# a16z/Lasso

Measured on AMD Instinct MI355X. Metric: prover lookups/sec for SparsePolynomialEvaluationProof, 2^24 AND lookups, higher is better.
Workload: dtype u256 (Montgomery Fr / ed25519 Fq integers)

## Files before the change

lasso_amd/_abi.py:

```python
import ctypes as C

u64 = C.c_uint64
u32 = C.c_uint32
i32 = C.c_int32
sz = C.c_size_t
vp = C.c_void_p


class Strategy(C.Structure):
    _fields_ = [("kind", i32), ("c", u32), ("log_m", u32), ("log_r", u32)]


class StrategyCustom(C.Structure):
    _fields_ = [("base", Strategy), ("num_subtables", u32), ("num_memories", u32), ("tables_u32", C.POINTER(vp)), ("tables_fr", C.POINTER(vp)),
                ("memory_subtable", vp), ("memory_dimension", vp), ("num_terms", u32), ("reserved", u32), ("coeff", vp), ("term_start", vp), ("term_mem", vp)]


class OperandLayout(C.Structure):
    _fields_ = [("operands", u32), ("chunk_bits", u32), ("msb_first", u32)]

    def __repr__(self):
        return f"OperandLayout({self.operands}, {self.chunk_bits}, {self.msb_first})"


# ... 101 lines not shown
        "lasso_rccl_selftest": (i32, [vp]),
        "lasso_ctx_device_uuid": (i32, [vp, vp]),
        "lasso_bullet_tail_ahead_ok": (i32, [vp, vp]),
        "lasso_bullet_tail_ahead": (i32, [vp, vp, sz, vp, vp, vp, sz, vp, vp, vp]),
        "lasso_bases_prepare": (i32, [vp, vp, u32]),
        "lasso_rccl_allgather": (i32, [vp, vp, vp, sz]),
        "lasso_point_row_bytes": (sz, []),
        "lasso_hyrax_commit_rows_dev": (i32, [vp, vp, sz, sz, vp, vp]),
        "lasso_points_reduce_compress": (i32, [vp, vp, u32, sz, vp]),
        "lasso_gather_u32": (i32, [vp, vp, vp, sz, vp]),
        "lasso_materialize_subtable_u32": (i32, [vp, P(Strategy), u32, vp]),
        "lasso_msm": (i32, [vp, vp, vp, sz, vp]),
        "lasso_msm_dev": (i32, [vp, vp, vp, sz, vp]),
        "lasso_inner_products_lr": (i32, [vp, vp, vp, sz, vp]),
        "lasso_bullet_lr": (i32, [vp, vp, sz, vp, sz, vp, vp, vp]),
        "lasso_bullet_round": (i32, [vp, vp, sz, vp, vp, vp, vp, vp, vp, sz, vp, vp, vp, vp]),
        "lasso_bullet_ahead_ok": (i32, [vp, vp]),
        "lasso_bullet_round_ahead": (i32, [vp, vp, sz, vp, vp, vp, vp, vp, vp, sz, vp]),
        "lasso_bullet_post": (i32, [vp, vp, vp]),
        "lasso_bullet_fold": (i32, [vp, vp, vp, sz, vp, sz, vp, vp, vp]),
    }
    for name, (res, args) in sig.items():
        fn = getattr(lib, name)
        fn.restype = res
        fn.argtypes = args
    return sorted(sig)


WIRE_STATUS = ["ok", "ok-identity", "non-canonical", "bad-flags", "not-on-curve", "not-in-subgroup"]


def declare_wire(lib):
    fn = lib.lasso_points_decompress
    fn.restype = i32
    fn.argtypes = [vp, vp, sz, vp, vp, vp]
    return ["lasso_points_decompress"]


def declare_msm_points(lib):
    for name in ("lasso_msm_points", "lasso_msm_points_dev"):
        fn = getattr(lib, name)
        fn.restype = i32
        fn.argtypes = [vp, vp, vp, sz, vp]
    return ["lasso_msm_points", "lasso_msm_points_dev"]


def declare_operands(lib):
    fn = lib.lasso_densify_dim_operands
    fn.restype = i32
    fn.argtypes = [vp, vp, vp, sz, C.POINTER(OperandLayout), sz, sz, sz, u32, u32, u32, vp, vp, vp, vp]
    return ["lasso_densify_dim_operands"]


HEADER_SYMBOLS = None
```

lasso_amd/build.py:

```python
import os
import subprocess
import sys

HERE = os.path.dirname(os.path.abspath(__file__))
ROOT = os.path.dirname(HERE)
HIPCC = os.environ.get("HIPCC", "/opt/rocm/bin/hipcc")
ARCH = "gfx950"


def _stale(target, sources):
    if not os.path.exists(target):
        return True
    t = os.path.getmtime(target)
    return any(os.path.getmtime(s) > t for s in sources)


def _glob(d, exts):
    return [os.path.join(d, f) for f in sorted(os.listdir(d)) if f.endswith(exts)]


CURVES = {"curve25519": ("", []), "bn254": ("_bn254", ["-DLASSO_BN254", "-Wl,-Bsymbolic"])}


def build_device(force=False, verbose=False, curve="curve25519"):
    suffix, flags = CURVES[curve]
    csrc = os.path.join(HERE, "csrc")
    target = os.path.join(HERE, f"liblasso_hip{suffix}.so")
    sources = _glob(csrc, (".hip", ".cuh")) + [os.path.join(ROOT, "include", f) for f in ("lasso_hip.h", "lasso_hip_wire.h", "lasso_hip_msm.h", "lasso_hip_operands.h", "lasso_custom_check.h")]
    if force or _stale(target, sources):
        extra = os.environ.get("LASSO_EXTRA_HIPCC_FLAGS", "").split()
        cmd = [HIPCC, f"--offload-arch={ARCH}", "-O3", "-std=c++17", "-fPIC", "-shared", "-Wno-unused-result", *flags, *extra,
               "-o", target, os.path.join(csrc, "lasso_hip.hip")]
        if verbose:
            print(" ".join(cmd))
        subprocess.check_call(cmd)
    return target


def host_march_flags():
    ov = os.environ.get("LASSO_HOST_MARCH")
    if ov:
        return [] if ov == "none" else [f"-march={ov}"] + (["-DLASSO_HOST_V3"] if ov == "x86-64-v3" else [])
    try:
        flags = set(next(l for l in open("/proc/cpuinfo") if l.startswith("flags")).split())
    except Exception:
        flags = set()
    if {"avx2", "bmi1", "bmi2", "fma", "movbe"} <= flags:
        return ["-march=x86-64-v3", "-DLASSO_HOST_V3"]
    return []


def build_host(force=False, verbose=False, curve="curve25519"):
    suffix, flags = CURVES[curve]
    hdir = os.path.join(HERE, "host")
    target = os.path.join(HERE, f"liblasso_prover{suffix}.so")
    sources = _glob(hdir, (".cpp", ".hpp")) + _glob(os.path.join(HERE, "csrc"), (".cuh",)) + [os.path.join(ROOT, "include", f) for f in ("lasso_hip.h", "lasso_hip_wire.h", "lasso_hip_msm.h", "lasso_hip_operands.h", "lasso_prover.h", "lasso_custom_check.h")]
    if not os.path.exists(os.path.join(hdir, "prover_capi.cpp")):
        return None
    dev = build_device(force=False, verbose=verbose, curve=curve)
    if force or _stale(target, sources + [dev]):
        cmd = ["g++", "-O2", *host_march_flags(), "-std=c++17", "-fPIC", "-shared", "-Wall", "-Wno-unused-function", "-Wno-unknown-pragmas", "-fno-gnu-unique", "-Wl,-Bsymbolic", *flags, "-o", target,
               os.path.join(hdir, "prover_capi.cpp"), "-L" + HERE, f"-llasso_hip{suffix}", "-Wl,-rpath,$ORIGIN"]
        if verbose:
            print(" ".join(cmd))
        subprocess.check_call(cmd)
    return target


def build_all(force=False, verbose=False):
    out = []
    for curve in CURVES:
        out += [build_device(force, verbose, curve), build_host(force, verbose, curve)]
    return tuple(out)


if __name__ == "__main__":
    print(build_all(force="--force" in sys.argv, verbose=True))
```

lasso_amd/csrc/densify_kernels.cuh:

```cuda
#pragma once
#include <hip/hip_runtime.h>
#include "fr29.cuh"
#include "operand_layout.cuh"

#define RADIX_TILE 4096
#define RADIX_THREADS 256

__global__ void __launch_bounds__(256) k_densify_extract(const uint64_t* __restrict__ idx, size_t n_lookups, size_t C, size_t col, size_t s, uint64_t m, uint32_t world, uint32_t rank,
                                                          uint32_t* __restrict__ keys, uint32_t* __restrict__ vals, uint32_t* __restrict__ dim_u32, fr_t* __restrict__ dim_fr, uint32_t* __restrict__ bad) {
  const fr29 r2s = fr29_r2s();
  for (size_t k = blockIdx.x * (size_t)blockDim.x + threadIdx.x; k < s; k += (size_t)gridDim.x * blockDim.x) {
    uint64_t a = k < n_lookups ? idx[k * C + col] : 0;
    if (a >= m) { atomicOr(bad, 1u); a = 0; }
    keys[k] = (uint32_t)a; vals[k] = (uint32_t)k;
    if (k % world == rank) { dim_u32[k / world] = (uint32_t)a; dim_fr[k / world] = fr29_store(fr29_mul(fr29_from_u64_int(a), r2s)); }
  }
}

__global__ void __launch_bounds__(256) k_densify_extract_operands(const uint64_t* __restrict__ x, const uint64_t* __restrict__ y, size_t n_lookups, lasso_operand_layout layout, size_t C, size_t col, size_t s,
                                                                   uint32_t world, uint32_t rank, uint32_t* __restrict__ keys, uint32_t* __restrict__ vals, uint32_t* __restrict__ dim_u32,
                                                                   fr_t* __restrict__ dim_fr, uint32_t* __restrict__ bad) {
  const fr29 r2s = fr29_r2s();
  for (size_t k = blockIdx.x * (size_t)blockDim.x + threadIdx.x; k < s; k += (size_t)gridDim.x * blockDim.x) {
    uint64_t a = 0;
// ... 44 lines not shown
  for (size_t b0 = 0; b0 < nb; b0 += 256) {
    const size_t i = b0 + threadIdx.x;
    const uint32_t v = i < nb ? sums[i] : 0;
    uint32_t total; const uint32_t ex = block_exscan_256(v, sm, total);
    if (i < nb) sums[i] = carry + ex;
    __syncthreads();
    if (threadIdx.x == 0) carry += total;
    __syncthreads();
  }
}
__global__ void __launch_bounds__(256) k_scan_apply(uint32_t* __restrict__ data, size_t n, const uint32_t* __restrict__ sums) {
  __shared__ uint32_t sm[256];
  const size_t base = (size_t)blockIdx.x * 4096 + (size_t)threadIdx.x * 16;
  uint32_t v[16], s = 0;
  for (int j = 0; j < 16; j++) { v[j] = base + j < n ? data[base + j] : 0; s += v[j]; }
  uint32_t total; uint32_t run = sums[blockIdx.x] + block_exscan_256(s, sm, total);
  for (int j = 0; j < 16; j++) if (base + j < n) { data[base + j] = run; run += v[j]; }
}

__global__ void __launch_bounds__(RADIX_THREADS) k_radix_scatter(const uint32_t* __restrict__ keys_in, const uint32_t* __restrict__ vals_in, size_t n, uint32_t shift, const uint32_t* __restrict__ offs,
                                                                  uint32_t ntiles, uint32_t* __restrict__ keys_out, uint32_t* __restrict__ vals_out) {
  __shared__ uint32_t next[256];
  const uint32_t t = threadIdx.x, tile = blockIdx.x, lane = t & 63, wave = t >> 6;
  next[t] = offs[(size_t)t * ntiles + tile];
  __syncthreads();
  const size_t base = (size_t)tile * RADIX_TILE;
  for (uint32_t r = 0; r < RADIX_TILE / RADIX_THREADS; r++) {
    const size_t i = base + r * RADIX_THREADS + t;
    const bool valid = i < n;
    const uint32_t key = valid ? keys_in[i] : 0, val = valid ? vals_in[i] : 0, d = (key >> shift) & 255u;
    uint64_t peers = __ballot(valid);
#pragma unroll
    for (int b = 0; b < 8; b++) { const uint64_t bal = __ballot((d >> b) & 1u); peers &= ((d >> b) & 1u) ? bal : ~bal; }
    const uint32_t rank = (uint32_t)__popcll(peers & ((1ull << lane) - 1ull)), cnt = (uint32_t)__popcll(peers);
    uint32_t pos = 0;
    for (uint32_t w = 0; w < RADIX_THREADS / 64; w++) {
      if (wave == w && valid) pos = next[d] + rank;
      __syncthreads();
      if (wave == w && valid && rank == 0) next[d] += cnt;
      __syncthreads();
    }
    if (valid) { keys_out[pos] = key; vals_out[pos] = val; }
  }
}

__global__ void __launch_bounds__(256) k_densify_runs(const uint32_t* __restrict__ skeys, size_t s, uint32_t* __restrict__ run_start, uint32_t* __restrict__ run_end) {
  for (size_t i = blockIdx.x * (size_t)blockDim.x + threadIdx.x; i < s; i += (size_t)gridDim.x * blockDim.x) {
    const uint32_t a = skeys[i];
    if (i == 0 || skeys[i - 1] != a) run_start[a] = (uint32_t)i;
    if (i + 1 == s || skeys[i + 1] != a) run_end[a] = (uint32_t)(i + 1);
  }
}
__global__ void __launch_bounds__(256) k_densify_read(const uint32_t* __restrict__ skeys, const uint32_t* __restrict__ svals, size_t s, const uint32_t* __restrict__ run_start, uint32_t world,
                                                       uint32_t rank, fr_t* __restrict__ read_fr) {
  const fr29 r2s = fr29_r2s();
  for (size_t i = blockIdx.x * (size_t)blockDim.x + threadIdx.x; i < s; i += (size_t)gridDim.x * blockDim.x) {
    const uint32_t pos = svals[i];
    if (pos % world != rank) continue;
    const uint32_t ts = (uint32_t)i - run_start[skeys[i]];
    read_fr[pos / world] = fr29_store(fr29_mul(fr29_from_u64_int(ts), r2s));
  }
}
__global__ void __launch_bounds__(256) k_densify_final(const uint32_t* __restrict__ run_start, const uint32_t* __restrict__ run_end, size_t m, uint32_t world, uint32_t rank, fr_t* __restrict__ final_fr) {
  const fr29 r2s = fr29_r2s();
  for (size_t a = (blockIdx.x * (size_t)blockDim.x + threadIdx.x) * world + rank; a < m; a += (size_t)gridDim.x * blockDim.x * world)
    final_fr[a / world] = fr29_store(fr29_mul(fr29_from_u64_int(run_end[a] - run_start[a]), r2s));
}
```

lasso_amd/csrc/device_switches.cuh:

```cuda
#pragma once
#include <cstddef>
#include <cstdint>
#include <cstdlib>

namespace lasso { namespace dsw {
inline bool unless0(const char* e) { return !(e && e[0] == '0'); }
inline bool if1(const char* e) { return e && e[0] == '1'; }
#define LASSO_DSWITCH(type, name, value) inline type name() { static const type v = (value); return v; }
LASSO_DSWITCH(bool, tagged_results, unless0(getenv("LASSO_TAGGED_RESULTS")))
LASSO_DSWITCH(long long, seq_start, [] { const char* e = getenv("LASSO_SEQ_START"); return e ? (long long)(uint32_t)strtoul(e, nullptr, 0) : -1LL; }())
LASSO_DSWITCH(bool, msm_tagged, unless0(getenv("LASSO_MSM_TAGGED")))
LASSO_DSWITCH(long, cubic_nx, [] { const char* e = getenv("LASSO_CUBIC_NX"); return e ? atol(e) : 0L; }())
LASSO_DSWITCH(bool, cubic_wide, unless0(getenv("LASSO_CUBIC_WIDE")))
LASSO_DSWITCH(unsigned, direct_nx, [] { const char* e = getenv("LASSO_DIRECT_NX"); const long x = e ? atol(e) : 16; return (unsigned)(x < 0 ? 0 : x > 64 ? 64 : x); }())
LASSO_DSWITCH(bool, eq_inline_big, if1(getenv("LASSO_EQ_INLINE_BIG")))
LASSO_DSWITCH(bool, lb_pipeline, unless0(getenv("LASSO_LB_PIPELINE")))
LASSO_DSWITCH(bool, lb_nt, if1(getenv("LASSO_LB_NT")))
LASSO_DSWITCH(unsigned, ahead_inkernel_wgs, [] { const char* e = getenv("LASSO_AHEAD_INKERNEL_WGS"); const long x = e ? atol(e) : 32; return (unsigned)(x < 0 ? 0 : x > 4096 ? 4096 : x); }())
LASSO_DSWITCH(bool, rounds_ahead, unless0(getenv("LASSO_ROUNDS_AHEAD")))
LASSO_DSWITCH(bool, layer_ahead, unless0(getenv("LASSO_LAYER_AHEAD")))
LASSO_DSWITCH(bool, tail_q_256, [] { const char* e = getenv("LASSO_TAIL_Q"); return (e ? atol(e) : 0) == 256; }())
LASSO_DSWITCH(bool, exp_no_leaf_store, if1(getenv("LASSO_EXP_NO_LEAF_STORE")))
LASSO_DSWITCH(size_t, msm_direct_max_n, [] { const char* e = getenv("LASSO_MSM_DIRECT_MAX_N"); return e ? (size_t)atoll(e) : (((size_t)1 << 17) + 64); }())
LASSO_DSWITCH(size_t, msm_direct8_max_n, [] { if (!unless0(getenv("LASSO_MSM_DIRECT8"))) return (size_t)0; const char* e = getenv("LASSO_MSM_DIRECT8_MAX_N"); return e ? (size_t)atoll(e) : (((size_t)1 << 14) + 64); }())
LASSO_DSWITCH(bool, msm_direct, unless0(getenv("LASSO_MSM_DIRECT")))
LASSO_DSWITCH(long, msm_direct_wgs, [] { const char* e = getenv("LASSO_MSM_DIRECT_WGS"); return e ? atol(e) : 0L; }())
LASSO_DSWITCH(bool, msm_fused, unless0(getenv("LASSO_MSM_FUSED")))
LASSO_DSWITCH(bool, msm_rows8, unless0(getenv("LASSO_MSM_ROWS8")))
LASSO_DSWITCH(bool, msm_rows8w, unless0(getenv("LASSO_MSM_ROWS8W")))
LASSO_DSWITCH(size_t, msm_rows8w_waves, [] { const char* e = getenv("LASSO_MSM_ROWS8W_WAVES"); const long x = e ? atol(e) : 0; return (size_t)(x < 0 ? 0 : x); }())
LASSO_DSWITCH(bool, msm_full8, if1(getenv("LASSO_MSM_FULL8")))
LASSO_DSWITCH(bool, bullet_ahead, unless0(getenv("LASSO_BULLET_AHEAD")))
LASSO_DSWITCH(bool, bullet_tail_ahead, unless0(getenv("LASSO_BULLET_TAIL_AHEAD")))
inline bool msm_pip() { return unless0(getenv("LASSO_MSM_PIP")); }
inline size_t msm_pip_min_cols() { const char* e = getenv("LASSO_MSM_PIP_MIN_COLS"); const long x = e ? atol(e) : 512; return (size_t)(x < 1 ? 1 : x); }
inline size_t msm_pip_scratch_mb() { const char* e = getenv("LASSO_MSM_PIP_SCRATCH_MB"); const long x = e ? atol(e) : 1200; return (size_t)(x < 16 ? 16 : x); }
#undef LASSO_DSWITCH
} }
```

lasso_amd/csrc/fr29.cuh:

```cuda
#pragma once
#include <stdint.h>
#include "fr.cuh"
#include "mont29.cuh"

#ifdef LASSO_BN254
struct Bn254FrM {
  static LHD int32_t p(int k) { const int32_t P[9] = {268435457, 521120927, 240919632, 131109107, 361091715, 47923392, 10936641, 240920116, 3171406}; return P[k]; }
  static constexpr uint32_t PINV = 268435455u;
  static constexpr int32_t QC = 1420063842;
  static constexpr int32_t ONE_S_0 = 268435287, ONE_S_1 = 514263732, ONE_S_2 = 86771339, ONE_S_3 = 391139145, ONE_S_4 = 178784091, ONE_S_5 = 490881230, ONE_S_6 = 299191303,
                           ONE_S_7 = 86689704, ONE_S_8 = 903222;
  static constexpr int32_t K522_0 = 95853524, K522_1 = 102173274, K522_2 = 34397646, K522_3 = 498479371, K522_4 = 240439551, K522_5 = 486036963, K522_6 = 471195907,
                           K522_7 = 131109217, K522_8 = 656714;
  static LHD m29<Bn254FrM> k5() { return m29_limbs<Bn254FrM>(268430039, 492061940, 71535269, 62181526, 323781850, 244503300, 348886451, 68918589, 360451); }
  static LHD m29<Bn254FrM> k10() { return m29_limbs<Bn254FrM>(268262109, 223975601, 492627914, 522739689, 150938553, 164142673, 394138283, 408892696, 2020216); }
  static LHD m29<Bn254FrM> r2s() { return m29_limbs<Bn254FrM>(338539743, 433494286, 343078028, 115075043, 193254777, 284818167, 304038784, 396432094, 1209799); }
};
typedef Bn254FrM FrM29;
#else
struct Curve25519FrM {
  static LHD int32_t p(int k) { const int32_t P[9] = {485872621, 9640146, 501691798, 502512965, 333, 0, 0, 0, 1 << 20}; return P[k]; }
  static constexpr uint32_t PINV = 307527195u;
  static constexpr int32_t ONE_S_0 = 290322925, ONE_S_1 = 442594051, ONE_S_2 = 259787148, ONE_S_3 = 377041255, ONE_S_4 = 536700270, ONE_S_5 = 536870911, ONE_S_6 = 536870911,
                           ONE_S_7 = 536870911, ONE_S_8 = 1048575;
// ... 14 lines not shown

template <> LHD m29<FrM29> m29_canonical<FrM29>(const m29<FrM29>& a) {
  m29<FrM29> w = m29_weak(a);
  const int32_t f = w.v[8] >> 20;
  m29<FrM29> r; int64_t c = 0;
#pragma unroll
  for (int k = 0; k < 9; k++) { int64_t x = (int64_t)w.v[k] - (int64_t)f * FrM29::p(k) + c; if (k < 8) { r.v[k] = (int32_t)x & M29_MASK; c = x >> 29; } else r.v[8] = (int32_t)x; }
  const int32_t g = r.v[8] >> 20;
  m29<FrM29> s; c = 0;
#pragma unroll
  for (int k = 0; k < 9; k++) { int64_t x = (int64_t)r.v[k] - (int64_t)g * FrM29::p(k) + c; if (k < 8) { s.v[k] = (int32_t)x & M29_MASK; c = x >> 29; } else s.v[8] = (int32_t)x; }
  const bool keep_r = s.v[8] < 0;
#pragma unroll
  for (int k = 0; k < 9; k++) s.v[k] = keep_r ? r.v[k] : s.v[k];
  return s;
}
template <> LHD m29<FrM29> m29_reduce_columns<FrM29>(const int64_t* col, int shift) {
  int64_t l[9]; int64_t c = 0;
#pragma unroll
  for (int k = 0; k < 9; k++) { const int64_t x = col[k] * ((int64_t)1 << shift) + c; if (k < 8) { l[k] = x & M29_MASK; c = x >> 29; } else l[8] = x; }
  const int32_t f = (int32_t)(l[8] >> 20) - 1;
  m29<FrM29> r; c = 0;
#pragma unroll
  for (int k = 0; k < 9; k++) { const int64_t x = l[k] - (int64_t)f * FrM29::p(k) + c; if (k < 8) { r.v[k] = (int32_t)x & M29_MASK; c = x >> 29; } else r.v[8] = (int32_t)x; }
  return m29_canonical(r);
}
template <> LHD m29<FrM29> m29_from_columns<FrM29>(const int64_t* col) {
  const int32_t ONE_S[9] = {FrM29::ONE_S_0, FrM29::ONE_S_1, FrM29::ONE_S_2, FrM29::ONE_S_3, FrM29::ONE_S_4, FrM29::ONE_S_5, FrM29::ONE_S_6, FrM29::ONE_S_7, FrM29::ONE_S_8};
  int64_t l[9]; int64_t c = 0;
#pragma unroll
  for (int k = 0; k < 9; k++) { int64_t x = col[k] + c; c = x >> 29; l[k] = x & M29_MASK; }
  m29<FrM29> r; int64_t d = 0;
#pragma unroll
  for (int k = 0; k < 9; k++) { int64_t x = l[k] + c * ONE_S[k] + d; if (k < 8) { r.v[k] = (int32_t)x & M29_MASK; d = x >> 29; } else r.v[8] = (int32_t)x; }
  return r;
}
#endif

typedef m29<FrM29> fr29;
typedef m29_acc<FrM29> fr29_acc;
#define FR29_MASK M29_MASK

static constexpr auto& fr29_from_limbs = m29_limbs<FrM29>;
#ifdef LASSO_BN254
LHD fr29 fr29_zero() { return m29_zero<FrM29>(); }
LHD fr29 fr29_add(const fr29& a, const fr29& b) { return m29_add(a, b); }
LHD fr29 fr29_sub(const fr29& a, const fr29& b) { return m29_sub(a, b); }
LHD fr29 fr29_weak(const fr29& a) { return m29_weak(a); }
LHD fr29 fr29_mul(const fr29& a, const fr29& b) { return m29_mul(a, b); }
LHD fr29_acc fr29_acc_zero() { return m29_acc_zero<FrM29>(); }
LHD void fr29_mul_acc(fr29_acc& acc, const fr29& a, const fr29& b) { m29_mul_acc(acc, a, b); }
LHD void fr29_acc_carry(fr29_acc& acc) { m29_acc_carry(acc); }
LHD fr29 fr29_acc_reduce(const fr29_acc& acc) { return m29_acc_reduce(acc); }
LHD fr29 fr29_semi(const fr29& a) { return m29_near(a); }
LHD fr29 fr29_canonical(const fr29& a) { return m29_canonical(a); }
LHD fr29 fr29_reduce_columns(const int64_t* col, int shift) { return m29_reduce_columns<FrM29>(col, shift); }
LHD fr29 fr29_from_columns(const int64_t* col) { return m29_from_columns<FrM29>(col); }
LHD fr29 fr29_unpack_u(const fr_t& x) { return m29_unpack_words<FrM29>(x.v); }
LHD fr29 fr29_unpack_s(const fr_t& x) { return m29_unpack_words_shl5<FrM29>(x.v); }
LHD fr_t fr29_pack(const fr29& a) { fr_t r; m29_pack_words(a, r.v); return r; }
#else
static constexpr auto& fr29_zero = m29_zero<FrM29>;
static constexpr auto& fr29_add = m29_add<FrM29>;
static constexpr auto& fr29_sub = m29_sub<FrM29>;
static constexpr auto& fr29_weak = m29_weak<FrM29>;
static constexpr auto& fr29_mul = m29_mul<FrM29>;
static constexpr auto& fr29_acc_zero = m29_acc_zero<FrM29>;
static constexpr auto& fr29_mul_acc = m29_mul_acc<FrM29>;
static constexpr auto& fr29_acc_carry = m29_acc_carry<FrM29>;
static constexpr auto& fr29_acc_reduce = m29_acc_reduce<FrM29>;
static constexpr auto& fr29_semi = m29_near<FrM29>;
static constexpr auto& fr29_canonical = m29_canonical<FrM29>;
static constexpr auto& fr29_reduce_columns = m29_reduce_columns<FrM29>;
static constexpr auto& fr29_from_columns = m29_from_columns<FrM29>;
LHD fr29 fr29_unpack_u(const fr_t& x) {
  fr29 r;
#pragma unroll
  for (int k = 0; k < 9; k++) {
    const int bit = 29 * k, w = bit >> 5, s = bit & 31;
    uint64_t two = (uint64_t)x.v[w] | ((w + 1 < 8) ? ((uint64_t)x.v[w + 1] << 32) : 0);
    r.v[k] = (int32_t)((uint32_t)(two >> s) & FR29_MASK);
  }
  return r;
}
LHD fr29 fr29_unpack_s(const fr_t& x) {
  fr29 r;
  r.v[0] = (int32_t)((x.v[0] << 5) & FR29_MASK);
#pragma unroll
  for (int k = 1; k < 9; k++) {
    const int bit = 29 * k - 5, w = bit >> 5, s = bit & 31;
    uint64_t two = (uint64_t)x.v[w] | ((w + 1 < 8) ? ((uint64_t)x.v[w + 1] << 32) : 0);
    r.v[k] = (int32_t)((uint32_t)(two >> s) & FR29_MASK);
  }
  return r;
}
LHD fr_t fr29_pack(const fr29& a) {
  fr_t r;
#pragma unroll
  for (int w = 0; w < 8; w++) {
    const int k0 = (32 * w) / 29, s = 32 * w - 29 * k0;
    uint64_t acc = (uint64_t)(uint32_t)a.v[k0] >> s;
    int have = 29 - s;
    if (k0 + 1 < 9) { acc |= (uint64_t)(uint32_t)a.v[k0 + 1] << have; have += 29; }
    if (have < 32 && k0 + 2 < 9) acc |= (uint64_t)(uint32_t)a.v[k0 + 2] << have;
    r.v[w] = (uint32_t)acc;
  }
  return r;
}
#endif

LHD fr29 fr29_one_s() { return fr29_from_limbs(FrM29::ONE_S_0, FrM29::ONE_S_1, FrM29::ONE_S_2, FrM29::ONE_S_3, FrM29::ONE_S_4, FrM29::ONE_S_5, FrM29::ONE_S_6, FrM29::ONE_S_7, FrM29::ONE_S_8); }
LHD fr29 fr29_k5() { return FrM29::k5(); }
LHD fr29 fr29_k10() { return FrM29::k10(); }
LHD fr29 fr29_r2s() { return FrM29::r2s(); }
LHD fr29 fr29_int_from_uu() { fr29 r = fr29_zero(); r.v[0] = 1 << 10; return r; }
LHD fr29 fr29_from_u64_int(uint64_t x) { return fr29_from_limbs((int32_t)(x & FR29_MASK), (int32_t)((x >> 29) & FR29_MASK), (int32_t)(x >> 58), 0, 0, 0, 0, 0, 0); }
LHD fr_t fr29_store(const fr29& a) { return fr29_pack(fr29_canonical(a)); }
```

lasso_amd/csrc/lasso_hip.hip:

```cpp
#include <hip/hip_runtime.h>
#include <mutex>
#include <string>
#include <unordered_map>
#include <vector>
#include <cstring>
#include <functional>
#include <cstdio>
#include <cstdlib>
#include <ctime>
#include "../../include/lasso_hip.h"
#include "device_switches.cuh"
#include "launch_plan.cuh"
#include "poly_kernels.cuh"
#include "msm_kernels.cuh"
#include "densify_kernels.cuh"
#include "../../include/lasso_hip_wire.h"
#include "wire_kernels.cuh"
#include "../../include/lasso_hip_msm.h"
#include "msm_points_kernels.cuh"
#include "../../include/lasso_hip_operands.h"

__global__ void __launch_bounds__(256) k_inner_lr(const fr_t* __restrict__ a, const fr_t* __restrict__ b, size_t half, fr_t* __restrict__ partials) {
  __shared__ RedScratch S;
  fr29 acc[3] = {fr29_zero(), fr29_zero(), fr29_zero()}; uint32_t cnt = 0;
  for (size_t i = blockIdx.x * (size_t)blockDim.x + threadIdx.x; i < half; i += (size_t)gridDim.x * blockDim.x) {
    acc[0] = fr29_weak(fr29_add(acc[0], fr29_mul(fr29_unpack_u(a[i]), fr29_unpack_s(b[half + i]))));
    acc[1] = fr29_weak(fr29_add(acc[1], fr29_mul(fr29_unpack_u(a[half + i]), fr29_unpack_s(b[i]))));
    if ((++cnt & 127u) == 0) { acc[0] = fr29_mul(acc[0], fr29_one_s()); acc[1] = fr29_mul(acc[1], fr29_one_s()); }
  }
  store_block_partials<3>(acc, 2, partials + 2 * (size_t)blockIdx.x, 0, S);
}

static_assert(sizeof(lasso_fr) == 32 && sizeof(fr_t) == 32, "Fr layout");
static_assert(sizeof(lasso_affine) == 64 && sizeof(lasso_point) == 128 && sizeof(ed_point) == 128 && sizeof(niels29) == (MSM_NIELS_ALIGN > 16 ? 128 : 112) && sizeof(pt29) == MSM_PT29_BYTES, "curve layouts");

namespace dsw = lasso::dsw;
struct EventPair { hipEvent_t a, b; int kid; double bytes, units, units2; bool large; bool counted; };
#define LASSO_PROF_COUNT_SLOTS 4096
struct lasso_ctx {
  int device = 0;
  hipStream_t stream = nullptr;
  std::string err;
  void* d_scratch = nullptr; size_t scratch_cap = 0;
  void* d_pip = nullptr; size_t pip_cap = 0;
  fr_t* d_small = nullptr;
  fr_t* h_small = nullptr;
  size_t small_cap = 0;
  uint32_t* h_flag = nullptr; uint32_t* d_flag = nullptr;
  uint32_t* h_tag = nullptr; uint32_t* d_tag = nullptr;
  bool tagged = true;
  HandoffState proto;
  std::vector<lasso_fr> group_tmp;
  uint32_t* mail_h = nullptr; uint32_t* mail_d = nullptr;
  uint32_t seq = 0;
  uint64_t stat_waits = 0; double stat_wait_us = 0;
  fr_t* d_big = nullptr; fr_t* h_big = nullptr; size_t big_cap = 0;
  uint32_t* d_flags = nullptr;
  uint32_t* d_counters = nullptr;
  uint32_t* d_gmail = nullptr;
  uint32_t* pmail_h = nullptr; uint32_t* pmail_d = nullptr; uint32_t* d_gpoint = nullptr;
  uint32_t prof_mask = 0;
  std::vector<EventPair> events; size_t events_used = 0;
  uint64_t prof_launches[LASSO_K_COUNT] = {0}; double prof_ms[LASSO_K_COUNT] = {0}; double prof_bytes[LASSO_K_COUNT] = {0};
  uint64_t big_launches[LASSO_K_COUNT] = {0}; double big_ms[LASSO_K_COUNT] = {0}; double big_bytes[LASSO_K_COUNT] = {0};
  double prof_units[LASSO_K_COUNT] = {0}; double big_units[LASSO_K_COUNT] = {0};
  double prof_units2[LASSO_K_COUNT] = {0}; double big_units2[LASSO_K_COUNT] = {0};
  double prof_units3[LASSO_K_COUNT] = {0}; double big_units3[LASSO_K_COUNT] = {0};
  uint32_t* d_prof_counts = nullptr;
  void* d_terms = nullptr; std::vector<uint8_t> terms_host;
  void* rccl_comm = nullptr; int rccl_world = 0; int rccl_rank = -1;
  std::unordered_map<void*, size_t> mem_sizes; uint64_t mem_live = 0, mem_peak = 0; std::mutex mem_mu;
};
struct lasso_bases {
  size_t n = 0; niels29* d_table = nullptr;
  lasso_ctx* owner = nullptr;
  niels29* d_mult = nullptr;
  niels29* d_mult8 = nullptr;
  niels29* d_tab8[2] = {nullptr, nullptr};
  bool tab8_failed = false;
  std::mutex tab8_mu;
};

static thread_local std::string g_create_err;
static std::mutex g_ctx_mu; static std::vector<lasso_ctx*> g_ctx_live;
static lasso_ctx* live_or_null(lasso_ctx* c) { std::lock_guard<std::mutex> g(g_ctx_mu); for (lasso_ctx* x : g_ctx_live) if (x == c) return c; return nullptr; }

static int32_t fail(lasso_ctx* c, int32_t code, const std::string& msg) { if (c) c->err = msg; else g_create_err = msg; return code; }
#define HIPCHK(c, call) do { hipError_t e_ = (call); if (e_ != hipSuccess) return fail((c), e_ == hipErrorOutOfMemory ? LASSO_ERR_OOM : LASSO_ERR_HIP, std::string(#call) + ": " + hipGetErrorString(e_)); } while (0)
static inline bool bind_device(lasso_ctx* c) { if (!c) return true; int d = -1; if (hipGetDevice(&d) == hipSuccess && d == c->device) return true; return hipSetDevice(c->device) == hipSuccess; }
#define REQUIRE(c, cond) do { if (!bind_device(c)) return fail((c), LASSO_ERR_HIP, "hipSetDevice failed for the context's device"); \
                              if (!(cond)) return fail((c), LASSO_ERR_INVALID, std::string("invalid argument: ") + #cond); } while (0)

static hipError_t dmalloc(lasso_ctx* c, void** p, size_t bytes) {
  hipError_t e = hipMalloc(p, bytes);
  if (e == hipSuccess && c) { std::lock_guard<std::mutex> g(c->mem_mu); c->mem_sizes[*p] = bytes; c->mem_live += bytes; if (c->mem_live > c->mem_peak) c->mem_peak = c->mem_live; }
  return e;
}
static hipError_t dfree(lasso_ctx* c, void* p) {
  if (c && p) { std::lock_guard<std::mutex> g(c->mem_mu); auto it = c->mem_sizes.find(p); if (it != c->mem_sizes.end()) { c->mem_live -= it->second; c->mem_sizes.erase(it); } }
  return hipFree(p);
}

static int32_t grow_guard(lasso_ctx* c) {
  if (c->proto.no_grow) return LASSO_ERR_UNSUPPORTED;
  if (c->proto.waiting_on_device()) return fail(c, LASSO_ERR_INVALID, "a launch is waiting on the device for its challenge: only lasso_result_wait and the post of that challenge are legal until then");
  return 0;
}
static int32_t ensure_scratch(lasso_ctx* c, size_t bytes) {
  if (bytes <= c->scratch_cap) return 0;
  if (int32_t g = grow_guard(c)) return g;
// ... 985 lines not shown
}
int32_t lasso_read_heads(lasso_ctx* c, const lasso_fr* const* d_polys, uint32_t k, lasso_fr* out) {
  REQUIRE(c, d_polys && out && k >= 1 && k <= LASSO_MAX_PTRS);
  PtrTable P; for (uint32_t i = 0; i < k; i++) { REQUIRE(c, d_polys[i]); P.p[i] = (const fr_t*)d_polys[i]; }
  int32_t rc = ensure_small(c, k); if (rc) return rc;
  hipLaunchKernelGGL(k_read_heads, dim3(1), dim3(LASSO_BLOCK), 0, c->stream, P, k, c->d_small);
  HIPCHK(c, hipGetLastError());
  return fetch_small(c, k, out);
}
int32_t lasso_read_runs(lasso_ctx* c, const lasso_fr* const* d_polys, uint32_t k, uint32_t count, lasso_fr* out) {
  REQUIRE(c, d_polys && out && k >= 1 && k <= LASSO_MAX_PTRS && count >= 1 && (size_t)k * count <= 16384);
  PtrTable P; for (uint32_t i = 0; i < k; i++) { REQUIRE(c, d_polys[i]); P.p[i] = (const fr_t*)d_polys[i]; }
  int32_t rc = ensure_small(c, (size_t)k * count); if (rc) return rc;
  hipLaunchKernelGGL(k_read_runs, dim3((k * count + LASSO_BLOCK - 1) / LASSO_BLOCK), dim3(LASSO_BLOCK), 0, c->stream, P, k, count, c->d_small);
  HIPCHK(c, hipGetLastError());
  return fetch_small(c, (size_t)k * count, out);
}
static void gp_layers_from(lasso_ctx* c, fr_t* in, size_t len) {
  while (len >= 16 * LASSO_BLOCK) {
    const size_t q = len / 4;
    hipLaunchKernelGGL(k_gp_layer2, dim3(grid_for(q, 4096)), dim3(LASSO_BLOCK), 0, c->stream, (const fr_t*)in, q, in + len, in + len + len / 2);
    in += len + len / 2; len = q;
  }
  while (len > 2 * LASSO_BLOCK) {
    size_t half = len / 2;
    hipLaunchKernelGGL(k_gp_layer, dim3(grid_for(half, 4096)), dim3(LASSO_BLOCK), 0, c->stream, (const fr_t*)in, half, in + len);
    in += len; len = half;
  }
  if (len > 2) hipLaunchKernelGGL(k_gp_tail, dim3(1), dim3(LASSO_BLOCK), 0, c->stream, in, len);
}
int32_t lasso_gp_build(lasso_ctx* c, lasso_fr* d_tree, size_t n) {
  REQUIRE(c, d_tree && n >= 2 && (n & (n - 1)) == 0);
  ProfScope ps(c, LASSO_K_GP, 48.0 * n * 2.0);
  gp_layers_from(c, (fr_t*)d_tree, n);
  HIPCHK(c, hipGetLastError()); return 0;
}
int32_t lasso_fingerprint_ops_gp(lasso_ctx* c, const lasso_fr* d_table, const uint32_t* d_dim, const lasso_fr* d_read, size_t s, const lasso_fr* gamma, const lasso_fr* tau,
                                 lasso_fr* d_tree_r, lasso_fr* d_tree_w) {
  REQUIRE(c, d_table && d_dim && d_read && gamma && tau && d_tree_r && d_tree_w && s >= 4 && (s & (s - 1)) == 0);
  fr_t g = to_fr(gamma), g2 = fr_sqr(g), t = to_fr(tau);
  fr_t* tr = (fr_t*)d_tree_r; fr_t* tw = (fr_t*)d_tree_w;
  {
    ProfScope ps(c, LASSO_K_FINGERPRINT, (32.0 * 3 + 64.0) * s + 2 * 48.0 * s);
    const uint32_t store_leaves = dsw::exp_no_leaf_store() ? 0u : 1u;
    hipLaunchKernelGGL(k_fingerprint_ops_l1<false>, dim3(grid_for(s / 2, 4096)), dim3(LASSO_BLOCK), 0, c->stream, (const fr_t*)d_table, d_dim, (const void*)d_read, s, g, g2, t, tr, tw, tr + s, tw + s, store_leaves);
  }
  {
    ProfScope ps(c, LASSO_K_GP, 2 * 48.0 * s);
    gp_layers_from(c, tr + s, s / 2);
    gp_layers_from(c, tw + s, s / 2);
  }
  HIPCHK(c, hipGetLastError()); return 0;
}
static int32_t fingerprint_gp_upper_impl(lasso_ctx* c, const lasso_fr* d_table, const uint32_t* d_dim, const void* d_read, bool read_u32, size_t s, const lasso_fr* gamma, const lasso_fr* tau,
                                         lasso_fr* d_upper_r, lasso_fr* d_upper_w) {
  REQUIRE(c, d_table && d_dim && d_read && gamma && tau && d_upper_r && d_upper_w && s >= 4 && (s & (s - 1)) == 0);
  fr_t g = to_fr(gamma), g2 = fr_sqr(g), t = to_fr(tau);
  fr_t* ur = (fr_t*)d_upper_r; fr_t* uw = (fr_t*)d_upper_w;
  {
    ProfScope ps(c, LASSO_K_FINGERPRINT, (32.0 * 3 + 64.0) * s + 2 * 48.0 * s);
    if (read_u32) hipLaunchKernelGGL(k_fingerprint_ops_l1<true>, dim3(grid_for(s / 2, 4096)), dim3(LASSO_BLOCK), 0, c->stream, (const fr_t*)d_table, d_dim, d_read, s, g, g2, t, (fr_t*)nullptr, (fr_t*)nullptr, ur, uw, 0u);
    else hipLaunchKernelGGL(k_fingerprint_ops_l1<false>, dim3(grid_for(s / 2, 4096)), dim3(LASSO_BLOCK), 0, c->stream, (const fr_t*)d_table, d_dim, d_read, s, g, g2, t, (fr_t*)nullptr, (fr_t*)nullptr, ur, uw, 0u);
  }
  {
    ProfScope ps(c, LASSO_K_GP, 2 * 48.0 * s);
    gp_layers_from(c, ur, s / 2);
    gp_layers_from(c, uw, s / 2);
  }
  HIPCHK(c, hipGetLastError()); return 0;
}
int32_t lasso_fingerprint_ops_gp_upper(lasso_ctx* c, const lasso_fr* d_table, const uint32_t* d_dim, const lasso_fr* d_read, size_t s, const lasso_fr* gamma, const lasso_fr* tau,
                                       lasso_fr* d_upper_r, lasso_fr* d_upper_w) { return fingerprint_gp_upper_impl(c, d_table, d_dim, d_read, false, s, gamma, tau, d_upper_r, d_upper_w); }
int32_t lasso_fingerprint_ops_gp_upper_u32(lasso_ctx* c, const lasso_fr* d_table, const uint32_t* d_dim, const uint32_t* d_read_u32, size_t s, const lasso_fr* gamma, const lasso_fr* tau,
                                           lasso_fr* d_upper_r, lasso_fr* d_upper_w) { return fingerprint_gp_upper_impl(c, d_table, d_dim, d_read_u32, true, s, gamma, tau, d_upper_r, d_upper_w); }
static int32_t fingerprint_strips_impl(lasso_ctx* c, const lasso_fr* d_table, const uint32_t* d_dim, const void* d_read, bool read_u32, size_t s, const lasso_fr* gamma, const lasso_fr* tau,
                                       uint32_t nstrips, size_t i0, size_t cs, lasso_fr* d_out_r, lasso_fr* d_out_w) {
  REQUIRE(c, d_table && d_dim && d_read && gamma && tau && d_out_r && d_out_w && s >= 4 && (s & (s - 1)) == 0 && (nstrips == 2 || nstrips == 4) && cs >= 1);
  const size_t stride = s / 2 / nstrips;
  REQUIRE(c, stride >= 1 && i0 + cs <= stride);
  fr_t g = to_fr(gamma), g2 = fr_sqr(g), t = to_fr(tau);
  const size_t total = 2 * (size_t)nstrips * cs;
  ProfScope ps(c, LASSO_K_FINGERPRINT, (32.0 * 3 + 64.0) * total);
  if (read_u32) hipLaunchKernelGGL(k_fingerprint_ops_strips<true>, dim3(grid_for(total, 4096)), dim3(LASSO_BLOCK), 0, c->stream, (const fr_t*)d_table, d_dim, d_read, s, g, g2, t, nstrips, stride, i0, cs, (fr_t*)d_out_r, (fr_t*)d_out_w);
  else hipLaunchKernelGGL(k_fingerprint_ops_strips<false>, dim3(grid_for(total, 4096)), dim3(LASSO_BLOCK), 0, c->stream, (const fr_t*)d_table, d_dim, d_read, s, g, g2, t, nstrips, stride, i0, cs, (fr_t*)d_out_r, (fr_t*)d_out_w);
  HIPCHK(c, hipGetLastError()); return 0;
}
int32_t lasso_fingerprint_ops_strips(lasso_ctx* c, const lasso_fr* d_table, const uint32_t* d_dim, const lasso_fr* d_read, size_t s, const lasso_fr* gamma, const lasso_fr* tau,
                                     uint32_t nstrips, size_t i0, size_t cs, lasso_fr* d_out_r, lasso_fr* d_out_w) { return fingerprint_strips_impl(c, d_table, d_dim, d_read, false, s, gamma, tau, nstrips, i0, cs, d_out_r, d_out_w); }
int32_t lasso_fingerprint_ops_strips_u32(lasso_ctx* c, const lasso_fr* d_table, const uint32_t* d_dim, const uint32_t* d_read_u32, size_t s, const lasso_fr* gamma, const lasso_fr* tau,
                                         uint32_t nstrips, size_t i0, size_t cs, lasso_fr* d_out_r, lasso_fr* d_out_w) { return fingerprint_strips_impl(c, d_table, d_dim, d_read_u32, true, s, gamma, tau, nstrips, i0, cs, d_out_r, d_out_w); }
int32_t lasso_fingerprint_ops(lasso_ctx* c, const lasso_fr* d_table, const uint32_t* d_dim, const lasso_fr* d_read, size_t s, const lasso_fr* gamma, const lasso_fr* tau,
                              lasso_fr* d_read_out, lasso_fr* d_write_out) {
  REQUIRE(c, d_table && d_dim && d_read && gamma && tau && d_read_out && d_write_out); if (!s) return 0;
  fr_t g = to_fr(gamma), g2 = fr_sqr(g), t = to_fr(tau);
  ProfScope ps(c, LASSO_K_FINGERPRINT, (32.0 * 3 + 64.0) * s);
  hipLaunchKernelGGL(k_fingerprint_ops, dim3(grid_for(s, 4096)), dim3(LASSO_BLOCK), 0, c->stream, (const fr_t*)d_table, d_dim, (const fr_t*)d_read, s, g, g2, t, (fr_t*)d_read_out, (fr_t*)d_write_out);
  HIPCHK(c, hipGetLastError()); return 0;
}
int32_t lasso_fingerprint_mem(lasso_ctx* c, const lasso_fr* d_table, const lasso_fr* d_final, size_t m, const lasso_fr* gamma, const lasso_fr* tau, lasso_fr* d_init_out, lasso_fr* d_final_out) {
  return lasso_fingerprint_mem_slab(c, d_table, d_final, m, 1, 0, gamma, tau, d_init_out, d_final_out);
}
int32_t lasso_fingerprint_mem_slab(lasso_ctx* c, const lasso_fr* d_table, const lasso_fr* d_final, size_t m, uint32_t world, uint32_t rank, const lasso_fr* gamma, const lasso_fr* tau,
                                   lasso_fr* d_init_out, lasso_fr* d_final_out) {
  REQUIRE(c, d_table && d_final && gamma && tau && d_init_out && d_final_out && world >= 1 && rank < world); if (!m) return 0;
  fr_t g = to_fr(gamma), g2 = fr_sqr(g), t = to_fr(tau);
  ProfScope ps(c, LASSO_K_FINGERPRINT, (64.0 + 64.0) * m);
// ... 17 lines not shown
  HIPCHK(c, hipGetLastError());
  HIPCHK(c, hipMemcpyAsync(c->h_big, c->d_big, r_size * sizeof(fr_t), hipMemcpyDeviceToHost, c->stream));
  HIPCHK(c, hipStreamSynchronize(c->stream));
  memcpy(out, c->h_big, r_size * sizeof(fr_t));
  return 0;
}

int32_t lasso_matvec_left_dev(lasso_ctx* c, const lasso_fr* d_Z, const lasso_fr* d_L, size_t l_size, size_t r_size, lasso_fr* d_out) {
  REQUIRE(c, d_Z && d_L && d_out && l_size >= 1 && r_size >= 1);
  size_t col_blocks = (r_size + LASSO_BLOCK - 1) / LASSO_BLOCK;
  size_t nchunks = (1024 + col_blocks - 1) / col_blocks; if (nchunks > l_size) nchunks = l_size; if (nchunks < 1) nchunks = 1;
  size_t rows_per_chunk = (l_size + nchunks - 1) / nchunks; nchunks = (l_size + rows_per_chunk - 1) / rows_per_chunk;
  int32_t rc = ensure_scratch(c, nchunks * r_size * sizeof(fr_t)); if (rc) return rc;
  fr_t* partials = (fr_t*)c->d_scratch;
  ProfScope ps(c, LASSO_K_MATVEC, 32.0 * l_size * r_size);
  hipLaunchKernelGGL(k_matvec_left, dim3((unsigned)col_blocks, (unsigned)nchunks), dim3(LASSO_BLOCK), 0, c->stream, (const fr_t*)d_Z, (const fr_t*)d_L, l_size, r_size, rows_per_chunk, partials);
  hipLaunchKernelGGL(k_matvec_reduce, dim3((unsigned)col_blocks), dim3(LASSO_BLOCK), 0, c->stream, (const fr_t*)partials, nchunks, r_size, (fr_t*)d_out);
  HIPCHK(c, hipGetLastError()); return 0;
}
int32_t lasso_fr_to_u32(lasso_ctx* c, const lasso_fr* d_src, size_t n, uint32_t* d_dst, uint32_t* max_out) {
  REQUIRE(c, d_src && d_dst && n >= 1);
  HIPCHK(c, hipMemsetAsync(c->d_flags, 0, 8, c->stream));
  hipLaunchKernelGGL(k_fr_to_u32, dim3(grid_for(n, 4096)), dim3(256), 0, c->stream, (const fr_t*)d_src, n, d_dst, c->d_flags);
  HIPCHK(c, hipGetLastError());
  uint32_t flags[2];
  HIPCHK(c, hipMemcpyAsync(flags, c->d_flags, 8, hipMemcpyDeviceToHost, c->stream));
  HIPCHK(c, hipStreamSynchronize(c->stream));
  if (flags[1]) return fail(c, LASSO_ERR_INVALID, "lasso_fr_to_u32: a value does not fit 32 bits");
  if (max_out) *max_out = flags[0];
  return 0;
}
int32_t lasso_fr_to_bytes(lasso_ctx* c, const lasso_fr* d_src, size_t n, uint8_t* out) {
  REQUIRE(c, d_src && out && n >= 1);
  if (n <= ((size_t)1 << 16)) {
    int32_t rc = ensure_small(c, n); if (rc) return rc;
    hipLaunchKernelGGL(k_fr_to_canonical, dim3(grid_for(n)), dim3(256), 0, c->stream, (const fr_t*)d_src, n, c->d_small);
    HIPCHK(c, hipGetLastError());
    return fetch_small(c, n, (lasso_fr*)out);
  }
  int32_t rc = ensure_scratch(c, n * sizeof(fr_t)); if (rc) return rc;
  hipLaunchKernelGGL(k_fr_to_canonical, dim3(grid_for(n)), dim3(256), 0, c->stream, (const fr_t*)d_src, n, (fr_t*)c->d_scratch);
  HIPCHK(c, hipGetLastError());
  HIPCHK(c, hipMemcpyAsync(out, c->d_scratch, n * 32, hipMemcpyDeviceToHost, c->stream));
  HIPCHK(c, hipStreamSynchronize(c->stream));
  return 0;
}

int32_t lasso_densify_dim(lasso_ctx* c, const uint64_t* d_indices, size_t n_lookups, size_t C, size_t dim, size_t s, uint32_t log_m, uint32_t* d_dim_u32, lasso_fr* d_dim, lasso_fr* d_read,
                          lasso_fr* d_final) {
  return lasso_densify_dim_slab(c, d_indices, n_lookups, C, dim, s, log_m, 1, 0, d_dim_u32, d_dim, d_read, d_final);
}
static int32_t densify_dim_run(lasso_ctx* c, size_t n_lookups, size_t s, uint32_t log_m, uint32_t world, uint32_t rank, lasso_fr* d_read, lasso_fr* d_final, double extract_bytes,
                               const char* bad_msg, const std::function<void(uint32_t*, uint32_t*)>& extract) {
  const size_t m = (size_t)1 << log_m;
  const uint32_t ntiles = (uint32_t)((s + RADIX_TILE - 1) / RADIX_TILE);
  const size_t nh = (size_t)256 * ntiles, nb = (nh + 4095) / 4096;
  const size_t words = 4 * s + nh + nb + 2 * m + 64;
  int32_t rc = ensure_scratch(c, words * 4); if (rc) return rc;
  uint32_t* kA = (uint32_t*)c->d_scratch; uint32_t* vA = kA + s; uint32_t* kB = vA + s; uint32_t* vB = kB + s;
  uint32_t* hist = vB + s; uint32_t* sums = hist + nh; uint32_t* run_start = sums + nb; uint32_t* run_end = run_start + m;
  HIPCHK(c, hipMemsetAsync(c->d_flags, 0, 8, c->stream));
  HIPCHK(c, hipMemsetAsync(run_start, 0, 2 * m * 4, c->stream));
  ProfScope ps(c, LASSO_K_MISC, extract_bytes + (32.0 * 2 + 4.0) * s + 32.0 * m);
  extract(kA, vA);
  const uint32_t npass = log_m == 0 ? 1 : (log_m + 7) / 8;
  for (uint32_t p = 0; p < npass; p++) {
    hipLaunchKernelGGL(k_radix_hist, dim3(ntiles), dim3(RADIX_THREADS), 0, c->stream, (const uint32_t*)kA, s, 8 * p, hist, ntiles);
    hipLaunchKernelGGL(k_scan_block_sums, dim3((unsigned)nb), dim3(256), 0, c->stream, (const uint32_t*)hist, nh, sums);
    hipLaunchKernelGGL(k_scan_sums, dim3(1), dim3(256), 0, c->stream, sums, nb);
    hipLaunchKernelGGL(k_scan_apply, dim3((unsigned)nb), dim3(256), 0, c->stream, hist, nh, (const uint32_t*)sums);
    hipLaunchKernelGGL(k_radix_scatter, dim3(ntiles), dim3(RADIX_THREADS), 0, c->stream, (const uint32_t*)kA, (const uint32_t*)vA, s, 8 * p, (const uint32_t*)hist, ntiles, kB, vB);
    std::swap(kA, kB); std::swap(vA, vB);
  }
  hipLaunchKernelGGL(k_densify_runs, dim3(grid_for(s, 4096)), dim3(256), 0, c->stream, (const uint32_t*)kA, s, run_start, run_end);
  hipLaunchKernelGGL(k_densify_read, dim3(grid_for(s, 4096)), dim3(256), 0, c->stream, (const uint32_t*)kA, (const uint32_t*)vA, s, (const uint32_t*)run_start, world, rank, (fr_t*)d_read);
  hipLaunchKernelGGL(k_densify_final, dim3(grid_for(m / world, 4096)), dim3(256), 0, c->stream, (const uint32_t*)run_start, (const uint32_t*)run_end, m, world, rank, (fr_t*)d_final);
  HIPCHK(c, hipGetLastError());
  uint32_t flags[2];
  HIPCHK(c, hipMemcpyAsync(flags, c->d_flags, 8, hipMemcpyDeviceToHost, c->stream));
  HIPCHK(c, hipStreamSynchronize(c->stream));
  if (flags[0]) return fail(c, LASSO_ERR_INVALID, bad_msg);
  return 0;
}
int32_t lasso_densify_dim_slab(lasso_ctx* c, const uint64_t* d_indices, size_t n_lookups, size_t C, size_t dim, size_t s, uint32_t log_m, uint32_t world, uint32_t rank, uint32_t* d_dim_u32,
                               lasso_fr* d_dim, lasso_fr* d_read, lasso_fr* d_final) {
  REQUIRE(c, d_indices && d_dim_u32 && d_dim && d_read && d_final && C >= 1 && dim < C && s >= 1 && (s & (s - 1)) == 0 && n_lookups <= s && s < ((size_t)1 << 32) && log_m <= 32);
  REQUIRE(c, world >= 1 && (world & (world - 1)) == 0 && rank < world && world <= s && world <= ((size_t)1 << log_m));
  return densify_dim_run(c, n_lookups, s, log_m, world, rank, d_read, d_final, 8.0 * n_lookups, "lookup index out of range (memory_address >= M, densified.rs:46)", [&](uint32_t* kA, uint32_t* vA) {
    hipLaunchKernelGGL(k_densify_extract, dim3(grid_for(s, 4096)), dim3(256), 0, c->stream, d_indices, n_lookups, C, dim, s, (uint64_t)1 << log_m, world, rank, kA, vA, d_dim_u32, (fr_t*)d_dim, c->d_flags);
  });
}
int32_t lasso_densify_dim_operands(lasso_ctx* c, const uint64_t* d_x, const uint64_t* d_y, size_t n_lookups, const lasso_operand_layout* layout, size_t C, size_t dim, size_t s, uint32_t log_m,
                                   uint32_t world, uint32_t rank, uint32_t* d_dim_u32, lasso_fr* d_dim, lasso_fr* d_read, lasso_fr* d_final) {
  REQUIRE(c, d_x && d_dim_u32 && d_dim && d_read && d_final && C >= 1 && dim < C && s >= 1 && (s & (s - 1)) == 0 && n_lookups <= s && s < ((size_t)1 << 32) && log_m <= 32);
  REQUIRE(c, world >= 1 && (world & (world - 1)) == 0 && rank < world && world <= s && world <= ((size_t)1 << log_m));
  if (const int bad = operand_layout_check(layout, C, log_m)) return fail(c, LASSO_ERR_INVALID, std::string("lasso_densify_dim_operands: ") + operand_layout_error(bad));
  if ((d_y != nullptr) != (layout->operands == 2u)) return fail(c, LASSO_ERR_INVALID, "lasso_densify_dim_operands: " OPL_MSG_Y);
  const lasso_operand_layout L = *layout;
  return densify_dim_run(c, n_lookups, s, log_m, world, rank, d_read, d_final, 8.0 * L.operands * n_lookups, "lasso_densify_dim_operands: " OPL_MSG_FIT, [&](uint32_t* kA, uint32_t* vA) {
    hipLaunchKernelGGL(k_densify_extract_operands, dim3(grid_for(s, 4096)), dim3(256), 0, c->stream, d_x, d_y, n_lookups, L, C, dim, s, world, rank, kA, vA, d_dim_u32, (fr_t*)d_dim, c->d_flags);
  });
}

int32_t lasso_points_decompress(lasso_ctx* c, const uint8_t* wire32, size_t n, lasso_affine* out, uint8_t* canon32, uint8_t* status) {
  REQUIRE(c, status && (wire32 || n == 0) && n < ((size_t)1 << 31));
  if (!n) return 0;
  int32_t rc = ensure_scratch(c, 129 * n);
  if (rc) return rc == LASSO_ERR_UNSUPPORTED ? fail(c, rc, "lasso_points_decompress: the scratch buffer cannot grow while a resident kernel is active") : rc;
  uint8_t* base = (uint8_t*)c->d_scratch;
  HIPCHK(c, hipMemcpyAsync(base, wire32, 32 * n, hipMemcpyHostToDevice, c->stream));
  {
    ProfScope ps(c, LASSO_K_MISC, 129.0 * n);
    hipLaunchKernelGGL(k_points_decompress, dim3((unsigned)((n + WIRE_THREADS - 1) / WIRE_THREADS)), dim3(WIRE_THREADS), 0, c->stream, (const uint4*)base, n, (uint4*)(base + 32 * n), (uint4*)(base + 96 * n), base + 128 * n);
  }
  HIPCHK(c, hipGetLastError());
  std::vector<uint8_t> host(97 * n);
  HIPCHK(c, hipMemcpyAsync(host.data(), base + 32 * n, 97 * n, hipMemcpyDeviceToHost, c->stream));
  HIPCHK(c, hipStreamSynchronize(c->stream));
  if (out) memcpy(out, host.data(), 64 * n);
  if (canon32) memcpy(canon32, host.data() + 64 * n, 32 * n);
  memcpy(status, host.data() + 96 * n, n);
  return 0;
}
int32_t lasso_bases_create(lasso_ctx* c, const lasso_affine* points, size_t n, lasso_bases** out) { return lasso_bases_create_opt(c, points, n, 1, out); }
int32_t lasso_bases_create_opt(lasso_ctx* c, const lasso_affine* points, size_t n, int32_t byte_multiples, lasso_bases** out) {
  REQUIRE(c, points && out && n >= 1 && n * MSM_WINDOWS < ((size_t)1 << 32));
  lasso_bases* b = new lasso_bases(); b->n = n; b->owner = c;
  void* d_aff = nullptr;
// ... 29 lines not shown
  for (niels29* t : b->d_tab8) if (t) (void)dfree(o, t);
  delete b;
}
static const niels29* ensure_tab8(lasso_ctx* c, const lasso_bases* cb, uint32_t w8) {
  lasso_bases* b = const_cast<lasso_bases*>(cb);
  std::lock_guard<std::mutex> lock(b->tab8_mu);
  if (b->d_tab8[w8]) return b->d_tab8[w8];
  if (b->tab8_failed) return nullptr;
  niels29* t = nullptr;
  lasso_ctx* const owner = live_or_null(b->owner);
  if (dmalloc(owner, (void**)&t, (size_t)MSM8_MULTS * b->n * sizeof(niels29)) != hipSuccess) { (void)hipGetLastError(); b->tab8_failed = true; return nullptr; }
  hipLaunchKernelGGL(k_precompute_tab8, dim3((unsigned)((b->n + 63) / 64)), dim3(64), 0, c->stream, (const niels29*)b->d_table, b->n, w8, t);
  if (hipGetLastError() != hipSuccess || hipStreamSynchronize(c->stream) != hipSuccess) { (void)hipGetLastError(); (void)dfree(owner, t); b->tab8_failed = true; return nullptr; }
  b->d_tab8[w8] = t;
  return t;
}
int32_t lasso_bases_prepare(lasso_ctx* c, const lasso_bases* b, uint32_t byte_windows) {
  REQUIRE(c, b && byte_windows >= 1 && byte_windows <= 2 && !c->proto.waiting_on_device() && !c->proto.tail_active);
  if (!dsw::msm_rows8()) return 0;
  for (uint32_t w = 0; w < byte_windows; w++) if (!ensure_tab8(c, b, w)) break;
  return 0;
}

static size_t msm_pts_bytes(size_t rows, size_t n_cols) { return msm_pts_bytes(rows, n_cols, msm_direct_wgs(dsw::msm_direct_wgs())); }
static bool msm_tagged(lasso_ctx* c) { return c->tagged && dsw::msm_tagged(); }
#define MSM_RES(c) (msm_tagged(c) ? (ed_point*)(c)->d_tag : (ed_point*)(c)->d_small), (c)->d_counters + LASSO_MAX_PTRS + 8, (msm_tagged(c) ? LASSO_TAGGED : (c)->d_flag)
static int32_t run_msm_direct(lasso_ctx* c, const uint8_t* d_scal, size_t row_stride, size_t rows, size_t n_cols, const MsmColMap& cm, const lasso_bases* b, uint8_t* scratch_after, lasso_point* out,
                              int mode = 0, const lasso_fr* scale = nullptr, const lasso_fr* tail = nullptr, uint32_t sstride = 1, uint32_t soffset = 0,
                              const lasso_fr* const* heads = nullptr, const uint32_t* gate_seq = nullptr) {
  const MsmDirectPlan P = msm_direct_plan(rows, n_cols, b->d_mult8 != nullptr, dsw::msm_direct_wgs());
  const size_t K = P.K; const uint32_t ipc = P.ipc;
  const uint32_t seq = gate_seq ? *gate_seq : next_seq(c);
  const fr_t* const h0 = heads ? (const fr_t*)heads[0] : nullptr; const fr_t* const h1 = heads ? (const fr_t*)heads[1] : nullptr;
  const uint32_t* const ggm = gate_seq ? (const uint32_t*)c->d_gmail : nullptr;
  {
    ProfScope ps(c, LASSO_K_MSM_DIRECT, (double)rows * n_cols * 32, P.ref_adds, false, P.adds);
    const fr_t z = fr_zero();
#define LAUNCH_DIRECT(M, WB_, TAB_, SC, T0, T1) hipLaunchKernelGGL((k_msm_direct<M, WB_>), dim3((unsigned)K, (unsigned)rows), dim3(MSM_THREADS), 0, c->stream, (const uint32_t*)d_scal, row_stride / 4, (uint32_t)n_cols, ipc, cm, \
                       (const niels29*)TAB_, b->n, (pt29*)scratch_after, MSM_RES(c), seq, SC, T0, T1, ps.counter(), sstride, soffset, h0, h1, ggm)
    if (P.w8) {
      if (mode == 0) LAUNCH_DIRECT(0, 8, b->d_mult8, z, z, z);
      else if (mode == 1) LAUNCH_DIRECT(1, 8, b->d_mult8, z, z, z);
      else LAUNCH_DIRECT(2, 8, b->d_mult8, to_fr(scale), to_fr(tail), to_fr(tail + 1));
    } else {
      if (mode == 0) LAUNCH_DIRECT(0, 4, b->d_mult, z, z, z);
      else if (mode == 1) LAUNCH_DIRECT(1, 4, b->d_mult, z, z, z);
      else LAUNCH_DIRECT(2, 4, b->d_mult, to_fr(scale), to_fr(tail), to_fr(tail + 1));
    }
  }
  HIPCHK(c, hipGetLastError());
  if (gate_seq) return 0;
  return wait_flag(c, seq, rows * (sizeof(ed_point) / sizeof(fr_t)), (lasso_fr*)out, msm_tagged(c));
}
static int32_t run_msm(lasso_ctx* c, const uint8_t* d_scal, uint32_t bps, uint32_t W, size_t row_stride, size_t rows, size_t n_cols, const lasso_bases* b, uint8_t* scratch_after, lasso_point* out,
                       uint8_t* out_compressed = nullptr, void* d_rows_out = nullptr) {
  const MsmShape shape = {bps, W, rows, n_cols, out_compressed != nullptr, d_rows_out != nullptr};
  const MsmSwitches sw = {dsw::msm_direct(), dsw::msm_rows8(), dsw::msm_rows8w(), dsw::msm_full8(), dsw::msm_pip(), dsw::msm_rows8w_waves(), dsw::msm_pip_min_cols(), dsw::msm_pip_scratch_mb(), dsw::msm_direct_wgs()};
  MsmHave have = {b->n, b->d_mult != nullptr, b->d_mult8 != nullptr, true, true};
  MsmPlan P = msm_plan(shape, have, sw);
  if (P.kernel == MSM_K_DIRECT) { const MsmColMap id = {0, 0, 0, 0}; return run_msm_direct(c, d_scal, row_stride, rows, n_cols, id, b, scratch_after, out); }
  const niels29* t8[2] = {nullptr, nullptr};
  if (P.kernel == MSM_K_ROWS8W || P.kernel == MSM_K_ROWS8) {
    t8[0] = ensure_tab8(c, b, 0); t8[1] = P.W8 > 1 && t8[0] ? ensure_tab8(c, b, 1) : t8[0];
    if (!t8[1]) { have.tab8 = false; P = msm_plan(shape, have, sw); }
  } else if (P.kernel == MSM_K_PIP && ensure_pip(c, P.pip_group * P.pip_row_bytes + 256) != 0) { have.pip_scratch = false; P = msm_plan(shape, have, sw); }
  if (d_rows_out) out_compressed = (uint8_t*)d_rows_out;
  const size_t K = P.K;
  pt29* d_partial = (pt29*)scratch_after;
  const bool small = P.result == MSM_R_FLAG;
  ed_point* d_final = small ? (ed_point*)c->d_small : (ed_point*)(((uintptr_t)(d_partial + rows * K) + 15) & ~(uintptr_t)15);
  const uint32_t seq = small ? next_seq(c) : 0;
  {
    ProfScope ps(c, LASSO_K_MSM, (double)rows * n_cols * bps, P.ref_adds, rows > MSM_SMALL_ROWS, P.adds);
    switch (P.kernel) {
      case MSM_K_ROWS8W:
        hipLaunchKernelGGL(k_msm_rows8w, dim3((unsigned)((P.waves + MSM_THREADS / 64 - 1) / (MSM_THREADS / 64))), dim3(MSM_THREADS), 0, c->stream, (const uint32_t*)d_scal, row_stride / 4,
                           (uint32_t)n_cols, P.W8, t8[0], t8[1], b->n, d_partial, (uint32_t)rows, ps.counter(), (uint32_t)P.rpw);
        break;
      case MSM_K_ROWS8:
        hipLaunchKernelGGL(k_msm_rows8, dim3((unsigned)K, (unsigned)rows), dim3(MSM_THREADS), 0, c->stream, (const uint32_t*)d_scal, row_stride / 4, (uint32_t)n_cols, (uint32_t)P.cols_per_chunk, P.W8,
                           t8[0], t8[1], b->n, d_partial, ps.counter());
        break;
      case MSM_K_PIP: {
        const size_t pip_group = P.pip_group, pip_items = P.pip_items;
        uint8_t* base = (uint8_t*)c->d_pip;
        uint32_t* d_sorted = (uint32_t*)base; uint32_t* d_offs = d_sorted + pip_group * pip_items; uint16_t* d_perm = (uint16_t*)(d_offs + pip_group * (MSM_PIP_BUCKETS + 1));
        uint8_t* d_vtop = (uint8_t*)(d_perm + pip_group * MSM_PIP_BUCKETS);
        pt29* d_bk = (pt29*)((((uintptr_t)(d_vtop + pip_group * n_cols)) + 15) & ~(uintptr_t)15);
        for (size_t r0 = 0; r0 < rows; r0 += pip_group) {
          const unsigned g = (unsigned)(rows - r0 < pip_group ? rows - r0 : pip_group);
          hipLaunchKernelGGL(k_msm_pip_sort, dim3(g), dim3(MSM_THREADS), 0, c->stream, d_scal + r0 * row_stride, row_stride, (uint32_t)n_cols, (uint32_t)b->n, d_sorted, pip_items, d_offs, d_perm, d_vtop, ps.counter());
          hipLaunchKernelGGL(k_msm_pip_accumulate, dim3(g, MSM_PIP_PER_THREAD), dim3(MSM_THREADS), 0, c->stream, (const uint32_t*)d_sorted, pip_items, (const uint32_t*)d_offs, (const uint16_t*)d_perm, (const niels29*)b->d_table, d_bk);
          hipLaunchKernelGGL(k_msm_pip_reduce, dim3(g), dim3(MSM_THREADS), 0, c->stream, (const pt29*)d_bk, (const uint8_t*)d_vtop, (uint32_t)n_cols, (const niels29*)b->d_table + (size_t)(MSM_WINDOWS - 1) * b->n, d_partial + r0);
        }
      } break;
      case MSM_K_FULL8:
        hipLaunchKernelGGL((k_msm_rows_full<8>), dim3((unsigned)K, (unsigned)rows), dim3(MSM_THREADS), 0, c->stream, (const uint32_t*)d_scal, row_stride / 4, (uint32_t)n_cols, (uint32_t)P.cols_per_chunk,
                           (const niels29*)b->d_mult8, b->n, d_partial, ps.counter());
        break;
      default:
        hipLaunchKernelGGL(k_msm_buckets, dim3((unsigned)K, (unsigned)rows), dim3(MSM_THREADS), 0, c->stream, d_scal, bps, W, row_stride, n_cols, P.cols_per_chunk, (const niels29*)b->d_table, b->n, d_partial, ps.counter());
    }
    hipLaunchKernelGGL(k_points_sum, dim3((unsigned)rows), dim3(MSM_THREADS), 0, c->stream, (const pt29*)d_partial, (uint32_t)K, d_final, out_compressed ? (uint32_t*)d_final : (uint32_t*)nullptr,
                       c->d_counters + LASSO_MAX_PTRS + 1, small ? c->d_flag : (uint32_t*)nullptr, seq);
  }
  HIPCHK(c, hipGetLastError());
  switch (P.result) {
    case MSM_R_DEVICE_ROWS: HIPCHK(c, hipMemcpyAsync(d_rows_out, d_final, rows * sizeof(pt29), hipMemcpyDeviceToDevice, c->stream)); return 0;
    case MSM_R_COMPRESSED_MAPPED: {
      int32_t rc = ensure_small(c, rows); if (rc) return rc;
      hipLaunchKernelGGL(k_points_compress, dim3((unsigned)((rows + 255) / 256)), dim3(256), 0, c->stream, (const pt29*)d_final, rows, (uint32_t*)c->d_small);
      HIPCHK(c, hipGetLastError());
      return fetch_small(c, rows, (lasso_fr*)out_compressed);
    }
    case MSM_R_COMPRESSED_MEMCPY: {
      uint32_t* d_wire = (uint32_t*)(((uintptr_t)((pt29*)d_final + rows) + 15) & ~(uintptr_t)15);
      hipLaunchKernelGGL(k_points_compress, dim3((unsigned)((rows + 255) / 256)), dim3(256), 0, c->stream, (const pt29*)d_final, rows, d_wire);
      HIPCHK(c, hipGetLastError());
      HIPCHK(c, hipMemcpyAsync(out_compressed, d_wire, rows * 32, hipMemcpyDeviceToHost, c->stream));
      HIPCHK(c, hipStreamSynchronize(c->stream));
      return 0;
    }
    case MSM_R_FLAG: return wait_flag(c, seq, rows * (sizeof(ed_point) / sizeof(fr_t)), (lasso_fr*)out);
    default: break;
  }
  HIPCHK(c, hipMemcpyAsync(out, d_final, rows * sizeof(ed_point), hipMemcpyDeviceToHost, c->stream));
  HIPCHK(c, hipStreamSynchronize(c->stream));
  return 0;
}
static int32_t hyrax_commit_impl(lasso_ctx* c, const lasso_fr* d_Z, size_t l_size, size_t r_size, const lasso_bases* b, lasso_point* out, uint8_t* out_compressed, void* d_rows_out = nullptr);
int32_t lasso_hyrax_commit_rows_dev(lasso_ctx* c, const lasso_fr* d_Z, size_t l_size, size_t r_size, const lasso_bases* b, void* d_rows) { REQUIRE(c, d_rows); return hyrax_commit_impl(c, d_Z, l_size, r_size, b, nullptr, nullptr, d_rows); }
size_t lasso_point_row_bytes(void) { return sizeof(pt29); }
int32_t lasso_hyrax_commit(lasso_ctx* c, const lasso_fr* d_Z, size_t l_size, size_t r_size, const lasso_bases* b, lasso_point* out) { REQUIRE(c, out); return hyrax_commit_impl(c, d_Z, l_size, r_size, b, out, nullptr); }
int32_t lasso_hyrax_commit_compressed(lasso_ctx* c, const lasso_fr* d_Z, size_t l_size, size_t r_size, const lasso_bases* b, uint8_t* out32) { REQUIRE(c, out32); return hyrax_commit_impl(c, d_Z, l_size, r_size, b, nullptr, out32); }
static int32_t hyrax_commit_impl(lasso_ctx* c, const lasso_fr* d_Z, size_t l_size, size_t r_size, const lasso_bases* b, lasso_point* out, uint8_t* out_compressed, void* d_rows_out) {
  REQUIRE(c, d_Z && b && l_size >= 1 && r_size >= 1 && r_size <= b->n && l_size < ((size_t)1 << 31));
  const size_t n = l_size * r_size;
  const size_t pts_bytes = msm_pts_bytes(l_size, r_size);
  int32_t rc = ensure_scratch(c, n * 4 + 256 + pts_bytes); if (rc) return rc;
  uint8_t* d_scal = (uint8_t*)c->d_scratch;
  HIPCHK(c, hipMemsetAsync(c->d_flags, 0, 8, c->stream));
  {
    ProfScope ps(c, LASSO_K_MISC, 36.0 * n);
    hipLaunchKernelGGL(k_fr_to_u32, dim3(grid_for(n, 4096)), dim3(256), 0, c->stream, (const fr_t*)d_Z, n, (uint32_t*)d_scal, c->d_flags);
  }
  uint32_t flags[2];
  HIPCHK(c, hipMemcpyAsync(flags, c->d_flags, 8, hipMemcpyDeviceToHost, c->stream));
  HIPCHK(c, hipStreamSynchronize(c->stream));
  if (!flags[1]) {
    uint32_t bits = 0; while (bits < 32 && (flags[0] >> bits)) bits++;
    uint32_t W = (bits + 3) / 4; if (W == 0) W = 1;
    return run_msm(c, d_scal, 4, W, r_size * 4, l_size, r_size, b, d_scal + ((n * 4 + 255) & ~(size_t)255), out, out_compressed, d_rows_out);
  }
  rc = ensure_scratch(c, n * 32 + pts_bytes); if (rc) return rc;
  d_scal = (uint8_t*)c->d_scratch;
  hipLaunchKernelGGL(k_fr_to_canonical, dim3(grid_for(n, 4096)), dim3(256), 0, c->stream, (const fr_t*)d_Z, n, (fr_t*)d_scal);
  return run_msm(c, d_scal, 32, MSM_WINDOWS, r_size * 32, l_size, r_size, b, d_scal + n * 32, out, out_compressed, d_rows_out);
}
int32_t lasso_hyrax_commit_compressed_u32(lasso_ctx* c, const uint32_t* d_u32, uint32_t max_value, size_t l_size, size_t r_size, const lasso_bases* b, uint8_t* out32) {
  REQUIRE(c, d_u32 && out32 && b && l_size >= 1 && r_size >= 1 && r_size <= b->n && l_size < ((size_t)1 << 31));
  int32_t rc = ensure_scratch(c, msm_pts_bytes(l_size, r_size) + 256); if (rc) return rc;
  uint32_t bits = 0; while (bits < 32 && (max_value >> bits)) bits++;
  uint32_t W = (bits + 3) / 4; if (W == 0) W = 1;
  return run_msm(c, (const uint8_t*)d_u32, 4, W, r_size * 4, l_size, r_size, b, (uint8_t*)c->d_scratch, nullptr, out32);
}
__global__ void __launch_bounds__(256) k_gather_u32(const uint32_t* __restrict__ table, const uint32_t* __restrict__ idx, size_t n, uint32_t* __restrict__ out) {
  for (size_t i = blockIdx.x * (size_t)blockDim.x + threadIdx.x; i < n; i += (size_t)gridDim.x * blockDim.x) out[i] = table[idx[i]];
}
int32_t lasso_gather_u32(lasso_ctx* c, const uint32_t* d_table, const uint32_t* d_idx, size_t n, uint32_t* d_out) {
  REQUIRE(c, d_table && d_idx && d_out); if (!n) return 0;
  ProfScope ps(c, LASSO_K_MISC, 12.0 * n);
  hipLaunchKernelGGL(k_gather_u32, dim3(grid_for(n)), dim3(256), 0, c->stream, d_table, d_idx, n, d_out);
  HIPCHK(c, hipGetLastError()); return 0;
}
int32_t lasso_msm(lasso_ctx* c, const lasso_bases* b, const lasso_fr* scalars, size_t n, lasso_point* out) {
  REQUIRE(c, b && scalars && out && n >= 1 && n <= b->n);
  int32_t rc = ensure_scratch(c, n * 64 + msm_pts_bytes(1, n)); if (rc) return rc;
  fr_t* d_in = (fr_t*)c->d_scratch; fr_t* d_can = d_in + n;
  HIPCHK(c, hipMemcpyAsync(d_in, scalars, n * 32, hipMemcpyHostToDevice, c->stream));
  hipLaunchKernelGGL(k_fr_to_canonical, dim3(grid_for(n)), dim3(256), 0, c->stream, (const fr_t*)d_in, n, d_can);
  return run_msm(c, (const uint8_t*)d_can, 32, MSM_WINDOWS, n * 32, 1, n, b, (uint8_t*)(d_can + n), out);
}

int32_t lasso_msm_dev(lasso_ctx* c, const lasso_bases* b, const lasso_fr* d_scalars, size_t n, lasso_point* out) {
  REQUIRE(c, b && d_scalars && out && n >= 1 && n <= b->n);
  int32_t rc = ensure_scratch(c, n * 32 + msm_pts_bytes(1, n)); if (rc) return rc;
  fr_t* d_can = (fr_t*)c->d_scratch;
  if (b->d_mult && dsw::msm_direct() && dsw::msm_fused()) {
    const MsmColMap id = {0, 0, 0, 0};
    return run_msm_direct(c, (const uint8_t*)d_scalars, n * 32, 1, n, id, b, (uint8_t*)c->d_scratch, out, 1);
  }
  hipLaunchKernelGGL(k_fr_to_canonical, dim3(grid_for(n)), dim3(256), 0, c->stream, (const fr_t*)d_scalars, n, d_can);
  return run_msm(c, (const uint8_t*)d_can, 32, MSM_WINDOWS, n * 32, 1, n, b, (uint8_t*)(d_can + n), out);
}
static inline size_t up256(size_t x) { return (x + 255) & ~(size_t)255; }
static int32_t msm_points_impl(lasso_ctx* c, const char* who, const lasso_affine* points, const lasso_fr* scalars, size_t n, bool on_host, lasso_point* out) {
  REQUIRE(c, out && n < ((size_t)1 << 28) && (n == 0 || (points && scalars)));
  const size_t K = n ? (n + MSMP_CHUNK - 1) / MSMP_CHUNK : 1;
  const size_t o_pts = 0, o_scal = o_pts + (on_host ? up256(n * sizeof(lasso_affine)) : 0), o_nl = o_scal + (on_host ? up256(n * sizeof(lasso_fr)) : 0), o_dig = o_nl + up256(n * sizeof(niels29));
  const size_t o_part = o_dig + up256(n * MSMP_NW), o_wsum = o_part + up256(MSMP_NW * K * sizeof(pt29)), o_out = o_wsum + up256(MSMP_NW * sizeof(pt29));
  int32_t rc = ensure_scratch(c, o_out + 256);
  if (rc) return rc == LASSO_ERR_UNSUPPORTED ? fail(c, rc, std::string(who) + ": the scratch buffer cannot grow while a resident kernel is active") : rc;
  uint8_t* base = (uint8_t*)c->d_scratch;
  const fq_t* d_aff = (const fq_t*)points; const fr_t* d_scal = (const fr_t*)scalars;
  if (on_host && n) {
    HIPCHK(c, hipMemcpyAsync(base + o_pts, points, n * sizeof(lasso_affine), hipMemcpyHostToDevice, c->stream));
    HIPCHK(c, hipMemcpyAsync(base + o_scal, scalars, n * sizeof(lasso_fr), hipMemcpyHostToDevice, c->stream));
    d_aff = (const fq_t*)(base + o_pts); d_scal = (const fr_t*)(base + o_scal);
  }
  {
    ProfScope ps(c, LASSO_K_MSM, (double)n * (sizeof(lasso_affine) + sizeof(lasso_fr)), msm_ref_adds(1, n, FR_MODULUS_BITS), false, (double)n * MSMP_NW);
    if (n) hipLaunchKernelGGL(k_msmp_prepare, dim3((unsigned)((n + 255) / 256)), dim3(256), 0, c->stream, d_aff, d_scal, (uint32_t)n, (niels29*)(base + o_nl), (int8_t*)(base + o_dig));
    hipLaunchKernelGGL(k_msmp_buckets, dim3(MSMP_NW, (unsigned)K), dim3(MSM_THREADS), 0, c->stream, (const int8_t*)(base + o_dig), (uint32_t)n, (const niels29*)(base + o_nl), (pt29*)(base + o_part));
    hipLaunchKernelGGL(k_points_sum, dim3(MSMP_NW), dim3(MSM_THREADS), 0, c->stream, (const pt29*)(base + o_part), (uint32_t)K, (ed_point*)nullptr, (uint32_t*)(base + o_wsum),
                       (uint32_t*)nullptr, (uint32_t*)nullptr, 0u);
    hipLaunchKernelGGL(k_msmp_horner, dim3(1), dim3(64), 0, c->stream, (const pt29*)(base + o_wsum), (ed_point*)(base + o_out));
  }
  HIPCHK(c, hipGetLastError());
  HIPCHK(c, hipMemcpyAsync(out, base + o_out, sizeof(ed_point), hipMemcpyDeviceToHost, c->stream));
  HIPCHK(c, hipStreamSynchronize(c->stream));
  return 0;
}
int32_t lasso_msm_points(lasso_ctx* c, const lasso_affine* points, const lasso_fr* scalars, size_t n, lasso_point* out) { return msm_points_impl(c, "lasso_msm_points", points, scalars, n, true, out); }
int32_t lasso_msm_points_dev(lasso_ctx* c, const lasso_affine* d_points, const lasso_fr* d_scalars, size_t n, lasso_point* out) { return msm_points_impl(c, "lasso_msm_points_dev", d_points, d_scalars, n, false, out); }
__global__ void __launch_bounds__(256) k_scale_to_integers(const fr_t* __restrict__ src, size_t n, fr_t scale, fr_t t0, fr_t t1, fr_t* __restrict__ dst) {
  const fr29 ss = fr29_unpack_s(scale); fr29 k32 = fr29_zero(); k32.v[0] = 32;
  for (size_t i = blockIdx.x * (size_t)blockDim.x + threadIdx.x; i < n; i += (size_t)gridDim.x * blockDim.x) dst[i] = fr29_store(fr29_mul(fr29_mul(fr29_unpack_u(src[i]), ss), k32));
// ... 148 lines not shown
```

lasso_amd/csrc/mont29.cuh:

```cuda
#pragma once
#include <stdint.h>

#ifndef LHD
#if defined(__HIPCC__)
#define LHD __host__ __device__ __forceinline__
#else
#define LHD inline
#endif
#endif

#define M29_MASK 0x1fffffff

template <class M> struct m29 { int32_t v[9]; };

template <class M> LHD m29<M> m29_zero() { m29<M> r;
#pragma unroll
  for (int i = 0; i < 9; i++) r.v[i] = 0; return r; }
template <class M> LHD m29<M> m29_limbs(int32_t a0, int32_t a1, int32_t a2, int32_t a3, int32_t a4, int32_t a5, int32_t a6, int32_t a7, int32_t a8) {
  m29<M> r; r.v[0] = a0; r.v[1] = a1; r.v[2] = a2; r.v[3] = a3; r.v[4] = a4; r.v[5] = a5; r.v[6] = a6; r.v[7] = a7; r.v[8] = a8; return r;
}
template <class M> LHD m29<M> m29_add(const m29<M>& a, const m29<M>& b) { m29<M> r;
#pragma unroll
  for (int i = 0; i < 9; i++) r.v[i] = a.v[i] + b.v[i]; return r; }
template <class M> LHD m29<M> m29_sub(const m29<M>& a, const m29<M>& b) { m29<M> r;
// ... 107 lines not shown
    const int bit = 29 * k - 5, i = bit >> 5, s = bit & 31;
    const uint64_t two = (uint64_t)w[i] | ((i + 1 < 8) ? ((uint64_t)w[i + 1] << 32) : 0);
    r.v[k] = (int32_t)((uint32_t)(two >> s) & M29_MASK);
  }
  return r;
}
template <class M> LHD void m29_pack_words(const m29<M>& a, uint32_t* out) {
#pragma unroll
  for (int w = 0; w < 8; w++) {
    const int k0 = (32 * w) / 29, s = 32 * w - 29 * k0;
    uint64_t acc = (uint64_t)(uint32_t)a.v[k0] >> s;
    int have = 29 - s;
    if (k0 + 1 < 9) { acc |= (uint64_t)(uint32_t)a.v[k0 + 1] << have; have += 29; }
    if (have < 32 && k0 + 2 < 9) acc |= (uint64_t)(uint32_t)a.v[k0 + 2] << have;
    out[w] = (uint32_t)acc;
  }
}

template <class M> struct m29_acc { int64_t h[17]; };
template <class M> LHD m29_acc<M> m29_acc_zero() { m29_acc<M> r;
#pragma unroll
  for (int k = 0; k < 17; k++) r.h[k] = 0; return r; }
template <class M> LHD void m29_mul_acc(m29_acc<M>& acc, const m29<M>& a, const m29<M>& b) {
#pragma unroll
  for (int i = 0; i < 9; i++)
#pragma unroll
    for (int j = 0; j < 9; j++) acc.h[i + j] += (int64_t)a.v[i] * b.v[j];
}
template <class M> LHD void m29_acc_carry(m29_acc<M>& acc) {
#pragma unroll
  for (int k = 0; k < 16; k++) { acc.h[k + 1] += acc.h[k] >> 29; acc.h[k] &= M29_MASK; }
}
template <class M> LHD m29<M> m29_from_columns(const int64_t* col) {
  int64_t l[9]; int64_t c = 0;
#pragma unroll
  for (int k = 0; k < 9; k++) { const int64_t x = col[k] + c; c = x >> 29; l[k] = x & M29_MASK; }
  m29<M> lo;
#pragma unroll
  for (int k = 0; k < 9; k++) lo.v[k] = (int32_t)l[k];
  const int32_t K522[9] = {M::K522_0, M::K522_1, M::K522_2, M::K522_3, M::K522_4, M::K522_5, M::K522_6, M::K522_7, M::K522_8};
  return m29_weak<M>(m29_add<M>(lo, m29_mul<M>(m29_from_i64<M>(c), m29_const<M>(K522))));
}
template <class M> LHD m29<M> m29_acc_reduce(const m29_acc<M>& acc) {
  int64_t h[17];
#pragma unroll
  for (int k = 0; k < 17; k++) h[k] = acc.h[k];
  m29_rows<M>(h);
  int64_t col[9];
#pragma unroll
  for (int k = 0; k < 8; k++) col[k] = h[9 + k];
  col[8] = 0;
  return m29_from_columns<M>(col);
}
template <class M> LHD m29<M> m29_reduce_columns(const int64_t* col, int shift) {
  int64_t l[9]; int64_t c = 0;
#pragma unroll
  for (int k = 0; k < 9; k++) { const int64_t x = col[k] * ((int64_t)1 << shift) + c; c = x >> 29; l[k] = x & M29_MASK; }
  m29<M> lo;
#pragma unroll
  for (int k = 0; k < 9; k++) lo.v[k] = (int32_t)l[k];
  const int32_t ONE_S[9] = {M::ONE_S_0, M::ONE_S_1, M::ONE_S_2, M::ONE_S_3, M::ONE_S_4, M::ONE_S_5, M::ONE_S_6, M::ONE_S_7, M::ONE_S_8};
  const int32_t K522[9] = {M::K522_0, M::K522_1, M::K522_2, M::K522_3, M::K522_4, M::K522_5, M::K522_6, M::K522_7, M::K522_8};
  const m29<M> a = m29_mul<M>(lo, m29_const<M>(ONE_S)), b = m29_mul<M>(m29_from_i64<M>(c), m29_const<M>(K522));
  return m29_canonical<M>(m29_add<M>(a, b));
}
```

lasso_amd/csrc/msm_kernels.cuh:

```cuda
#pragma once
#include <hip/hip_runtime.h>
#include "fq.cuh"
#include "fe29.cuh"
#include "poly_kernels.cuh"

#define MSM_BATCH 8192
#ifdef MSM_TABLE_COLMAJOR
#define MSM_IDX(w, m1, j, tn, NW, NM) ((((size_t)(j)) * (NW) + (w)) * (NM) + (m1))
#define MSM_COL_BASE(tab, j0, NW, NM) ((tab) + (size_t)(j0) * (NW) * (NM))
#else
#define MSM_IDX(w, m1, j, tn, NW, NM) ((((size_t)(w)) * (NM) + (m1)) * (tn) + (j))
#define MSM_COL_BASE(tab, j0, NW, NM) ((tab) + (j0))
#endif

__global__ void k_precompute_table(const fq_t* __restrict__ aff, size_t n, niels29* __restrict__ table) {
  size_t j = blockIdx.x * (size_t)blockDim.x + threadIdx.x;
  if (j >= n) return;
#ifdef LASSO_BN254
  niels29 e = niels_from_affine(aff[2 * j], aff[2 * j + 1]);
  table[j] = e;
  for (int w = 1; w < MSM_WINDOWS; w++) {
    pt29 P = pt_madd(pt_identity(), e);
    for (int k = 0; k < 4; k++) P = pt_dbl(P);
    const fe29 zi = fe_inv_chain(P.Z);
// ... 387 lines not shown
  __syncthreads();
  for (uint32_t off = 1; off < MSM_THREADS; off <<= 1) {
    pt29 v; const bool a = t + off < MSM_THREADS;
    if (a) v = pts[t + off];
    __syncthreads();
    if (a) pts[t] = pt_add(pts[t], v, d2);
    __syncthreads();
  }
  if (t == 0) pts[0] = pt_identity();
  __syncthreads();
  msm_coop_tree(pts, st, MSM_THREADS, d2);
  pt29 W = pt_identity();
  if (t == 0) W = pts[0];
  __syncthreads();
  pts[t] = T;
  __syncthreads();
  msm_coop_tree(pts, st, MSM_THREADS, d2);
  pt29 V = pt_identity();
  if (t == 0) V = pt_add(pts[0], pt_dbl(pt_dbl(pt_dbl(W))), d2);
  __syncthreads();
  pt29 top = pt_identity();
  for (uint32_t c = t; c < n_cols; c += MSM_THREADS) {
    const uint32_t v = vtop[r * n_cols + c];
    if (v) { const niels29 e = top_table[c]; for (uint32_t i = 0; i < v; i++) top = pt_madd(top, e); }
  }
  pts[t] = top;
  __syncthreads();
  msm_coop_tree(pts, st, MSM_THREADS, d2);
  if (t == 0) out[r] = pt_add(V, pts[0], d2);
}

#define MSM8_MULTS 255
__global__ void __launch_bounds__(64) k_precompute_tab8(const niels29* __restrict__ table, size_t n, uint32_t w8, niels29* __restrict__ tab8, uint32_t nm = MSM8_MULTS) {
  const size_t j = blockIdx.x * (size_t)blockDim.x + threadIdx.x;
  if (j >= n) return;
  w8 += blockIdx.y;
  const uint32_t wy = blockIdx.y, nwin = gridDim.y;
  const niels29 b = table[(size_t)(2 * w8) * n + j];
  const fe29 d2 = fe_d2();
  tab8[MSM_IDX(wy, 0, j, n, nwin, nm)] = b;
  pt29 P = pt_madd(pt_identity(), b);
  for (uint32_t m0 = 2; m0 <= nm; m0 += 16) {
    pt29 q[16]; fe29 pre[16];
    const uint32_t cnt = nm + 1 - m0 < 16 ? nm + 1 - m0 : 16;
    for (uint32_t c = 0; c < cnt; c++) { P = pt_madd(P, b); q[c] = P; pre[c] = c ? fe_mul(pre[c - 1], P.Z) : P.Z; }
    fe29 inv = fe_inv_chain(pre[cnt - 1]);
    for (uint32_t c = cnt; c-- > 0;) {
      const fe29 zi = c ? fe_mul(inv, pre[c - 1]) : inv;
      if (c) inv = fe_mul(inv, q[c].Z);
      tab8[MSM_IDX(wy, m0 + c - 1, j, n, nwin, nm)] = niels_from_xy29(fe_mul(q[c].X, zi), fe_mul(q[c].Y, zi), d2);
    }
  }
}
__global__ void __launch_bounds__(MSM_THREADS) k_msm_rows8(const uint32_t* __restrict__ scal, size_t row_words, uint32_t n_cols, uint32_t cols_per_chunk, uint32_t W8,
                                                            const niels29* __restrict__ tab8_0, const niels29* __restrict__ tab8_1, size_t tn, pt29* __restrict__ out, uint32_t* digit_count) {
  __shared__ pt29 pts[MSM_THREADS];
  __shared__ fe29 st[MSM_ST_ROWS][4];
  const fe29 d2 = fe_d2();
  const uint32_t t = threadIdx.x;
  const uint32_t* row = scal + (size_t)blockIdx.y * row_words;
  const uint32_t c0 = blockIdx.x * cols_per_chunk;
  uint32_t c1 = c0 + cols_per_chunk; if (c1 > n_cols) c1 = n_cols;
  pt29 B = pt_identity();
  niels29 cur; bool have = false; uint32_t nadds = 0;
  for (uint32_t c = c0 + t; c < c1; c += MSM_THREADS) {
    const uint32_t v = row[c];
    for (uint32_t w = 0; w < W8; w++) {
      const uint32_t d = (v >> (8 * w)) & 255u;
      nadds += d != 0;
      const niels29 nxt = (w ? tab8_1 : tab8_0)[d ? MSM_IDX(0, d - 1, c, tn, 1, MSM8_MULTS) : 0];
      if (have) B = pt_madd(B, cur);
      cur = nxt; have = d != 0;
    }
  }
  if (have) B = pt_madd(B, cur);
  msm_count_adds(digit_count, nadds);
  pts[t] = B;
  __syncthreads();
  msm_coop_tree(pts, st, MSM_THREADS, d2);
  if (t == 0) out[(size_t)blockIdx.y * gridDim.x + blockIdx.x] = pts[0];
}

__global__ void __launch_bounds__(MSM_THREADS) k_msm_rows8w(const uint32_t* __restrict__ scal, size_t row_words, uint32_t n_cols, uint32_t W8, const niels29* __restrict__ tab8_0,
                                                             const niels29* __restrict__ tab8_1, size_t tn, pt29* __restrict__ out, uint32_t rows, uint32_t* digit_count, uint32_t rpw) {
  __shared__ pt29 pts[MSM_THREADS];
  const fe29 d2 = fe_d2();
  const uint32_t t = threadIdx.x, wave = t >> 6, lane = t & 63u;
  pt29* mine = pts + 64 * wave;
  uint32_t nadds = 0;
  for (uint32_t k = 0; k < rpw; k++) {
    const uint32_t r = (blockIdx.x * (MSM_THREADS / 64) + wave) * rpw + k;
    if (r >= rows) break;
    pt29 B = pt_identity();
    const uint32_t* row = scal + (size_t)r * row_words;
    niels29 cur; bool have = false;
    uint32_t v_next = lane < n_cols ? row[lane] : 0u;
    for (uint32_t c = lane; c < n_cols; c += 64) {
      const uint32_t v = v_next;
      v_next = c + 64 < n_cols ? row[c + 64] : 0u;
      for (uint32_t w = 0; w < W8; w++) {
        const uint32_t d = (v >> (8 * w)) & 255u;
        nadds += d != 0;
        const niels29 nxt = (w ? tab8_1 : tab8_0)[d ? MSM_IDX(0, d - 1, c, tn, 1, MSM8_MULTS) : 0];
        if (have) B = pt_madd(B, cur);
        cur = nxt; have = d != 0;
      }
    }
    if (have) B = pt_madd(B, cur);
    mine[lane] = B;
    for (uint32_t s2 = 32; s2 > 0; s2 >>= 1) {
      __builtin_amdgcn_fence(__ATOMIC_RELEASE, "wavefront"); __builtin_amdgcn_wave_barrier(); __builtin_amdgcn_fence(__ATOMIC_ACQUIRE, "wavefront");
      if (lane < s2) { const pt29 x = pt_add(mine[lane], mine[lane + s2], d2); mine[lane] = x; }
    }
    if (lane == 0) out[r] = mine[0];
    __builtin_amdgcn_fence(__ATOMIC_RELEASE, "wavefront"); __builtin_amdgcn_wave_barrier(); __builtin_amdgcn_fence(__ATOMIC_ACQUIRE, "wavefront");
  }
  msm_count_adds(digit_count, nadds);
}

#define MSM_DIRECT_MAX_COLS 160
template <int WB> struct MsmD {
  static constexpr uint32_t WINDOWS = msm_direct_windows(WB), LOGW = WB == 4 ? 6u : 5u, MULTS = 1u << (WB - 1), DMASK = (1u << WB) - 1u, PER_WORD = 32u / WB;
  static constexpr uint32_t BIAS = WB == 4 ? 0x88888888u : 0x80808080u;
};
template <int WB>
__device__ __forceinline__ void msm_recode(const uint32_t* s, uint32_t* dst) {
  uint64_t carry = 0;
#pragma unroll
  for (int k = 0; k < 8; k++) { const uint64_t x = (uint64_t)s[k] + MsmD<WB>::BIAS + carry; dst[k] = (uint32_t)x; carry = x >> 32; }
}
struct MsmLeft { niels29 e; uint32_t valid = 0, rem = 0; };
#ifndef LASSO_BN254
#define MSM_LEFT_MAX 64u
__device__ __forceinline__ void msm_coop_leftover(pt29* pts, fe29 (*st)[4], fe29 (*ln)[3], uint32_t* lval, const MsmLeft& L) {
  if (!L.rem) return;
  const uint32_t t = threadIdx.x, c = t & 3u, g = t >> 2;
  if (t < L.rem) { ln[t][0] = L.e.ypx; ln[t][1] = L.e.ymx; ln[t][2] = L.e.t2d; lval[t] = L.valid; }
  __syncthreads();
  const bool act = g < L.rem && lval[g] != 0;
  if (act) st[g][c] = pt_coop4_madd_stage1(pts[g], &ln[g][0], c);
  tree_wave_sync();
  if (act) reinterpret_cast<fe29*>(&pts[g])[c] = pt_coop4_stage2p(&st[g][0], c);
  __syncthreads();
}
#endif
template <int WB>
__device__ __forceinline__ pt29 msm_direct_accumulate(const uint32_t* sb, uint32_t col0, uint32_t it0, uint32_t it1, const MsmColMap& cm, uint32_t row, const niels29* __restrict__ mult, size_t tn,
                                                      uint32_t* digit_count = nullptr, const uint32_t* phys = nullptr, MsmLeft* left = nullptr) {
  typedef MsmD<WB> D;
  const uint32_t t = threadIdx.x;
  pt29 B = pt_identity();
  niels29 cur; bool have = false; uint32_t nadds = 0;
#ifndef LASSO_BN254
  if (left) {
    const uint32_t span = it1 - it0, rem = span % MSM_THREADS;
    if (rem != 0 && rem <= MSM_LEFT_MAX && span > MSM_THREADS) {
      left->rem = rem; it1 -= rem;
      const uint32_t it = it1 + t;
      bool valid = t < rem; int32_t d = 0; uint32_t c = 0, w = 0;
      if (valid) { c = it >> D::LOGW; w = it & (D::WINDOWS - 1u); d = (int32_t)((sb[(c - col0) * 8 + w / D::PER_WORD] >> (WB * (w % D::PER_WORD))) & D::DMASK) - (int32_t)D::MULTS; valid = d != 0; }
      const uint32_t m = d < 0 ? (uint32_t)(-d) : (uint32_t)d;
      const size_t idx = valid ? MSM_IDX(w, m - 1, (phys ? phys[c - col0] : msm_phys_col(cm, row, c)), tn, D::WINDOWS, D::MULTS) : 0;
      if (t < rem) left->e = niels_cond_neg(mult[idx], d < 0);
      left->valid = valid ? 1u : 0u; nadds += valid;
    }
  }
#endif
  for (uint32_t base = it0; base < it1; base += MSM_THREADS) {
    const uint32_t it = base + t;
    bool valid = it < it1; int32_t d = 0; uint32_t c = 0, w = 0;
// ... 392 lines not shown
```

lasso_amd/csrc/poly_kernels.cuh:

```cuda
#pragma once
#include <hip/hip_runtime.h>
#include "fr.cuh"
#include "fr29.cuh"
#include "handoff_device.cuh"
#include "launch_plan.cuh"

#ifndef LASSO_MAX_PTRS
#define LASSO_MAX_PTRS 136
#endif
#define LASSO_MAX_ALPHA 32

struct PtrTable { const fr_t* p[LASSO_MAX_PTRS]; };
struct MutPtrTable { fr_t* p[LASSO_MAX_PTRS]; };
struct PtrTable8 { const fr_t* p[8]; };
struct MutPtrTable8 { fr_t* p[8]; };
struct StrategyDev { int kind; uint32_t c, log_m, log_r, alpha; };
struct WeightTable { fr_t w[LASSO_MAX_ALPHA]; };

struct RedScratch { int32_t rows[LASSO_BLOCK * 27]; int64_t strips[8 * 27]; int64_t cols[27]; };
template <int NV>
__device__ __forceinline__ void block_columns(const fr29* vals, RedScratch& S) {
  const uint32_t t = threadIdx.x;
  __syncthreads();
#pragma unroll
  for (int v = 0; v < NV; v++)
#pragma unroll
    for (int k = 0; k < 9; k++) S.rows[t * 27 + v * 9 + k] = vals[v].v[k];
  __syncthreads();
  if (t < 8 * 27) {
    const uint32_t j = t % 27, g = t / 27;
    int64_t s = 0;
    if (j < NV * 9) {
#pragma unroll 8
      for (uint32_t r = 0; r < 32; r++) s += S.rows[(g * 32 + r) * 27 + j];
    }
    S.strips[g * 27 + j] = s;
  }
  __syncthreads();
  if (t < 27) {
    int64_t s = 0;
#pragma unroll
    for (int g = 0; g < 8; g++) s += S.strips[g * 27 + t];
    S.cols[t] = s;
  }
  __syncthreads();
}
__device__ __forceinline__ fr_t columns_to_fr(const RedScratch& S, int v, int shift) {
  int64_t c[9];
#pragma unroll
  for (int k = 0; k < 9; k++) c[k] = S.cols[v * 9 + k];
  return fr29_pack(fr29_reduce_columns(c, shift));
}
__device__ __forceinline__ void acc_add(fr29& acc, const fr29& t, uint32_t& count) {
  acc = fr29_weak(fr29_add(acc, t));
  if ((++count & 127u) == 0) acc = fr29_mul(acc, fr29_one_s());
}
// ... 1005 lines not shown
}

__global__ void __launch_bounds__(LASSO_BLOCK) k_multi_dot(PtrTable polys, uint32_t nx, uint32_t ny, const fr_t* __restrict__ w, size_t n, fr_t* __restrict__ partials) {
  __shared__ RedScratch R;
  const CubicGrid g = cubic_grid(nx, ny);
  const fr_t* __restrict__ z = polys.p[g.by];
  fr29_acc wa = fr29_acc_zero(); uint32_t cnt = 0;
  for (size_t i = g.bx * (size_t)blockDim.x + threadIdx.x; i < n; i += (size_t)nx * blockDim.x) {
    fr29_mul_acc(wa, fr29_unpack_u(z[i]), fr29_unpack_s(w[i]));
    if (++cnt == 3) { fr29_acc_carry(wa); cnt = 0; }
  }
  fr29_acc_carry(wa);
  fr29 acc[1] = {fr29_acc_reduce(wa)};
  store_block_partials<1>(acc, 1, partials + (size_t)g.by * nx + g.bx, 0, R);
}

struct RTable { fr_t r[32]; };
__global__ void k_eq_small(RTable R, uint32_t ell, fr_t scale, fr_t* __restrict__ out) {
  size_t x = blockIdx.x * (size_t)blockDim.x + threadIdx.x;
  if (x >= ((size_t)1 << ell)) return;
  fr29 p = fr29_unpack_u(scale);
  const fr29 one_s = fr29_one_s();
  for (uint32_t j = 0; j < ell; j++) { const bool bit = (x >> (ell - 1 - j)) & 1; const fr29 rs = fr29_unpack_s(R.r[j]); p = fr29_mul(bit ? rs : fr29_sub(one_s, rs), p); }
  out[x] = fr29_store(p);
}
struct RTable16 { fr_t r[16]; };
__global__ void k_eq_small2(RTable16 Rh, uint32_t hi_bits, fr_t scale, fr_t* __restrict__ hi, uint32_t hi_blocks, RTable16 Rl, uint32_t lo_bits, fr_t* __restrict__ lo) {
  const bool is_lo = blockIdx.x >= hi_blocks;
  const uint32_t ell = is_lo ? lo_bits : hi_bits;
  const size_t x = (blockIdx.x - (is_lo ? hi_blocks : 0u)) * (size_t)blockDim.x + threadIdx.x;
  if (x >= ((size_t)1 << ell)) return;
  fr29 p = is_lo ? fr29_unpack_u(fr_one()) : fr29_unpack_u(scale);
  const fr29 one_s = fr29_one_s();
  if (is_lo) { for (uint32_t j = 0; j < ell; j++) { const bool bit = (x >> (ell - 1 - j)) & 1; const fr29 rs = fr29_unpack_s(Rl.r[j]); p = fr29_mul(bit ? rs : fr29_sub(one_s, rs), p); } lo[x] = fr29_store(p); }
  else { for (uint32_t j = 0; j < ell; j++) { const bool bit = (x >> (ell - 1 - j)) & 1; const fr29 rs = fr29_unpack_s(Rh.r[j]); p = fr29_mul(bit ? rs : fr29_sub(one_s, rs), p); } hi[x] = fr29_store(p); }
}
__global__ void k_eq_small2_mem(const uint32_t* __restrict__ gp, uint32_t seq, uint32_t hi_bits, fr_t* __restrict__ hi, uint32_t hi_blocks, uint32_t lo_bits, fr_t* __restrict__ lo) {
  if (!gate_point_ok(gp, seq)) return;
  const bool is_lo = blockIdx.x >= hi_blocks;
  const uint32_t ell = is_lo ? lo_bits : hi_bits, j0 = is_lo ? hi_bits : 0u;
  const size_t x = (blockIdx.x - (is_lo ? hi_blocks : 0u)) * (size_t)blockDim.x + threadIdx.x;
  if (x >= ((size_t)1 << ell)) return;
  fr29 p = is_lo ? fr29_unpack_u(fr_one()) : fr29_unpack_u(gate_point_fr(gp, hi_bits + lo_bits));
  const fr29 one_s = fr29_one_s();
  for (uint32_t j = 0; j < ell; j++) { const bool bit = (x >> (ell - 1 - j)) & 1; const fr29 rs = fr29_unpack_s(gate_point_fr(gp, j0 + j)); p = fr29_mul(bit ? rs : fr29_sub(one_s, rs), p); }
  (is_lo ? lo : hi)[x] = fr29_store(p);
}
__global__ void __launch_bounds__(LASSO_BLOCK) k_eq_outer(const fr_t* __restrict__ hi, const fr_t* __restrict__ lo, uint32_t lo_bits, size_t n, fr_t* __restrict__ out, const uint32_t* __restrict__ gp = nullptr, uint32_t seq = 0) {
  if (gp != nullptr && !gate_point_ok(gp, seq)) return;
  const size_t mask = ((size_t)1 << lo_bits) - 1;
  for (size_t x = blockIdx.x * (size_t)blockDim.x + threadIdx.x; x < n; x += (size_t)gridDim.x * blockDim.x) out[x] = fr29_store(fr29_mul(fr29_unpack_u(hi[x >> lo_bits]), fr29_unpack_s(lo[x & mask])));
}

__global__ void __launch_bounds__(LASSO_BLOCK) k_gp_layer(const fr_t* __restrict__ in, size_t half, fr_t* __restrict__ out) {
  for (size_t i = blockIdx.x * (size_t)blockDim.x + threadIdx.x; i < half; i += (size_t)gridDim.x * blockDim.x) out[i] = fr29_store(fr29_mul(fr29_unpack_u(in[i]), fr29_unpack_s(in[i + half])));
}
__global__ void __launch_bounds__(LASSO_BLOCK) k_gp_layer2(const fr_t* __restrict__ in, size_t q, fr_t* __restrict__ o1, fr_t* __restrict__ o2) {
  for (size_t i = blockIdx.x * (size_t)blockDim.x + threadIdx.x; i < q; i += (size_t)gridDim.x * blockDim.x) {
    const fr_t a = fr29_store(fr29_mul(fr29_unpack_u(in[i]), fr29_unpack_s(in[i + 2 * q])));
    const fr_t b = fr29_store(fr29_mul(fr29_unpack_u(in[i + q]), fr29_unpack_s(in[i + 3 * q])));
    o1[i] = a; o1[i + q] = b;
    o2[i] = fr29_store(fr29_mul(fr29_unpack_u(a), fr29_unpack_s(b)));
  }
}
__global__ void k_gp_tail(fr_t* __restrict__ tree, size_t len) {
  fr_t* in = tree;
  while (len > 2) {
    size_t half = len / 2; fr_t* out = in + len;
    for (size_t i = threadIdx.x; i < half; i += blockDim.x) out[i] = fr29_store(fr29_mul(fr29_unpack_u(in[i]), fr29_unpack_s(in[i + half])));
    __threadfence_block();
    __syncthreads();
    in = out; len = half;
  }
}

__global__ void __launch_bounds__(LASSO_BLOCK) k_fingerprint_ops(const fr_t* __restrict__ table, const uint32_t* __restrict__ dim, const fr_t* __restrict__ read, size_t s,
                                                                  fr_t gamma, fr_t gamma2, fr_t tau, fr_t* __restrict__ out_r, fr_t* __restrict__ out_w) {
  const fr29 gs = fr29_unpack_s(gamma), g2s = fr29_unpack_s(gamma2), g2u = fr29_unpack_u(gamma2), tu = fr29_unpack_u(tau), r2s = fr29_r2s();
  for (size_t i = blockIdx.x * (size_t)blockDim.x + threadIdx.x; i < s; i += (size_t)gridDim.x * blockDim.x) {
    const uint32_t a = dim[i];
    fr29 h = fr29_add(fr29_mul(fr29_unpack_u(read[i]), g2s), fr29_mul(fr29_unpack_u(table[a]), gs));
    h = fr29_canonical(fr29_sub(fr29_add(h, fr29_mul(fr29_from_u64_int(a), r2s)), tu));
    out_r[i] = fr29_pack(h);
    out_w[i] = fr29_store(fr29_add(h, g2u));
  }
}
template <bool RU32>
__global__ void __launch_bounds__(LASSO_BLOCK) k_fingerprint_ops_l1(const fr_t* __restrict__ table, const uint32_t* __restrict__ dim, const void* __restrict__ read_any, size_t s,
                                                                     fr_t gamma, fr_t gamma2, fr_t tau, fr_t* __restrict__ out_r, fr_t* __restrict__ out_w, fr_t* __restrict__ l1_r, fr_t* __restrict__ l1_w,
                                                                     uint32_t store_leaves) {
  const fr29 gs = fr29_unpack_s(gamma), g2s = fr29_unpack_s(gamma2), g2u = fr29_unpack_u(gamma2), tu = fr29_unpack_u(tau), r2s = fr29_r2s();
  const fr29 g2r = fr29_mul(g2s, r2s);
  const fr_t* __restrict__ read = reinterpret_cast<const fr_t*>(read_any); const uint32_t* __restrict__ read32 = reinterpret_cast<const uint32_t*>(read_any);
  const size_t half = s / 2;
  for (size_t i = blockIdx.x * (size_t)blockDim.x + threadIdx.x; i < half; i += (size_t)gridDim.x * blockDim.x) {
    fr_t lr[2], lw[2];
#pragma unroll
    for (int e = 0; e < 2; e++) {
      const size_t k = i + e * half;
      const uint32_t a = dim[k];
      fr29 h = fr29_add(RU32 ? fr29_mul(fr29_from_u64_int(read32[k]), g2r) : fr29_mul(fr29_unpack_u(read[k]), g2s), fr29_mul(fr29_unpack_u(table[a]), gs));
      h = fr29_canonical(fr29_sub(fr29_add(h, fr29_mul(fr29_from_u64_int(a), r2s)), tu));
      lr[e] = fr29_pack(h); lw[e] = fr29_store(fr29_add(h, g2u));
      if (store_leaves) { out_r[k] = lr[e]; out_w[k] = lw[e]; }
    }
    l1_r[i] = fr29_store(fr29_mul(fr29_unpack_u(lr[0]), fr29_unpack_s(lr[1])));
    l1_w[i] = fr29_store(fr29_mul(fr29_unpack_u(lw[0]), fr29_unpack_s(lw[1])));
  }
}
template <bool RU32>
__global__ void __launch_bounds__(LASSO_BLOCK) k_fingerprint_ops_strips(const fr_t* __restrict__ table, const uint32_t* __restrict__ dim, const void* __restrict__ read_any, size_t s,
                                                                         fr_t gamma, fr_t gamma2, fr_t tau, uint32_t nstrips, size_t stride, size_t i0, size_t cs,
                                                                         fr_t* __restrict__ out_r, fr_t* __restrict__ out_w) {
  const fr29 gs = fr29_unpack_s(gamma), g2s = fr29_unpack_s(gamma2), g2u = fr29_unpack_u(gamma2), tu = fr29_unpack_u(tau), r2s = fr29_r2s();
  const fr29 g2r = fr29_mul(g2s, r2s);
  const fr_t* __restrict__ read = reinterpret_cast<const fr_t*>(read_any); const uint32_t* __restrict__ read32 = reinterpret_cast<const uint32_t*>(read_any);
  const size_t total = 2 * (size_t)nstrips * cs;
  for (size_t j = blockIdx.x * (size_t)blockDim.x + threadIdx.x; j < total; j += (size_t)gridDim.x * blockDim.x) {
    const size_t strip = j / cs, i = j - strip * cs, arr = strip / nstrips, t = strip - arr * nstrips;
    const size_t k = arr * (s / 2) + t * stride + i0 + i;
    const uint32_t a = dim[k];
    fr29 h = fr29_add(RU32 ? fr29_mul(fr29_from_u64_int(read32[k]), g2r) : fr29_mul(fr29_unpack_u(read[k]), g2s), fr29_mul(fr29_unpack_u(table[a]), gs));
    h = fr29_canonical(fr29_sub(fr29_add(h, fr29_mul(fr29_from_u64_int(a), r2s)), tu));
    out_r[j] = fr29_pack(h);
    out_w[j] = fr29_store(fr29_add(h, g2u));
  }
}
__global__ void __launch_bounds__(LASSO_BLOCK) k_fingerprint_mem(const fr_t* __restrict__ table, const fr_t* __restrict__ fin, size_t m, uint32_t world, uint32_t rank, fr_t gamma, fr_t gamma2, fr_t tau,
                                                                  fr_t* __restrict__ out_i, fr_t* __restrict__ out_f) {
  const fr29 gs = fr29_unpack_s(gamma), g2s = fr29_unpack_s(gamma2), tu = fr29_unpack_u(tau), r2s = fr29_r2s();
  for (size_t i = blockIdx.x * (size_t)blockDim.x + threadIdx.x; i < m; i += (size_t)gridDim.x * blockDim.x) {
    const size_t a = i * world + rank;
    const fr29 h = fr29_canonical(fr29_sub(fr29_add(fr29_mul(fr29_unpack_u(table[a]), gs), fr29_mul(fr29_from_u64_int(a), r2s)), tu));
    out_i[i] = fr29_pack(h);
    out_f[i] = fr29_store(fr29_add(h, fr29_mul(fr29_unpack_u(fin[i]), g2s)));
  }
}

__global__ void __launch_bounds__(LASSO_BLOCK) k_from_u32(const uint32_t* __restrict__ src, size_t n, fr_t* __restrict__ dst) {
  const fr29 r2s = fr29_r2s();
  for (size_t i = blockIdx.x * (size_t)blockDim.x + threadIdx.x; i < n; i += (size_t)gridDim.x * blockDim.x) dst[i] = fr29_store(fr29_mul(fr29_from_u64_int(src[i]), r2s));
}
__global__ void __launch_bounds__(LASSO_BLOCK) k_gather(const fr_t* __restrict__ table, const uint32_t* __restrict__ idx, size_t n, fr_t* __restrict__ out) {
  for (size_t i = blockIdx.x * (size_t)blockDim.x + threadIdx.x; i < n; i += (size_t)gridDim.x * blockDim.x) out[i] = table[idx[i]];
}
__global__ void k_read_heads(PtrTable polys, uint32_t k, fr_t* __restrict__ out) {
  uint32_t i = blockIdx.x * blockDim.x + threadIdx.x;
  if (i < k) out[i] = polys.p[i][0];
}
__global__ void k_read_runs(PtrTable polys, uint32_t k, uint32_t count, fr_t* __restrict__ out) {
  const uint32_t e = blockIdx.x * blockDim.x + threadIdx.x;
  if (e < k * count) out[e] = polys.p[e / count][e % count];
}
__device__ __forceinline__ fr_t fr29_to_integer(const fr29& u) { fr29 k32 = fr29_zero(); k32.v[0] = 32; return fr29_store(fr29_mul(u, k32)); }

__global__ void __launch_bounds__(LASSO_BLOCK) k_matvec_left(const fr_t* __restrict__ Z, const fr_t* __restrict__ Lv, size_t l_size, size_t r_size, size_t rows_per_chunk,
                                                              fr_t* __restrict__ partials) {
  size_t col = blockIdx.x * (size_t)blockDim.x + threadIdx.x;
  if (col >= r_size) return;
  size_t j0 = (size_t)blockIdx.y * rows_per_chunk, j1 = j0 + rows_per_chunk; if (j1 > l_size) j1 = l_size;
// ... 16 lines not shown
```

lasso_amd/device.py:

```python
import ctypes as C
import os

import numpy as np

from . import _abi
from .custom import strategy_ptr

HERE = os.path.dirname(os.path.abspath(__file__))


class LassoError(RuntimeError):
    pass


def load_device_library(path=None, curve="curve25519"):
    path = path or os.path.join(HERE, "liblasso_hip_bn254.so" if curve == "bn254" else "liblasso_hip.so")
    if not os.path.exists(path):
        raise LassoError(f"{path} is missing: build it with `python -c 'import __graft_entry__ as g; g.build()'` (no CPU fallback exists)")
    lib = C.CDLL(path)
    _abi.declare(lib)
    return lib


def _vp(a):
# ... 169 lines not shown
        out = np.empty((degree + 1, 4), dtype=np.uint64)
        self._chk(self.lib.lasso_sumcheck_combine_round(self.ctx, strategy_ptr(strategy), self._ptrs(ptrs), C.c_void_p(d_eq), n, degree, _vp(out)))
        return out

    def lt_prescale(self, strategy, ptrs, n, src=None):
        self._chk(self.lib.lasso_lt_prescale(self.ctx, strategy_ptr(strategy), None if src is None else self._ptrs(src), self._ptrs(ptrs), n))

    def sumcheck_combine_round_lt_scaled(self, strategy, ptrs, d_eq, n, degree):
        out = np.empty((degree + 1, 4), dtype=np.uint64)
        self._chk(self.lib.lasso_sumcheck_combine_round_lt_scaled(self.ctx, strategy_ptr(strategy), self._ptrs(ptrs), C.c_void_p(d_eq), n, degree, _vp(out)))
        return out

    def sumcheck_linear_eqw_round_u32(self, u32_ptrs, d_e, n):
        out = np.empty((3 * len(u32_ptrs), 4), dtype=np.uint64)
        self._chk(self.lib.lasso_sumcheck_linear_eqw_round_u32(self.ctx, self._ptrs(u32_ptrs), len(u32_ptrs), C.c_void_p(d_e), n, _vp(out)))
        return out.reshape(len(u32_ptrs), 3, 4)[:, :2].copy()

    def sumcheck_linear_eqw_round_fused_from_u32(self, u32_ptrs, ptrs, d_e, n, r):
        r = np.ascontiguousarray(r, dtype=np.uint64)
        out = np.empty((3 * len(ptrs), 4), dtype=np.uint64)
        self._chk(self.lib.lasso_sumcheck_linear_eqw_round_fused_from_u32(self.ctx, self._ptrs(u32_ptrs), self._ptrs(ptrs), len(ptrs), C.c_void_p(d_e), n, _vp(r), _vp(out)))
        return out.reshape(len(ptrs), 3, 4)[:, :2].copy()

    def sumcheck_combine_round_lt_u32(self, strategy, u32_ptrs, d_eq, n, degree):
        out = np.empty((degree + 1, 4), dtype=np.uint64)
        self._chk(self.lib.lasso_sumcheck_combine_round_lt_u32(self.ctx, strategy_ptr(strategy), self._ptrs(u32_ptrs), C.c_void_p(d_eq), n, degree, _vp(out)))
        return out

    def combine_claim(self, strategy, ptrs, d_eq, n):
        out = np.empty((1, 4), dtype=np.uint64)
        self._chk(self.lib.lasso_combine_claim(self.ctx, strategy_ptr(strategy), self._ptrs(ptrs), C.c_void_p(d_eq), n, _vp(out)))
        return out

    def multi_dot(self, ptrs, d_w, n):
        out = np.empty((len(ptrs), 4), dtype=np.uint64)
        self._chk(self.lib.lasso_multi_dot(self.ctx, self._ptrs(ptrs), len(ptrs), C.c_void_p(d_w), n, _vp(out)))
        return out

    def read_heads(self, ptrs):
        out = np.empty((len(ptrs), 4), dtype=np.uint64)
        self._chk(self.lib.lasso_read_heads(self.ctx, self._ptrs(ptrs), len(ptrs), _vp(out)))
        return out

    def gp_build(self, d_tree, n):
        self._chk(self.lib.lasso_gp_build(self.ctx, C.c_void_p(d_tree), n))

    def fingerprint_ops(self, d_table, d_dim, d_read, s, gamma, tau, d_ro, d_wo):
        g = np.ascontiguousarray(gamma, dtype=np.uint64); t = np.ascontiguousarray(tau, dtype=np.uint64)
        self._chk(self.lib.lasso_fingerprint_ops(self.ctx, C.c_void_p(d_table), C.c_void_p(d_dim), C.c_void_p(d_read), s, _vp(g), _vp(t), C.c_void_p(d_ro), C.c_void_p(d_wo)))

    def fingerprint_ops_gp(self, d_table, d_dim, d_read, s, gamma, tau, d_tree_r, d_tree_w):
        g = np.ascontiguousarray(gamma, dtype=np.uint64); t = np.ascontiguousarray(tau, dtype=np.uint64)
        self._chk(self.lib.lasso_fingerprint_ops_gp(self.ctx, C.c_void_p(d_table), C.c_void_p(d_dim), C.c_void_p(d_read), s, _vp(g), _vp(t), C.c_void_p(d_tree_r), C.c_void_p(d_tree_w)))

    def fingerprint_ops_gp_upper(self, d_table, d_dim, d_read, s, gamma, tau, d_upper_r, d_upper_w, read_u32=False):
        g = np.ascontiguousarray(gamma, dtype=np.uint64); t = np.ascontiguousarray(tau, dtype=np.uint64)
        fn = self.lib.lasso_fingerprint_ops_gp_upper_u32 if read_u32 else self.lib.lasso_fingerprint_ops_gp_upper
        self._chk(fn(self.ctx, C.c_void_p(d_table), C.c_void_p(d_dim), C.c_void_p(d_read), s, _vp(g), _vp(t), C.c_void_p(d_upper_r), C.c_void_p(d_upper_w)))

    def fingerprint_ops_strips(self, d_table, d_dim, d_read, s, gamma, tau, nstrips, i0, cs, d_out_r, d_out_w, read_u32=False):
        g = np.ascontiguousarray(gamma, dtype=np.uint64); t = np.ascontiguousarray(tau, dtype=np.uint64)
        fn = self.lib.lasso_fingerprint_ops_strips_u32 if read_u32 else self.lib.lasso_fingerprint_ops_strips
        self._chk(fn(self.ctx, C.c_void_p(d_table), C.c_void_p(d_dim), C.c_void_p(d_read), s, _vp(g), _vp(t), nstrips, i0, cs, C.c_void_p(d_out_r), C.c_void_p(d_out_w)))

    def fingerprint_mem(self, d_table, d_final, m, gamma, tau, d_io, d_fo):
        g = np.ascontiguousarray(gamma, dtype=np.uint64); t = np.ascontiguousarray(tau, dtype=np.uint64)
        self._chk(self.lib.lasso_fingerprint_mem(self.ctx, C.c_void_p(d_table), C.c_void_p(d_final), m, _vp(g), _vp(t), C.c_void_p(d_io), C.c_void_p(d_fo)))

    def matvec_left(self, d_z, L, l_size, r_size):
        L = np.ascontiguousarray(L, dtype=np.uint64)
        out = np.empty((r_size, 4), dtype=np.uint64)
        self._chk(self.lib.lasso_matvec_left(self.ctx, C.c_void_p(d_z), _vp(L), l_size, r_size, _vp(out)))
        return out

    def bases_create(self, affine):
        affine = np.ascontiguousarray(affine, dtype=np.uint64).reshape(-1, 8)
        b = C.c_void_p()
        self._chk(self.lib.lasso_bases_create(self.ctx, _vp(affine), affine.shape[0], C.byref(b)))
        return b.value

    def points_decompress(self, wire):
        if not hasattr(self, "_wire"):
            try:
                _abi.declare_wire(self.lib)
            except AttributeError:
                raise LassoError("this device library does not export lasso_points_decompress (include/lasso_hip_wire.h)")
            self._wire = True
        w = np.ascontiguousarray(np.frombuffer(wire, dtype=np.uint8) if isinstance(wire, (bytes, bytearray, memoryview)) else np.asarray(wire, dtype=np.uint8)).reshape(-1)
        if w.size % 32:
            raise LassoError("points_decompress: the input is not a whole number of 32-byte encodings")
        n = w.size // 32
        aff = np.zeros((n, 8), dtype=np.uint64); canon = np.zeros((n, 32), dtype=np.uint8); status = np.zeros(n, dtype=np.uint8)
        self._chk(self.lib.lasso_points_decompress(self.ctx, _vp(w), n, _vp(aff), _vp(canon), _vp(status)))
        return aff, canon, status

    def bases_destroy(self, b):
        self.lib.lasso_bases_destroy(self.ctx, C.c_void_p(b))

    def hyrax_commit(self, d_z, l_size, r_size, bases):
        out = np.empty((l_size, 16), dtype=np.uint64)
        self._chk(self.lib.lasso_hyrax_commit(self.ctx, C.c_void_p(d_z), l_size, r_size, C.c_void_p(bases), _vp(out)))
        return out

    def hyrax_commit_compressed(self, d_z, l_size, r_size, bases):
        out = np.empty((l_size, 32), dtype=np.uint8)
        self._chk(self.lib.lasso_hyrax_commit_compressed(self.ctx, C.c_void_p(d_z), l_size, r_size, C.c_void_p(bases), _vp(out)))
# ... 119 lines not shown
```

lasso_amd/host/prover.hpp:

```cpp
#pragma once
#include <array>
#include <functional>
#include <map>
#include <memory>
#include <string>
#include <vector>
#include "field_host.hpp"
#include "field52.hpp"
#include "switches.hpp"
#include "sumcheck_phase.hpp"
#include "hashes.hpp"
#include "../../include/lasso_prover.h"
#include "../csrc/operand_layout.cuh"
#include "../../include/lasso_custom_check.h"

#include <chrono>
#include <cstdio>
#include <cstdlib>

namespace lasso {

struct Trace {
  static bool on() { return sw::trace() == 1; }
  static bool mem() { return sw::trace() == 3; }
  const char* name; lasso_ctx* ctx; std::chrono::steady_clock::time_point t0; static int& depth() { static thread_local int d = 0; return d; }
  uint64_t w0 = 0; double wus0 = 0; uint64_t live0 = 0;
  Trace(const char* n, lasso_ctx* c) : name(n), ctx(c) {
    if (on()) { t0 = std::chrono::steady_clock::now(); depth()++; if (ctx) lasso_wait_stats(ctx, &w0, &wus0, 0); }
    if (mem() && ctx) { uint64_t pk = 0; lasso_mem_stats(ctx, &live0, &pk, 1); depth()++; }
  }
  ~Trace() {
    if (mem() && ctx) {
      uint64_t live = 0, pk = 0; lasso_mem_stats(ctx, &live, &pk, 1); depth()--;
      fprintf(stderr, "[mem] %*s%s: live at entry %.2f GB, peak inside %.2f GB, live at exit %.2f GB\n", 2 * depth(), "", name, live0 / 1e9, pk / 1e9, live / 1e9);
    }
    if (!on()) return;
    if (ctx) lasso_sync(ctx);
    depth()--;
    double ms = std::chrono::duration<double, std::milli>(std::chrono::steady_clock::now() - t0).count();
    uint64_t w1 = 0; double wus1 = 0; if (ctx) lasso_wait_stats(ctx, &w1, &wus1, 0);
    fprintf(stderr, "[trace] %*s%s: time.busy=%.3fms (device hand-offs %llu, host spinning %.3fms)\n", 2 * depth(), "", name, ms, (unsigned long long)(w1 - w0), (wus1 - wus0) * 1e-3);
  }
};

struct HostClock {
  static bool on() { return sw::trace() == 2; }
  static std::map<std::string, double>& buckets() { static thread_local std::map<std::string, double> b; return b; }
  const char* name; std::chrono::steady_clock::time_point t0;
  explicit HostClock(const char* n) : name(n) { if (on()) t0 = std::chrono::steady_clock::now(); }
  ~HostClock() { if (on()) buckets()[name] += std::chrono::duration<double, std::milli>(std::chrono::steady_clock::now() - t0).count(); }
  static void dump() { if (!on()) return; for (auto& kv : buckets()) fprintf(stderr, "[host] %-28s %.3f ms\n", kv.first.c_str(), kv.second); buckets().clear(); }
};
struct Error : std::runtime_error { using std::runtime_error::runtime_error; };
#define LASSO_REQUIRE(c) do { if (!(c)) throw Error(std::string("lasso prover: requirement failed: ") + #c); } while (0)

#define LASSO_HOST_TOPS_MAX_PTRS 128
inline size_t next_pow2(size_t n) { size_t p = 1; while (p < n) p <<= 1; return p; }
inline bool is_pow2(size_t n) { return n && !(n & (n - 1)); }
inline size_t ceil_log2(size_t n) { size_t k = 0; while (((size_t)1 << k) < n) k++; return k; }

typedef int32_t (*lasso_allgather_fn)(void* user, const void* send, void* recv, size_t bytes);
struct Comm {
  size_t rank = 0, world = 1; lasso_allgather_fn fn = nullptr; void* user = nullptr;
  bool shared_device = false;
  bool sharded() const { return world > 1; }
  size_t log_world() const { size_t k = 0; while (((size_t)1 << k) < world) k++; return k; }
  void allgather(const void* send, void* recv, size_t bytes) const {
// ... 481 lines not shown
  std::vector<lasso_point> rows(l_size);
  std::vector<Pt> pts(l_size);
  {
    const size_t P = d.comm.world; LASSO_REQUIRE(gens.bases_slab && r_size >= P);
    d.chk(lasso_hyrax_commit(d.ctx, d_Z, l_size, r_size / P, gens.bases_slab, rows.data()), "lasso_hyrax_commit");
    std::vector<lasso_point> all(l_size * P);
    d.comm.allgather(rows.data(), all.data(), l_size * sizeof(lasso_point));
    for (size_t i = 0; i < l_size; i++) { Pt acc = Pt::from_abi(all[i]); for (size_t g = 1; g < P; g++) acc = acc + Pt::from_abi(all[g * l_size + i]); pts[i] = acc; }
  }
  PolyCommitment c; c.rows = l_size; compress_batch(pts, c.compressed); return c;
}
inline PolyCommitment hyrax_commit(const Dev& d, const lasso_fr* d_Z, size_t num_vars, const PolyCommitmentGens& gens, const uint32_t* d_u32 = nullptr, uint32_t max_u32 = 0) {
  return hyrax_commit_rows(d, d_Z, (size_t)1 << (num_vars / 2), (size_t)1 << (num_vars - num_vars / 2), gens, d_u32, max_u32);
}
inline void append_poly_commitment(ProofTranscript& t, const char* label, const PolyCommitment& c) {
  t.append_message(label, "poly_commitment_begin");
  for (size_t i = 0; i < c.rows; i++) t.append_point_bytes("poly_commitment_share", &c.compressed[32 * i]);
  t.append_message(label, "poly_commitment_end");
}

struct SparsePolynomialCommitment { PolyCommitment l_variate_polys_commitment, log_m_variate_polys_commitment; size_t s, log_m, m; };
struct DensifiedRepresentation {
  const Dev* dev; size_t C, s, log_m, m;
  size_t s_loc, m_loc;
  std::vector<DBufU32> dim_u32;
  DBuf combined_l_variate_polys, combined_log_m_variate_polys;
  size_t nv_l, nv_m;
  bool compact = false;
  std::vector<DBufU32> read_u32; std::vector<uint32_t> read_max;
  const lasso_fr* dim(size_t i) const { LASSO_REQUIRE(!compact); return combined_l_variate_polys.p + i * s_loc; }
  const lasso_fr* read(size_t i) const { LASSO_REQUIRE(!compact); return combined_l_variate_polys.p + (C + i) * s_loc; }
  const uint32_t* block_u32(size_t b) const { return b < C ? dim_u32[b].p : read_u32[b - C].p; }
  uint32_t block_max(size_t b) const { return b < C ? (uint32_t)(m - 1) : read_max[b - C]; }
  void lift_block(size_t b, lasso_fr* d_tmp) const { dev->chk(lasso_fr_from_u32(dev->ctx, block_u32(b), s_loc, d_tmp), "lasso_fr_from_u32"); }
  const lasso_fr* final_(size_t i) const { return combined_log_m_variate_polys.p + i * m_loc; }

  template <class MakeSource>
  static std::unique_ptr<DensifiedRepresentation> densify_with(const Dev& d, const char* span, size_t n_lookups, size_t C, size_t log_m, MakeSource&& make_source) {
    Trace tr_all(span, d.ctx);
    auto D = std::make_unique<DensifiedRepresentation>();
    D->dev = &d; D->C = C; D->s = next_pow2(n_lookups); D->log_m = log_m; D->m = (size_t)1 << log_m;
    const size_t s = D->s, m = D->m, P = d.comm.world;
    if (d.comm.sharded() && (s < 2 * P || m < 2 * P)) throw Error("slab sharding needs at least 2 lookups and 2 table entries per rank");
    D->s_loc = s / P; D->m_loc = m / P;
    size_t n_l = next_pow2(2 * C * s), n_m = next_pow2(C) * m;
    D->nv_l = ceil_log2(n_l); D->nv_m = ceil_log2(n_m);
    if (d.comm.sharded() && (((size_t)1 << (D->nv_m - D->nv_m / 2)) < P || ((size_t)1 << (D->nv_l - D->nv_l / 2)) < P)) throw Error("slab sharding needs every Hyrax matrix to have at least one column per rank");
    D->compact = d.capacity && sw::capacity_compact() && D->s_loc >= sw::leafless_min() && s >= ((size_t)1 << (D->nv_l - D->nv_l / 2));
    D->combined_log_m_variate_polys = DBuf(d, n_m / P);
    if (!D->compact) D->combined_l_variate_polys = DBuf(d, n_l / P);
    if (!D->compact && n_l > 2 * C * s) d.chk(lasso_zero(d.ctx, D->combined_l_variate_polys.p + 2 * C * D->s_loc, (n_l - 2 * C * s) / P * sizeof(lasso_fr)), "lasso_zero");
    if (n_m > C * m) d.chk(lasso_zero(d.ctx, D->combined_log_m_variate_polys.p + C * D->m_loc, (n_m - C * m) / P * sizeof(lasso_fr)), "lasso_zero");
    auto densify_dim = make_source();
    DBuf tmp_dim, tmp_read; if (D->compact) { tmp_dim = DBuf(d, D->s_loc); tmp_read = DBuf(d, D->s_loc); }
    for (size_t i = 0; i < C; i++) {
      DBufU32 d_access(d, D->s_loc);
      lasso_fr* dim_out = D->compact ? tmp_dim.p : D->combined_l_variate_polys.p + i * D->s_loc;
      lasso_fr* read_out = D->compact ? tmp_read.p : D->combined_l_variate_polys.p + (C + i) * D->s_loc;
      densify_dim(i, s, d_access.p, dim_out, read_out, D->combined_log_m_variate_polys.p + i * D->m_loc);
      D->dim_u32.push_back(std::move(d_access));
      if (D->compact) {
        DBufU32 r32(d, D->s_loc); uint32_t mx = 0;
        d.chk(lasso_fr_to_u32(d.ctx, tmp_read.p, D->s_loc, r32.p, &mx), "lasso_fr_to_u32");
        D->read_u32.push_back(std::move(r32)); D->read_max.push_back(mx);
      }
    }
    if (D->compact) { tmp_dim.release(); tmp_read.release(); }
    if (d.capacity) (void)lasso_trim(d.ctx);
    return D;
  }
  static std::unique_ptr<DensifiedRepresentation> from_lookup_indices(const Dev& d, const uint64_t* indices, size_t n_lookups, size_t C, size_t log_m) {
    return densify_with(d, "DensifiedRepresentation.from_lookup_indices", n_lookups, C, log_m, [&] {
      auto d_idx = std::make_shared<DBufU64>(d, indices, n_lookups * C);
      return [&d, d_idx, n_lookups, C, log_m](size_t i, size_t s, uint32_t* access, lasso_fr* dim_out, lasso_fr* read_out, lasso_fr* final_out) {
        d.chk(lasso_densify_dim_slab(d.ctx, d_idx->p, n_lookups, C, i, s, (uint32_t)log_m, (uint32_t)d.comm.world, (uint32_t)d.comm.rank, access, dim_out, read_out, final_out), "lasso_densify_dim");
      };
    });
  }
  typedef int32_t (*OperandsEntry)(lasso_ctx*, const uint64_t*, const uint64_t*, size_t, const lasso_operand_layout*, size_t, size_t, size_t, uint32_t, uint32_t, uint32_t, uint32_t*, lasso_fr*, lasso_fr*, lasso_fr*);
  static std::unique_ptr<DensifiedRepresentation> from_operands(const Dev& d, OperandsEntry entry, const lasso_operand_layout& layout, const uint64_t* x, const uint64_t* y, bool on_device, size_t n_lookups,
                                                                size_t C, size_t log_m, uint64_t* dims_counter) {
    return densify_with(d, "DensifiedRepresentation.from_operands", n_lookups, C, log_m, [&] {
      std::shared_ptr<DBufU64> ux, uy;
      if (!on_device) { ux = std::make_shared<DBufU64>(d, x, n_lookups); if (y) uy = std::make_shared<DBufU64>(d, y, n_lookups); }
      const uint64_t* px = on_device ? x : ux->p; const uint64_t* py = !y ? nullptr : on_device ? y : uy->p;
      return [&d, ux, uy, px, py, entry, layout, n_lookups, C, log_m, dims_counter](size_t i, size_t s, uint32_t* access, lasso_fr* dim_out, lasso_fr* read_out, lasso_fr* final_out) {
        d.chk(entry(d.ctx, px, py, n_lookups, &layout, C, i, s, (uint32_t)log_m, (uint32_t)d.comm.world, (uint32_t)d.comm.rank, access, dim_out, read_out, final_out), "lasso_densify_dim_operands");
        if (dims_counter) ++*dims_counter;
      };
    });
  }
  SparsePolynomialCommitment commit(const SparsePolyCommitmentGens& gens) const {
    Trace tr_all("DensifiedRepresentation.commit", dev->ctx);
    SparsePolynomialCommitment c;
    if (!compact) c.l_variate_polys_commitment = hyrax_commit(*dev, combined_l_variate_polys.p, nv_l, gens.gens_combined_l_variate);
    else {
      const size_t L = (size_t)1 << (nv_l / 2), R = (size_t)1 << (nv_l - nv_l / 2), rows_per = s / R;
      PolyCommitment& pc = c.l_variate_polys_commitment; pc.rows = L; pc.compressed.reserve(32 * L);
      DBuf tmp(*dev, s_loc);
      for (size_t b = 0; b < 2 * C; b++) {
        PolyCommitment part;
        if (!dev->comm.sharded()) part = hyrax_commit_rows(*dev, nullptr, rows_per, R, gens.gens_combined_l_variate, block_u32(b), block_max(b));
        else { lift_block(b, tmp.p); part = hyrax_commit_rows(*dev, tmp.p, rows_per, R, gens.gens_combined_l_variate); }
        pc.compressed.insert(pc.compressed.end(), part.compressed.begin(), part.compressed.end());
      }
      if (2 * C * rows_per < L) {
        dev->chk(lasso_zero(dev->ctx, tmp.p, (R / dev->comm.world) * sizeof(lasso_fr)), "lasso_zero");
        PolyCommitment zero_row = hyrax_commit_rows(*dev, tmp.p, 1, R, gens.gens_combined_l_variate);
        for (size_t r = 2 * C * rows_per; r < L; r++) pc.compressed.insert(pc.compressed.end(), zero_row.compressed.begin(), zero_row.compressed.end());
      }
      tmp.release();
    }
// ... 773 lines not shown
    ScVec ch = t.challenge_vector(challenge_label, ceil_log2(evals.size()));
    evals.resize(next_pow2(evals.size()), Sc::zero());
    size_t len = evals.size();
    for (size_t i = ch.size(); i-- > 0;) { len /= 2; for (size_t k = 0; k < len; k++) evals[k] = evals[2 * k] + ch[i] * (evals[2 * k + 1] - evals[2 * k]); }
    LASSO_REQUIRE(len == 1);
    Sc joint = evals[0];
    ScVec r_joint = ch; r_joint.insert(r_joint.end(), r.begin(), r.end());
    t.append_scalar(joint_label, joint);
    if (prep && prep->ready) { LASSO_REQUIRE(prep->k == ch.size() && prep->k + r.size() == num_vars); return poly_eval_prove_prepped(*prep, ch, joint, g); }
    return poly_eval_prove(d_poly, num_vars, r_joint, joint, g);
  }

  void prove(const ScVec& r) {
    Trace tr_all("SparsePoly.prove", d.ctx);
    t.append_protocol_name("Lasso SparsePolynomialEvaluationProof");
    LASSO_REQUIRE(r.size() == ceil_log2(s));
    std::unique_ptr<Trace> sp(new Trace("Subtables.new", d.ctx));
    std::vector<DBufU32> tables_u32; const bool ints = S.integer_tables(); const uint32_t table_max = ints ? S.max_table_value() : 0;
    if (S.custom()) for (size_t i = 0; i < S.num_subtables(); i++) {
      tables.emplace_back(d, m);
      if (ints) { tables_u32.emplace_back(d, m); d.chk(lasso_upload(d.ctx, tables_u32.back().p, S.cabi.tables_u32[i], m * sizeof(uint32_t)), "lasso_upload"); }
      else d.chk(lasso_upload(d.ctx, tables.back().p, S.cabi.tables_fr[i], m * sizeof(lasso_fr)), "lasso_upload");
    } else
    if (ints) for (size_t i = 0; i < S.num_subtables(); i++) {
      tables_u32.emplace_back(d, m); tables.emplace_back(d, m);
      d.chk(lasso_materialize_subtable_u32(d.ctx, &S.abi, (uint32_t)i, tables_u32.back().p), "lasso_materialize_subtable_u32");
    } else {
      const std::vector<ScVec> tau = S.spark_point();
      for (size_t i = 0; i < S.num_subtables(); i++) {
        tables.emplace_back(d, m);
        std::vector<lasso_fr> tv; for (auto& x : tau[i]) tv.push_back(x.abi());
        d.chk(lasso_eq_evals(d.ctx, tv.data(), (uint32_t)tv.size(), tables.back().p), "lasso_eq_evals");
      }
    }
    if (!sw::side_stream() || P != 1) {} else d.chk(lasso_sync(d.ctx), "lasso_sync");
    size_t n_E = next_pow2(alpha * s); nv_derefs = ceil_log2(n_E);
    combined_E = DBuf(d, n_E / P);
    DBuf eq(d, s_loc);
    const bool side_new = P == 1 && !!sw::side_stream() && ints;
    lasso_ctx* fc = side_new ? d.side() : d.ctx;
    auto fchk = [&](int32_t rc, const char* what) { if (side_new) d.chk_side(rc, what); else d.chk(rc, what); };
    auto field_side = [&] {
      if (ints) for (size_t i = 0; i < tables.size(); i++) fchk(lasso_fr_from_u32(fc, tables_u32[i].p, m, tables[i].p), "lasso_fr_from_u32");
      if (n_E > alpha * s) fchk(lasso_zero(fc, combined_E.p + alpha * s_loc, (n_E - alpha * s) / P * sizeof(lasso_fr)), "lasso_zero");
      for (size_t i = 0; i < alpha; i++)
        fchk(lasso_gather(fc, tables[S.memory_to_subtable_index(i)].p, dense.dim_u32[S.memory_to_dimension_index(i)].p, s_loc, combined_E.p + i * s_loc), "lasso_gather");
    };
    ProofWriter W;
    PolyCommitment comm_derefs;
    DBufU32 E_u32;
    if (P == 1 && ints) {
      E_u32 = DBufU32(d, n_E);
      if (n_E > alpha * s) d.chk(lasso_zero(d.ctx, E_u32.p + alpha * s, (n_E - alpha * s) * sizeof(uint32_t)), "lasso_zero");
      for (size_t i = 0; i < alpha; i++)
        d.chk(lasso_gather_u32(d.ctx, tables_u32[S.memory_to_subtable_index(i)].p, dense.dim_u32[S.memory_to_dimension_index(i)].p, s, E_u32.p + i * s), "lasso_gather_u32");
      if (side_new) {
        field_side();
        std::vector<lasso_fr> rr; for (auto& x : r) rr.push_back(x.abi());
        d.chk_side(lasso_eq_evals(fc, rr.data(), (uint32_t)rr.size(), eq.p), "lasso_eq_evals");
      } else field_side();
      sp.reset(), sp.reset(new Trace("Subtables.commit", d.ctx));
      comm_derefs = hyrax_commit(d, combined_E.p, nv_derefs, gens.gens_derefs, E_u32.p, table_max);
      if (side_new) side_sync();
    } else {
      field_side();
      sp.reset(), sp.reset(new Trace("Subtables.commit", d.ctx));
      comm_derefs = hyrax_commit(d, combined_E.p, nv_derefs, gens.gens_derefs);
    }
    tables_u32.clear();
    if (!side_new) eq_evals_local(r, eq.p);
    std::vector<const lasso_fr*> Eptr; for (size_t i = 0; i < alpha; i++) Eptr.push_back(E(i));
    std::vector<lasso_fr> claim_abi(1);
    d.chk(lasso_defer_next(d.ctx), "lasso_defer_next");
    d.chk(lasso_combine_claim(d.ctx, S.abi_ptr(), Eptr.data(), eq.p, s_loc, claim_abi.data()), "lasso_combine_claim");
    t.append_message("subtable_evals_commitment", "begin_subtable_evals_commitment");
    append_poly_commitment(t, "comm_poly_row_col_ops_val", comm_derefs);
    t.append_message("subtable_evals_commitment", "end_subtable_evals_commitment");
    W.pts_vec(comm_derefs.compressed);
    sp.reset(), sp.reset(new Trace("Subtables.compute_sumcheck_claim", d.ctx));
    d.chk(lasso_result_wait(d.ctx, claim_abi.data(), 1), "lasso_result_wait");
    d.comm.sum(claim_abi);
    Sc claimed_eval = Sc::from_abi(claim_abi[0]);
    t.append_scalar("claim_eval_scalar_product", claimed_eval);
    ScVec r_z;
    sp.reset(), sp.reset(new Trace("Sumcheck.prove", d.ctx));
    ScVec sumcheck_heads;
    {
      const bool no_clone = S.linear();
      const size_t wl = no_clone && s_loc >= 4 ? s_loc / 2 : s_loc;
      const size_t per_piece = d.capacity ? s_loc / wl : alpha, n_pieces = (alpha + per_piece - 1) / per_piece;
      std::vector<DBuf> work; for (size_t i = 0; i < n_pieces; i++) work.emplace_back(d, d.capacity ? s_loc : alpha * wl);
      std::vector<lasso_fr*> polys; for (size_t i = 0; i < alpha; i++) polys.push_back(work[i / per_piece].p + (i % per_piece) * wl); polys.push_back(eq.p);
      std::vector<const uint32_t*> Eu32; if (P == 1 && (no_clone || table_max <= 1) && E_u32.p && sw::sumcheck_u32() && ceil_log2(s) > 0) for (size_t i = 0; i < alpha; i++) Eu32.push_back(E_u32.p + i * s);
      SumcheckProof sp = prove_arbitrary(ceil_log2(s), s_loc, polys, S.sumcheck_poly_degree(), r, r_z, &sumcheck_heads, &Eptr, Eu32.empty() ? nullptr : &Eu32);
      sp.write(W);
    }
    E_u32 = DBufU32();
    if (d.capacity) eq.reset();
    W.sc(claimed_eval);
    sp.reset(), sp.reset(new Trace("CombinedEval.prove", d.ctx));
    DBuf chis(d, s_loc);
    auto evaluate_at = [&](const std::vector<const lasso_fr*>& polys, const ScVec& point, size_t n_loc, DBuf& chi) {
      eq_evals_local(point, chi.p);
      std::vector<lasso_fr> out(polys.size());
      d.chk(lasso_multi_dot(d.ctx, polys.data(), (uint32_t)polys.size(), chi.p, n_loc, out.data()), "lasso_multi_dot");
      d.comm.sum(out);
      ScVec v; for (auto& o : out) v.push_back(Sc::from_abi(o)); return v;
    };
    ScVec eval_derefs = sumcheck_heads.size() == alpha && ceil_log2(s) > 0 ? sumcheck_heads : evaluate_at(Eptr, r_z, s_loc, chis);
    W.sc_arr(eval_derefs);
    t.append_protocol_name("Lasso CombinedTableEvalProof");
    joint_open("evals_ops_val", "challenge_combine_n_to_one", "joint_claim_eval", eval_derefs, true, combined_E.p, nv_derefs, r_z, gens.gens_derefs).write(W);
    sp.reset(), sp.reset(new Trace("MemoryChecking.prove", d.ctx));
    ScVec r_hash = t.challenge_vector("challenge_r_hash", 2);
    memory_checking_prove(r_hash[0], r_hash[1], Eptr, chis, W);
    sp.reset();
    proof_bytes.swap(W.b);
    HostClock::dump();
  }

  void memory_checking_prove(const Sc& gamma, const Sc& tau, const std::vector<const lasso_fr*>& Eptr, DBuf& chis, ProofWriter& W) {
    t.append_protocol_name("Lasso MemoryCheckingProof");
    lasso_fr g = gamma.abi(), ta = tau.abi();
    std::unique_ptr<Trace> sp(new Trace("Subtables.to_grand_products", d.ctx));
    std::vector<DBuf> t_init, t_read, t_write, t_final;
    const bool leafless = (d.capacity || dense.compact) && s_loc >= sw::leafless_min();
    if (d.capacity) { chis.reset(); d.trim_keep((leafless ? s_loc : 2 * s_loc) * sizeof(lasso_fr), 2 * alpha + (leafless && alpha == 4 ? 1 : 0)); }
    LeafLayer leaf; leaf.gamma = g; leaf.tau = ta; leaf.n_loc = s_loc;
    for (size_t i = 0; i < alpha; i++) {
      size_t j = S.memory_to_dimension_index(i); const lasso_fr* table = tables[S.memory_to_subtable_index(i)].p;
      DBuf ti(d, 2 * m_loc), tf(d, 2 * m_loc), tr(d, leafless ? s_loc : 2 * s_loc), tw(d, leafless ? s_loc : 2 * s_loc);
      d.chk(lasso_fingerprint_mem_slab(d.ctx, table, dense.final_(j), m_loc, (uint32_t)P, (uint32_t)d.comm.rank, &g, &ta, ti.p, tf.p), "lasso_fingerprint_mem");
      d.chk(lasso_gp_build(d.ctx, ti.p, m_loc), "lasso_gp_build"); d.chk(lasso_gp_build(d.ctx, tf.p, m_loc), "lasso_gp_build");
      if (leafless && dense.compact) {
        d.chk(lasso_fingerprint_ops_gp_upper_u32(d.ctx, table, dense.dim_u32[j].p, dense.read_u32[j].p, s_loc, &g, &ta, tr.p, tw.p), "lasso_fingerprint_ops_gp_upper_u32");
        leaf.mems.push_back({table, dense.dim_u32[j].p, nullptr, dense.read_u32[j].p});
      } else if (leafless) {
        d.chk(lasso_fingerprint_ops_gp_upper(d.ctx, table, dense.dim_u32[j].p, dense.read(j), s_loc, &g, &ta, tr.p, tw.p), "lasso_fingerprint_ops_gp_upper");
        leaf.mems.push_back({table, dense.dim_u32[j].p, dense.read(j)});
      } else if (s_loc >= 4) {
        d.chk(lasso_fingerprint_ops_gp(d.ctx, table, dense.dim_u32[j].p, dense.read(j), s_loc, &g, &ta, tr.p, tw.p), "lasso_fingerprint_ops_gp");
      } else {
        d.chk(lasso_fingerprint_ops(d.ctx, table, dense.dim_u32[j].p, dense.read(j), s_loc, &g, &ta, tr.p, tw.p), "lasso_fingerprint_ops");
        d.chk(lasso_gp_build(d.ctx, tr.p, s_loc), "lasso_gp_build"); d.chk(lasso_gp_build(d.ctx, tw.p, s_loc), "lasso_gp_build");
      }
      t_init.push_back(std::move(ti)); t_final.push_back(std::move(tf)); t_read.push_back(std::move(tr)); t_write.push_back(std::move(tw));
    }
    if (Trace::mem()) d.dump_live("trees built");
    sp.reset(), sp.reset(new Trace("ProductLayer.prove", d.ctx));
    t.append_protocol_name("Lasso ProductLayerProof");
    std::vector<DBuf> tops_store;
    auto root_and_top = [&](const DBuf& tree, size_t n_loc, lasso_fr*& top_out, size_t missing = 0) {
      lasso_fr two[2]; const lasso_fr* last[2] = {tree.p + (2 * n_loc - 4 - missing), tree.p + (2 * n_loc - 3 - missing)};
      d.chk(lasso_read_heads(d.ctx, last, 2, two), "lasso_read_heads");
      Sc local = Sc::from_abi(two[0]) * Sc::from_abi(two[1]);
      top_out = nullptr;
      if (P == 1) return local;
      std::vector<lasso_fr> mine{local.abi()}, all(P);
      d.comm.allgather(mine.data(), all.data(), sizeof(lasso_fr));
      tops_store.emplace_back(d, 2 * P);
      d.chk(lasso_upload(d.ctx, tops_store.back().p, all.data(), P * sizeof(lasso_fr)), "lasso_upload");
      if (P > 2) d.chk(lasso_gp_build(d.ctx, tops_store.back().p, P), "lasso_gp_build");
      top_out = tops_store.back().p;
      Sc prod = Sc::one(); for (auto& x : all) prod *= Sc::from_abi(x);
      return prod;
    };
    const bool slab_host_tops = P > 1 && sw::slab_host_tops();
    auto root_and_host_top = [&](const DBuf& tree, size_t n_loc, size_t missing, HostTops& T, size_t c, size_t kk) {
      lasso_fr two[2]; const lasso_fr* last[2] = {tree.p + (2 * n_loc - 4 - missing), tree.p + (2 * n_loc - 3 - missing)};
      d.chk(lasso_read_heads(d.ctx, last, 2, two), "lasso_read_heads");
      const Sc local = Sc::from_abi(two[0]) * Sc::from_abi(two[1]);
      std::vector<lasso_fr> mine{local.abi()}, all(P);
      d.comm.allgather(mine.data(), all.data(), sizeof(lasso_fr));
      if (T.run.empty()) { T.len = P; T.run.assign(kk, ScVec()); }
      ScVec& run = T.run[c]; run.clear(); run.reserve(2 * P - 2);
      for (auto& x : all) run.push_back(Sc::from_abi(x));
      for (size_t len = P, off = 0; len > 2; off += len, len /= 2) for (size_t i = 0; i < len / 2; i++) run.push_back(run[off + i] * run[off + i + len / 2]);
      return run[run.size() - 2] * run[run.size() - 1];
    };
    ScVec roots_rw, roots_if;
    std::vector<lasso_fr*> rw, inf, rw_top, inf_top;
    HostTops tops_rw, tops_if;
    auto read_tops = [&](const std::vector<DBuf>& ta, const std::vector<DBuf>& tb, size_t n_leaves, size_t missing, HostTops& out) {
      const size_t kk = 2 * ta.size(), m0 = host_m_stop(kk);
      if (P != 1 || !host_tail_budget() || kk > LASSO_HOST_TOPS_MAX_PTRS) return;
      size_t hl = 2 * m0; if (hl > n_leaves) hl = n_leaves;
      if (missing && hl >= n_leaves) return;
      if (hl < 2) return;
      const size_t count = 2 * hl - 2, start = 2 * n_leaves - 2 * hl - missing;
      std::vector<const lasso_fr*> ptr; for (size_t i = 0; i < ta.size(); i++) { ptr.push_back(ta[i].p + start); ptr.push_back(tb[i].p + start); }
      std::vector<lasso_fr> flat(kk * count);
      d.chk(lasso_read_runs(d.ctx, ptr.data(), (uint32_t)kk, (uint32_t)count, flat.data()), "lasso_read_runs");
      out.len = hl; out.run.assign(kk, ScVec(count));
      for (size_t c = 0; c < kk; c++) for (size_t i = 0; i < count; i++) out.run[c][i] = Sc::from_abi(flat[c * count + i]);
    };
    read_tops(t_read, t_write, s_loc, leafless ? s_loc : 0, tops_rw);
    read_tops(t_init, t_final, m_loc, 0, tops_if);
    auto root_of = [](const HostTops& T, size_t c) { const ScVec& r = T.run[c]; return r[r.size() - 2] * r[r.size() - 1]; };
    for (size_t i = 0; i < alpha; i++) {
      lasso_fr *ti_top = nullptr, *tr_top = nullptr, *tw_top = nullptr, *tf_top = nullptr;
// ... 91 lines not shown
```

lasso_amd/host/switches.hpp:

```cpp
#pragma once
#include <cstdlib>

namespace lasso { namespace sw {
inline bool unless0(const char* e) { return !(e && e[0] == '0'); }
inline bool if1(const char* e) { return e && e[0] == '1'; }
#define LASSO_SWITCH(type, name, value) inline type name() { static const type v = (value); return v; }
LASSO_SWITCH(int, trace, [] { const char* e = getenv("LASSO_TRACE"); return e && e[0] >= '1' && e[0] <= '3' ? e[0] - '0' : 0; }())
LASSO_SWITCH(bool, capacity, if1(getenv("LASSO_CAPACITY")))
LASSO_SWITCH(bool, capacity_compact, unless0(getenv("LASSO_CAPACITY_COMPACT")))
LASSO_SWITCH(size_t, leafless_min, [] { const char* e = getenv("LASSO_LEAFLESS_MIN"); const size_t x = e ? (size_t)atoll(e) : ((size_t)1 << 16); return x < 64 ? (size_t)64 : x; }())
LASSO_SWITCH(bool, throughput_ahead, if1(getenv("LASSO_THROUGHPUT_AHEAD")))
LASSO_SWITCH(bool, side_stream, unless0(getenv("LASSO_SIDE_STREAM")))
LASSO_SWITCH(bool, slab_open, unless0(getenv("LASSO_SLAB_OPEN")))
LASSO_SWITCH(bool, eq_inline, unless0(getenv("LASSO_EQ_INLINE")))
LASSO_SWITCH(bool, cubic_tail, unless0(getenv("LASSO_CUBIC_TAIL")))
LASSO_SWITCH(bool, linear_tail, unless0(getenv("LASSO_LINEAR_TAIL")))
LASSO_SWITCH(bool, rounds_ahead, unless0(getenv("LASSO_ROUNDS_AHEAD")))
LASSO_SWITCH(bool, slab_ahead, unless0(getenv("LASSO_SLAB_AHEAD")))
LASSO_SWITCH(bool, cubic_three_sums, if1(getenv("LASSO_CUBIC_THREE_SUMS")))
LASSO_SWITCH(bool, slab_host_tail, unless0(getenv("LASSO_SLAB_HOST_TAIL")))
LASSO_SWITCH(bool, slab_host_tops, unless0(getenv("LASSO_SLAB_HOST_TOPS")))
LASSO_SWITCH(bool, sumcheck_u32, unless0(getenv("LASSO_SUMCHECK_U32")))
LASSO_SWITCH(bool, host_ifma, unless0(getenv("LASSO_HOST_IFMA")))
inline size_t host_tail(bool ifma) { static const size_t v = [&] { const char* e = getenv("LASSO_HOST_TAIL"); const long x = e ? atol(e) : (ifma ? 128 : 32); return (size_t)(x < 0 ? 0 : x > 1024 ? 1024 : x); }(); return v; }
LASSO_SWITCH(bool, verify_device_points, unless0(getenv("LASSO_VERIFY_DEVICE_POINTS")))
LASSO_SWITCH(size_t, wire_device_min, [] { const char* e = getenv("LASSO_WIRE_DEVICE_MIN"); const long long x = e ? atoll(e) : 376; return (size_t)(x < 1 ? 1 : x); }())
LASSO_SWITCH(bool, verify_msm_points, unless0(getenv("LASSO_VERIFY_MSM_POINTS")))
LASSO_SWITCH(bool, densify_operands, unless0(getenv("LASSO_DENSIFY_OPERANDS")))
inline bool slab_rccl() { return unless0(getenv("LASSO_SLAB_RCCL")); }
inline bool debug_cubic_host() { return if1(getenv("LASSO_DEBUG_CUBIC_HOST")); }
#undef LASSO_SWITCH
} }
```

Before: 1.108 billion.

## Add u32 fingerprint leaves, paired product-tree builds, and gather-fused MSM commit

Densify now also keeps integer read timestamps as u32, so memory-checking leaves can be computed from u32 tables, dims and reads with a fused two-layer fingerprint kernel instead of reading full field elements. Init and final grand-product trees (and read/write trees) are built together by paired kernels that launch once per layer for both trees. The subtable commit can gather E values inside the MSM kernels rather than first materializing them with separate gather launches. This lowers memory traffic and launch count, at the cost of extra u32 buffers held across phases and more code paths behind default-on switches.

After: 1.124 billion (median of 6 runs). 1.01x the previous value.

```diff
diff --git a/include/lasso_hip_u32.h b/include/lasso_hip_u32.h
--- /dev/null
+++ b/include/lasso_hip_u32.h
@@ -0,0 +1,21 @@
+#ifndef LASSO_HIP_U32_H
+#define LASSO_HIP_U32_H
+#include "lasso_hip.h"
+#ifdef __cplusplus
+extern "C" {
+#endif
+
+int32_t lasso_densify_keep_read_u32(lasso_ctx* ctx, uint32_t* d_read_u32);
+
+int32_t lasso_fingerprint_ops_gp_u32(lasso_ctx* ctx, const uint32_t* d_table_u32, const uint32_t* d_dim, const uint32_t* d_read_u32, size_t s, const lasso_fr* gamma,
+                                     const lasso_fr* tau, lasso_fr* d_tree_read, lasso_fr* d_tree_write);
+
+int32_t lasso_gp_build2(lasso_ctx* ctx, lasso_fr* d_tree_a, lasso_fr* d_tree_b, size_t n);
+
+int32_t lasso_hyrax_commit_compressed_gather_u32(lasso_ctx* ctx, const uint32_t* const* d_tables, const uint32_t* const* d_dims, uint32_t n_mem, size_t s, uint32_t max_value,
+                                                 size_t l_size, size_t r_size, const lasso_bases* bases, uint32_t* d_e_u32, uint8_t* out32);
+
+#ifdef __cplusplus
+}
+#endif
+#endif
diff --git a/lasso_amd/_abi.py b/lasso_amd/_abi.py
--- a/lasso_amd/_abi.py
+++ b/lasso_amd/_abi.py
@@ -177,4 +177,18 @@
     return ["lasso_densify_dim_operands"]
 
 
+def declare_u32(lib):
+    sig = {
+        "lasso_densify_keep_read_u32": (i32, [vp, vp]),
+        "lasso_fingerprint_ops_gp_u32": (i32, [vp, vp, vp, vp, sz, vp, vp, vp, vp]),
+        "lasso_gp_build2": (i32, [vp, vp, vp, sz]),
+        "lasso_hyrax_commit_compressed_gather_u32": (i32, [vp, vp, vp, u32, sz, u32, sz, sz, vp, vp, vp]),
+    }
+    for name, (res, args) in sig.items():
+        fn = getattr(lib, name)
+        fn.restype = res
+        fn.argtypes = args
+    return sorted(sig)
+
+
 HEADER_SYMBOLS = None
diff --git a/lasso_amd/build.py b/lasso_amd/build.py
--- a/lasso_amd/build.py
+++ b/lasso_amd/build.py
@@ -26,7 +26,7 @@
     suffix, flags = CURVES[curve]
     csrc = os.path.join(HERE, "csrc")
     target = os.path.join(HERE, f"liblasso_hip{suffix}.so")
-    sources = _glob(csrc, (".hip", ".cuh")) + [os.path.join(ROOT, "include", f) for f in ("lasso_hip.h", "lasso_hip_wire.h", "lasso_hip_msm.h", "lasso_hip_operands.h", "lasso_custom_check.h")]
+    sources = _glob(csrc, (".hip", ".cuh")) + [os.path.join(ROOT, "include", f) for f in ("lasso_hip.h", "lasso_hip_wire.h", "lasso_hip_msm.h", "lasso_hip_operands.h", "lasso_hip_u32.h", "lasso_custom_check.h")]
     if force or _stale(target, sources):
         extra = os.environ.get("LASSO_EXTRA_HIPCC_FLAGS", "").split()
         cmd = [HIPCC, f"--offload-arch={ARCH}", "-O3", "-std=c++17", "-fPIC", "-shared", "-Wno-unused-result", *flags, *extra,
@@ -54,7 +54,7 @@
     suffix, flags = CURVES[curve]
     hdir = os.path.join(HERE, "host")
     target = os.path.join(HERE, f"liblasso_prover{suffix}.so")
-    sources = _glob(hdir, (".cpp", ".hpp")) + _glob(os.path.join(HERE, "csrc"), (".cuh",)) + [os.path.join(ROOT, "include", f) for f in ("lasso_hip.h", "lasso_hip_wire.h", "lasso_hip_msm.h", "lasso_hip_operands.h", "lasso_prover.h", "lasso_custom_check.h")]
+    sources = _glob(hdir, (".cpp", ".hpp")) + _glob(os.path.join(HERE, "csrc"), (".cuh",)) + [os.path.join(ROOT, "include", f) for f in ("lasso_hip.h", "lasso_hip_wire.h", "lasso_hip_msm.h", "lasso_hip_operands.h", "lasso_hip_u32.h", "lasso_prover.h", "lasso_custom_check.h")]
     if not os.path.exists(os.path.join(hdir, "prover_capi.cpp")):
         return None
     dev = build_device(force=False, verbose=verbose, curve=curve)
diff --git a/lasso_amd/csrc/densify_kernels.cuh b/lasso_amd/csrc/densify_kernels.cuh
--- a/lasso_amd/csrc/densify_kernels.cuh
+++ b/lasso_amd/csrc/densify_kernels.cuh
@@ -120,13 +120,14 @@
   }
 }
 __global__ void __launch_bounds__(256) k_densify_read(const uint32_t* __restrict__ skeys, const uint32_t* __restrict__ svals, size_t s, const uint32_t* __restrict__ run_start, uint32_t world,
-                                                       uint32_t rank, fr_t* __restrict__ read_fr) {
+                                                       uint32_t rank, fr_t* __restrict__ read_fr, uint32_t* __restrict__ read_u32) {
   const fr29 r2s = fr29_r2s();
   for (size_t i = blockIdx.x * (size_t)blockDim.x + threadIdx.x; i < s; i += (size_t)gridDim.x * blockDim.x) {
     const uint32_t pos = svals[i];
     if (pos % world != rank) continue;
     const uint32_t ts = (uint32_t)i - run_start[skeys[i]];
     read_fr[pos / world] = fr29_store(fr29_mul(fr29_from_u64_int(ts), r2s));
+    if (read_u32) read_u32[pos / world] = ts;
   }
 }
 __global__ void __launch_bounds__(256) k_densify_final(const uint32_t* __restrict__ run_start, const uint32_t* __restrict__ run_end, size_t m, uint32_t world, uint32_t rank, fr_t* __restrict__ final_fr) {
diff --git a/lasso_amd/csrc/device_switches.cuh b/lasso_amd/csrc/device_switches.cuh
--- a/lasso_amd/csrc/device_switches.cuh
+++ b/lasso_amd/csrc/device_switches.cuh
@@ -21,6 +21,7 @@
 LASSO_DSWITCH(bool, layer_ahead, unless0(getenv("LASSO_LAYER_AHEAD")))
 LASSO_DSWITCH(bool, tail_q_256, [] { const char* e = getenv("LASSO_TAIL_Q"); return (e ? atol(e) : 0) == 256; }())
 LASSO_DSWITCH(bool, exp_no_leaf_store, if1(getenv("LASSO_EXP_NO_LEAF_STORE")))
+LASSO_DSWITCH(bool, gp_pair, unless0(getenv("LASSO_GP_PAIR")))
 LASSO_DSWITCH(size_t, msm_direct_max_n, [] { const char* e = getenv("LASSO_MSM_DIRECT_MAX_N"); return e ? (size_t)atoll(e) : (((size_t)1 << 17) + 64); }())
 LASSO_DSWITCH(size_t, msm_direct8_max_n, [] { if (!unless0(getenv("LASSO_MSM_DIRECT8"))) return (size_t)0; const char* e = getenv("LASSO_MSM_DIRECT8_MAX_N"); return e ? (size_t)atoll(e) : (((size_t)1 << 14) + 64); }())
 LASSO_DSWITCH(bool, msm_direct, unless0(getenv("LASSO_MSM_DIRECT")))
@@ -29,6 +30,7 @@
 LASSO_DSWITCH(bool, msm_rows8, unless0(getenv("LASSO_MSM_ROWS8")))
 LASSO_DSWITCH(bool, msm_rows8w, unless0(getenv("LASSO_MSM_ROWS8W")))
 LASSO_DSWITCH(size_t, msm_rows8w_waves, [] { const char* e = getenv("LASSO_MSM_ROWS8W_WAVES"); const long x = e ? atol(e) : 0; return (size_t)(x < 0 ? 0 : x); }())
+LASSO_DSWITCH(bool, msm_gather, unless0(getenv("LASSO_MSM_GATHER")))
 LASSO_DSWITCH(bool, msm_full8, if1(getenv("LASSO_MSM_FULL8")))
 LASSO_DSWITCH(bool, bullet_ahead, unless0(getenv("LASSO_BULLET_AHEAD")))
 LASSO_DSWITCH(bool, bullet_tail_ahead, unless0(getenv("LASSO_BULLET_TAIL_AHEAD")))
diff --git a/lasso_amd/csrc/fingerprint_leaf.cuh b/lasso_amd/csrc/fingerprint_leaf.cuh
--- /dev/null
+++ b/lasso_amd/csrc/fingerprint_leaf.cuh
@@ -0,0 +1,27 @@
+#pragma once
+#include "fr29.cuh"
+
+struct fingerprint_consts {
+  fr29 g2r, gr, r2s;
+  fr29 g2u, tu;
+};
+LHD fingerprint_consts fingerprint_consts_from(const fr_t& gamma, const fr_t& gamma2, const fr_t& tau) {
+  fingerprint_consts K;
+  K.r2s = fr29_r2s();
+  K.g2r = fr29_mul(fr29_unpack_s(gamma2), K.r2s);
+  K.gr = fr29_mul(fr29_unpack_s(gamma), K.r2s);
+  K.g2u = fr29_unpack_u(gamma2); K.tu = fr29_unpack_u(tau);
+  return K;
+}
+LHD fr29 fingerprint_leaf_int(uint32_t t, uint32_t v, uint32_t a, const fingerprint_consts& K) {
+  fr29_acc acc = fr29_acc_zero();
+  fr29_mul_acc(acc, fr29_from_u64_int(t), K.g2r);
+  fr29_mul_acc(acc, fr29_from_u64_int(v), K.gr);
+  fr29_mul_acc(acc, fr29_from_u64_int(a), K.r2s);
+  return fr29_canonical(fr29_sub(fr29_acc_reduce_small(acc), K.tu));
+}
+LHD void fingerprint_leaves_int(uint32_t t, uint32_t v, uint32_t a, const fingerprint_consts& K, fr_t& leaf_r, fr_t& leaf_w) {
+  const fr29 h = fingerprint_leaf_int(t, v, a, K);
+  leaf_r = fr29_pack(h);
+  leaf_w = fr29_store(fr29_add(h, K.g2u));
+}
diff --git a/lasso_amd/csrc/fr29.cuh b/lasso_amd/csrc/fr29.cuh
--- a/lasso_amd/csrc/fr29.cuh
+++ b/lasso_amd/csrc/fr29.cuh
@@ -90,6 +90,7 @@
 LHD void fr29_mul_acc(fr29_acc& acc, const fr29& a, const fr29& b) { m29_mul_acc(acc, a, b); }
 LHD void fr29_acc_carry(fr29_acc& acc) { m29_acc_carry(acc); }
 LHD fr29 fr29_acc_reduce(const fr29_acc& acc) { return m29_acc_reduce(acc); }
+LHD fr29 fr29_acc_reduce_small(const fr29_acc& acc) { return m29_acc_reduce_small(acc); }
 LHD fr29 fr29_semi(const fr29& a) { return m29_near(a); }
 LHD fr29 fr29_canonical(const fr29& a) { return m29_canonical(a); }
 LHD fr29 fr29_reduce_columns(const int64_t* col, int shift) { return m29_reduce_columns<FrM29>(col, shift); }
@@ -107,6 +108,7 @@
 static constexpr auto& fr29_mul_acc = m29_mul_acc<FrM29>;
 static constexpr auto& fr29_acc_carry = m29_acc_carry<FrM29>;
 static constexpr auto& fr29_acc_reduce = m29_acc_reduce<FrM29>;
+static constexpr auto& fr29_acc_reduce_small = m29_acc_reduce_small<FrM29>;
 static constexpr auto& fr29_semi = m29_near<FrM29>;
 static constexpr auto& fr29_canonical = m29_canonical<FrM29>;
 static constexpr auto& fr29_reduce_columns = m29_reduce_columns<FrM29>;
diff --git a/lasso_amd/csrc/lasso_hip.hip b/lasso_amd/csrc/lasso_hip.hip
--- a/lasso_amd/csrc/lasso_hip.hip
+++ b/lasso_amd/csrc/lasso_hip.hip
@@ -19,6 +19,7 @@
 #include "../../include/lasso_hip_msm.h"
 #include "msm_points_kernels.cuh"
 #include "../../include/lasso_hip_operands.h"
+#include "../../include/lasso_hip_u32.h"
 
 __global__ void __launch_bounds__(256) k_inner_lr(const fr_t* __restrict__ a, const fr_t* __restrict__ b, size_t half, fr_t* __restrict__ partials) {
   __shared__ RedScratch S;
@@ -56,6 +57,7 @@
   uint64_t stat_waits = 0; double stat_wait_us = 0;
   fr_t* d_big = nullptr; fr_t* h_big = nullptr; size_t big_cap = 0;
   uint32_t* d_flags = nullptr;
+  uint32_t* keep_read_u32 = nullptr;
   uint32_t* d_counters = nullptr;
   uint32_t* d_gmail = nullptr;
   uint32_t* pmail_h = nullptr; uint32_t* pmail_d = nullptr; uint32_t* d_gpoint = nullptr;
@@ -1147,6 +1149,45 @@
   }
   HIPCHK(c, hipGetLastError()); return 0;
 }
+static void gp_layers_from2(lasso_ctx* c, fr_t* ta, fr_t* tb, size_t off, size_t len) {
+  if (!dsw::gp_pair()) { gp_layers_from(c, ta + off, len); gp_layers_from(c, tb + off, len); return; }
+  while (len >= 16 * LASSO_BLOCK) {
+    const size_t q = len / 4;
+    hipLaunchKernelGGL(k_gp_layer2_pair, dim3(grid_for(q, 4096), 2), dim3(LASSO_BLOCK), 0, c->stream, ta, tb, off, q);
+    off += len + len / 2; len = q;
+  }
+  while (len > 2 * LASSO_BLOCK) {
+    const size_t half = len / 2;
+    hipLaunchKernelGGL(k_gp_layer_pair, dim3(grid_for(half, 4096), 2), dim3(LASSO_BLOCK), 0, c->stream, ta, tb, off, half);
+    off += len; len = half;
+  }
+  if (len > 2) hipLaunchKernelGGL(k_gp_tail_pair, dim3(2), dim3(LASSO_BLOCK), 0, c->stream, ta, tb, off, len);
+}
+int32_t lasso_gp_build2(lasso_ctx* c, lasso_fr* d_tree_a, lasso_fr* d_tree_b, size_t n) {
+  REQUIRE(c, d_tree_a && d_tree_b && d_tree_a != d_tree_b && n >= 2 && (n & (n - 1)) == 0);
+  ProfScope ps(c, LASSO_K_GP, 2 * 48.0 * n * 2.0);
+  gp_layers_from2(c, (fr_t*)d_tree_a, (fr_t*)d_tree_b, 0, n);
+  HIPCHK(c, hipGetLastError()); return 0;
+}
+int32_t lasso_densify_keep_read_u32(lasso_ctx* c, uint32_t* d_read_u32) {
+  REQUIRE(c, true);
+  c->keep_read_u32 = d_read_u32; return 0;
+}
+int32_t lasso_fingerprint_ops_gp_u32(lasso_ctx* c, const uint32_t* d_table_u32, const uint32_t* d_dim, const uint32_t* d_read_u32, size_t s, const lasso_fr* gamma, const lasso_fr* tau,
+                                     lasso_fr* d_tree_r, lasso_fr* d_tree_w) {
+  REQUIRE(c, d_table_u32 && d_dim && d_read_u32 && gamma && tau && d_tree_r && d_tree_w && s >= 8 && (s & (s - 1)) == 0);
+  fr_t g = to_fr(gamma), g2 = fr_sqr(g), t = to_fr(tau);
+  fr_t* tr = (fr_t*)d_tree_r; fr_t* tw = (fr_t*)d_tree_w;
+  {
+    ProfScope ps(c, LASSO_K_FINGERPRINT, (32.0 * 3 + 64.0) * s + 2 * 48.0 * s + 2 * 48.0 * (s / 2));
+    hipLaunchKernelGGL(k_fingerprint_ops_int_l2, dim3(grid_for(s / 4, 4096)), dim3(LASSO_BLOCK), 0, c->stream, d_table_u32, d_dim, d_read_u32, s, g, g2, t, tr, tw, tr + s, tw + s, tr + s + s / 2, tw + s + s / 2);
+  }
+  {
+    ProfScope ps(c, LASSO_K_GP, 2 * 48.0 * (s / 2));
+    gp_layers_from2(c, tr, tw, s + s / 2, s / 4);
+  }
+  HIPCHK(c, hipGetLastError()); return 0;
+}
 static int32_t fingerprint_gp_upper_impl(lasso_ctx* c, const lasso_fr* d_table, const uint32_t* d_dim, const void* d_read, bool read_u32, size_t s, const lasso_fr* gamma, const lasso_fr* tau,
                                          lasso_fr* d_upper_r, lasso_fr* d_upper_w) {
   REQUIRE(c, d_table && d_dim && d_read && gamma && tau && d_upper_r && d_upper_w && s >= 4 && (s & (s - 1)) == 0);
@@ -1270,6 +1311,7 @@
 }
 static int32_t densify_dim_run(lasso_ctx* c, size_t n_lookups, size_t s, uint32_t log_m, uint32_t world, uint32_t rank, lasso_fr* d_read, lasso_fr* d_final, double extract_bytes,
                                const char* bad_msg, const std::function<void(uint32_t*, uint32_t*)>& extract) {
+  uint32_t* const read_u32 = c->keep_read_u32; c->keep_read_u32 = nullptr;
   const size_t m = (size_t)1 << log_m;
   const uint32_t ntiles = (uint32_t)((s + RADIX_TILE - 1) / RADIX_TILE);
   const size_t nh = (size_t)256 * ntiles, nb = (nh + 4095) / 4096;
@@ -1291,7 +1333,7 @@
     std::swap(kA, kB); std::swap(vA, vB);
   }
   hipLaunchKernelGGL(k_densify_runs, dim3(grid_for(s, 4096)), dim3(256), 0, c->stream, (const uint32_t*)kA, s, run_start, run_end);
-  hipLaunchKernelGGL(k_densify_read, dim3(grid_for(s, 4096)), dim3(256), 0, c->stream, (const uint32_t*)kA, (const uint32_t*)vA, s, (const uint32_t*)run_start, world, rank, (fr_t*)d_read);
+  hipLaunchKernelGGL(k_densify_read, dim3(grid_for(s, 4096)), dim3(256), 0, c->stream, (const uint32_t*)kA, (const uint32_t*)vA, s, (const uint32_t*)run_start, world, rank, (fr_t*)d_read, read_u32);
   hipLaunchKernelGGL(k_densify_final, dim3(grid_for(m / world, 4096)), dim3(256), 0, c->stream, (const uint32_t*)run_start, (const uint32_t*)run_end, m, world, rank, (fr_t*)d_final);
   HIPCHK(c, hipGetLastError());
   uint32_t flags[2];
@@ -1427,8 +1469,9 @@
   if (gate_seq) return 0;
   return wait_flag(c, seq, rows * (sizeof(ed_point) / sizeof(fr_t)), (lasso_fr*)out, msm_tagged(c));
 }
+__global__ void __launch_bounds__(256) k_gather_u32(const uint32_t* __restrict__ table, const uint32_t* __restrict__ idx, size_t n, uint32_t* __restrict__ out);
 static int32_t run_msm(lasso_ctx* c, const uint8_t* d_scal, uint32_t bps, uint32_t W, size_t row_stride, size_t rows, size_t n_cols, const lasso_bases* b, uint8_t* scratch_after, lasso_point* out,
-                       uint8_t* out_compressed = nullptr, void* d_rows_out = nullptr) {
+                       uint8_t* out_compressed = nullptr, void* d_rows_out = nullptr, const MsmGather* G = nullptr) {
   const MsmShape shape = {bps, W, rows, n_cols, out_compressed != nullptr, d_rows_out != nullptr};
   const MsmSwitches sw = {dsw::msm_direct(), dsw::msm_rows8(), dsw::msm_rows8w(), dsw::msm_full8(), dsw::msm_pip(), dsw::msm_rows8w_waves(), dsw::msm_pip_min_cols(), dsw::msm_pip_scratch_mb(), dsw::msm_direct_wgs()};
   MsmHave have = {b->n, b->d_mult != nullptr, b->d_mult8 != nullptr, true, true};
@@ -1439,6 +1482,11 @@
     t8[0] = ensure_tab8(c, b, 0); t8[1] = P.W8 > 1 && t8[0] ? ensure_tab8(c, b, 1) : t8[0];
     if (!t8[1]) { have.tab8 = false; P = msm_plan(shape, have, sw); }
   } else if (P.kernel == MSM_K_PIP && ensure_pip(c, P.pip_group * P.pip_row_bytes + 256) != 0) { have.pip_scratch = false; P = msm_plan(shape, have, sw); }
+  const bool self_gather = G && dsw::msm_gather() && (P.kernel == MSM_K_ROWS8W || P.kernel == MSM_K_ROWS8);
+  if (G && !self_gather) {
+    const size_t per = (size_t)G->rows_per_mem * n_cols;
+    for (uint32_t i = 0; i < G->n_mem; i++) hipLaunchKernelGGL(k_gather_u32, dim3(grid_for(per)), dim3(256), 0, c->stream, G->table[i], G->dim[i], per, G->e_out + i * per);
+  }
   if (d_rows_out) out_compressed = (uint8_t*)d_rows_out;
   const size_t K = P.K;
   pt29* d_partial = (pt29*)scratch_after;
@@ -1449,11 +1497,15 @@
     ProfScope ps(c, LASSO_K_MSM, (double)rows * n_cols * bps, P.ref_adds, rows > MSM_SMALL_ROWS, P.adds);
     switch (P.kernel) {
       case MSM_K_ROWS8W:
-        hipLaunchKernelGGL(k_msm_rows8w, dim3((unsigned)((P.waves + MSM_THREADS / 64 - 1) / (MSM_THREADS / 64))), dim3(MSM_THREADS), 0, c->stream, (const uint32_t*)d_scal, row_stride / 4,
+        if (self_gather) hipLaunchKernelGGL(k_msm_rows8w_gather, dim3((unsigned)((P.waves + MSM_THREADS / 64 - 1) / (MSM_THREADS / 64))), dim3(MSM_THREADS), 0, c->stream, *G,
+                           (uint32_t)n_cols, P.W8, t8[0], t8[1], b->n, d_partial, (uint32_t)rows, ps.counter(), (uint32_t)P.rpw);
+        else hipLaunchKernelGGL(k_msm_rows8w, dim3((unsigned)((P.waves + MSM_THREADS / 64 - 1) / (MSM_THREADS / 64))), dim3(MSM_THREADS), 0, c->stream, (const uint32_t*)d_scal, row_stride / 4,
                            (uint32_t)n_cols, P.W8, t8[0], t8[1], b->n, d_partial, (uint32_t)rows, ps.counter(), (uint32_t)P.rpw);
         break;
       case MSM_K_ROWS8:
-        hipLaunchKernelGGL(k_msm_rows8, dim3((unsigned)K, (unsigned)rows), dim3(MSM_THREADS), 0, c->stream, (const uint32_t*)d_scal, row_stride / 4, (uint32_t)n_cols, (uint32_t)P.cols_per_chunk, P.W8,
+        if (self_gather) hipLaunchKernelGGL(k_msm_rows8_gather, dim3((unsigned)K, (unsigned)rows), dim3(MSM_THREADS), 0, c->stream, *G, (uint32_t)n_cols, (uint32_t)P.cols_per_chunk, P.W8,
+                           t8[0], t8[1], b->n, d_partial, ps.counter());
+        else hipLaunchKernelGGL(k_msm_rows8, dim3((unsigned)K, (unsigned)rows), dim3(MSM_THREADS), 0, c->stream, (const uint32_t*)d_scal, row_stride / 4, (uint32_t)n_cols, (uint32_t)P.cols_per_chunk, P.W8,
                            t8[0], t8[1], b->n, d_partial, ps.counter());
         break;
       case MSM_K_PIP: {
@@ -1548,6 +1600,18 @@
   hipLaunchKernelGGL(k_gather_u32, dim3(grid_for(n)), dim3(256), 0, c->stream, d_table, d_idx, n, d_out);
   HIPCHK(c, hipGetLastError()); return 0;
 }
+int32_t lasso_hyrax_commit_compressed_gather_u32(lasso_ctx* c, const uint32_t* const* d_tables, const uint32_t* const* d_dims, uint32_t n_mem, size_t s, uint32_t max_value, size_t l_size,
+                                                 size_t r_size, const lasso_bases* b, uint32_t* d_e_u32, uint8_t* out32) {
+  REQUIRE(c, d_tables && d_dims && d_e_u32 && out32 && b && n_mem >= 1 && n_mem <= MSM_GATHER_MEMS && l_size >= 1 && r_size >= 1 && r_size <= b->n && l_size < ((size_t)1 << 31));
+  REQUIRE(c, s >= r_size && s % r_size == 0 && s / r_size < ((size_t)1 << 31) && (size_t)n_mem * (s / r_size) <= l_size);
+  MsmGather G = {};
+  for (uint32_t i = 0; i < n_mem; i++) { REQUIRE(c, d_tables[i] && d_dims[i]); G.table[i] = d_tables[i]; G.dim[i] = d_dims[i]; }
+  G.n_mem = n_mem; G.rows_per_mem = (uint32_t)(s / r_size); G.e_out = d_e_u32;
+  int32_t rc = ensure_scratch(c, msm_pts_bytes(l_size, r_size) + 256); if (rc) return rc;
+  uint32_t bits = 0; while (bits < 32 && (max_value >> bits)) bits++;
+  uint32_t W = (bits + 3) / 4; if (W == 0) W = 1;
+  return run_msm(c, (const uint8_t*)d_e_u32, 4, W, r_size * 4, l_size, r_size, b, (uint8_t*)c->d_scratch, nullptr, out32, nullptr, &G);
+}
 int32_t lasso_msm(lasso_ctx* c, const lasso_bases* b, const lasso_fr* scalars, size_t n, lasso_point* out) {
   REQUIRE(c, b && scalars && out && n >= 1 && n <= b->n);
   int32_t rc = ensure_scratch(c, n * 64 + msm_pts_bytes(1, n)); if (rc) return rc;
diff --git a/lasso_amd/csrc/mont29.cuh b/lasso_amd/csrc/mont29.cuh
--- a/lasso_amd/csrc/mont29.cuh
+++ b/lasso_amd/csrc/mont29.cuh
@@ -183,6 +183,17 @@
   col[8] = 0;
   return m29_from_columns<M>(col);
 }
+template <class M> LHD m29<M> m29_acc_reduce_small(const m29_acc<M>& acc) {
+  int64_t h[17];
+#pragma unroll
+  for (int k = 0; k < 17; k++) h[k] = acc.h[k];
+  m29_rows<M>(h);
+  m29<M> r; int64_t c = 0;
+#pragma unroll
+  for (int k = 9; k < 17; k++) { int64_t x = h[k] + c; c = x >> 29; r.v[k - 9] = (int32_t)x & M29_MASK; }
+  r.v[8] = (int32_t)c;
+  return r;
+}
 template <class M> LHD m29<M> m29_reduce_columns(const int64_t* col, int shift) {
   int64_t l[9]; int64_t c = 0;
 #pragma unroll
diff --git a/lasso_amd/csrc/msm_kernels.cuh b/lasso_amd/csrc/msm_kernels.cuh
--- a/lasso_amd/csrc/msm_kernels.cuh
+++ b/lasso_amd/csrc/msm_kernels.cuh
@@ -463,19 +463,28 @@
     }
   }
 }
-__global__ void __launch_bounds__(MSM_THREADS) k_msm_rows8(const uint32_t* __restrict__ scal, size_t row_words, uint32_t n_cols, uint32_t cols_per_chunk, uint32_t W8,
-                                                            const niels29* __restrict__ tab8_0, const niels29* __restrict__ tab8_1, size_t tn, pt29* __restrict__ out, uint32_t* digit_count) {
+#define MSM_GATHER_MEMS (LASSO_MAX_PTRS / 2)
+struct MsmGather { const uint32_t* dim[MSM_GATHER_MEMS]; const uint32_t* table[MSM_GATHER_MEMS]; uint32_t n_mem, rows_per_mem; uint32_t* e_out; };
+
+template <bool GATHER>
+__device__ __forceinline__ void msm_rows8_body(const uint32_t* __restrict__ scal, size_t row_words, uint32_t n_cols, uint32_t cols_per_chunk, uint32_t W8,
+                                               const niels29* __restrict__ tab8_0, const niels29* __restrict__ tab8_1, size_t tn, pt29* __restrict__ out, uint32_t* digit_count, const MsmGather* G) {
   __shared__ pt29 pts[MSM_THREADS];
   __shared__ fe29 st[MSM_ST_ROWS][4];
   const fe29 d2 = fe_d2();
   const uint32_t t = threadIdx.x;
-  const uint32_t* row = scal + (size_t)blockIdx.y * row_words;
+  const uint32_t* row = GATHER ? nullptr : scal + (size_t)blockIdx.y * row_words;
+  const uint32_t mem = GATHER ? blockIdx.y / G->rows_per_mem : 0u;
+  const bool live = !GATHER || mem < G->n_mem;
+  const uint32_t* __restrict__ dimrow = GATHER && live ? G->dim[mem] + (size_t)(blockIdx.y - mem * G->rows_per_mem) * n_cols : nullptr;
+  const uint32_t* __restrict__ tbl = GATHER && live ? G->table[mem] : nullptr;
   const uint32_t c0 = blockIdx.x * cols_per_chunk;
   uint32_t c1 = c0 + cols_per_chunk; if (c1 > n_cols) c1 = n_cols;
   pt29 B = pt_identity();
   niels29 cur; bool have = false; uint32_t nadds = 0;
-  for (uint32_t c = c0 + t; c < c1; c += MSM_THREADS) {
-    const uint32_t v = row[c];
+  if (live) for (uint32_t c = c0 + t; c < c1; c += MSM_THREADS) {
+    uint32_t v;
+    if (GATHER) { v = tbl[dimrow[c]]; G->e_out[(size_t)blockIdx.y * n_cols + c] = v; } else v = row[c];
     for (uint32_t w = 0; w < W8; w++) {
       const uint32_t d = (v >> (8 * w)) & 255u;
       nadds += d != 0;
@@ -491,9 +500,18 @@
   msm_coop_tree(pts, st, MSM_THREADS, d2);
   if (t == 0) out[(size_t)blockIdx.y * gridDim.x + blockIdx.x] = pts[0];
 }
-
-__global__ void __launch_bounds__(MSM_THREADS) k_msm_rows8w(const uint32_t* __restrict__ scal, size_t row_words, uint32_t n_cols, uint32_t W8, const niels29* __restrict__ tab8_0,
-                                                             const niels29* __restrict__ tab8_1, size_t tn, pt29* __restrict__ out, uint32_t rows, uint32_t* digit_count, uint32_t rpw) {
+__global__ void __launch_bounds__(MSM_THREADS) k_msm_rows8(const uint32_t* __restrict__ scal, size_t row_words, uint32_t n_cols, uint32_t cols_per_chunk, uint32_t W8,
+                                                            const niels29* __restrict__ tab8_0, const niels29* __restrict__ tab8_1, size_t tn, pt29* __restrict__ out, uint32_t* digit_count) {
+  msm_rows8_body<false>(scal, row_words, n_cols, cols_per_chunk, W8, tab8_0, tab8_1, tn, out, digit_count, nullptr);
+}
+__global__ void __launch_bounds__(MSM_THREADS) k_msm_rows8_gather(MsmGather G, uint32_t n_cols, uint32_t cols_per_chunk, uint32_t W8,
+                                                                   const niels29* __restrict__ tab8_0, const niels29* __restrict__ tab8_1, size_t tn, pt29* __restrict__ out, uint32_t* digit_count) {
+  msm_rows8_body<true>(nullptr, 0, n_cols, cols_per_chunk, W8, tab8_0, tab8_1, tn, out, digit_count, &G);
+}
+
+template <bool GATHER>
+__device__ __forceinline__ void msm_rows8w_body(const uint32_t* __restrict__ scal, size_t row_words, uint32_t n_cols, uint32_t W8, const niels29* __restrict__ tab8_0,
+                                                const niels29* __restrict__ tab8_1, size_t tn, pt29* __restrict__ out, uint32_t rows, uint32_t* digit_count, uint32_t rpw, const MsmGather* G) {
   __shared__ pt29 pts[MSM_THREADS];
   const fe29 d2 = fe_d2();
   const uint32_t t = threadIdx.x, wave = t >> 6, lane = t & 63u;
@@ -503,12 +521,22 @@
     const uint32_t r = (blockIdx.x * (MSM_THREADS / 64) + wave) * rpw + k;
     if (r >= rows) break;
     pt29 B = pt_identity();
-    const uint32_t* row = scal + (size_t)r * row_words;
+    const uint32_t* row = GATHER ? nullptr : scal + (size_t)r * row_words;
+    const uint32_t mem = GATHER ? r / G->rows_per_mem : 0u;
+    const bool live = !GATHER || mem < G->n_mem;
+    const uint32_t* __restrict__ dimrow = GATHER && live ? G->dim[mem] + (size_t)(r - mem * G->rows_per_mem) * n_cols : nullptr;
+    const uint32_t* __restrict__ tbl = GATHER && live ? G->table[mem] : nullptr;
+    uint32_t* __restrict__ erow = GATHER && live ? G->e_out + (size_t)r * n_cols : nullptr;
     niels29 cur; bool have = false;
-    uint32_t v_next = lane < n_cols ? row[lane] : 0u;
-    for (uint32_t c = lane; c < n_cols; c += 64) {
+    uint32_t a_next = GATHER && live && lane + 64 < n_cols ? dimrow[lane + 64] : 0u;
+    uint32_t v_next = !live || lane >= n_cols ? 0u : GATHER ? tbl[dimrow[lane]] : row[lane];
+    if (live) for (uint32_t c = lane; c < n_cols; c += 64) {
       const uint32_t v = v_next;
-      v_next = c + 64 < n_cols ? row[c + 64] : 0u;
+      if (GATHER) {
+        erow[c] = v;
+        v_next = c + 64 < n_cols ? tbl[a_next] : 0u;
+        a_next = c + 128 < n_cols ? dimrow[c + 128] : 0u;
+      } else v_next = c + 64 < n_cols ? row[c + 64] : 0u;
       for (uint32_t w = 0; w < W8; w++) {
         const uint32_t d = (v >> (8 * w)) & 255u;
         nadds += d != 0;
@@ -527,6 +555,14 @@
     __builtin_amdgcn_fence(__ATOMIC_RELEASE, "wavefront"); __builtin_amdgcn_wave_barrier(); __builtin_amdgcn_fence(__ATOMIC_ACQUIRE, "wavefront");
   }
   msm_count_adds(digit_count, nadds);
+}
+__global__ void __launch_bounds__(MSM_THREADS) k_msm_rows8w(const uint32_t* __restrict__ scal, size_t row_words, uint32_t n_cols, uint32_t W8, const niels29* __restrict__ tab8_0,
+                                                             const niels29* __restrict__ tab8_1, size_t tn, pt29* __restrict__ out, uint32_t rows, uint32_t* digit_count, uint32_t rpw) {
+  msm_rows8w_body<false>(scal, row_words, n_cols, W8, tab8_0, tab8_1, tn, out, rows, digit_count, rpw, nullptr);
+}
+__global__ void __launch_bounds__(MSM_THREADS) k_msm_rows8w_gather(MsmGather G, uint32_t n_cols, uint32_t W8, const niels29* __restrict__ tab8_0,
+                                                                    const niels29* __restrict__ tab8_1, size_t tn, pt29* __restrict__ out, uint32_t rows, uint32_t* digit_count, uint32_t rpw) {
+  msm_rows8w_body<true>(nullptr, 0, n_cols, W8, tab8_0, tab8_1, tn, out, rows, digit_count, rpw, &G);
 }
 
 #define MSM_DIRECT_MAX_COLS 160
diff --git a/lasso_amd/csrc/poly_kernels.cuh b/lasso_amd/csrc/poly_kernels.cuh
--- a/lasso_amd/csrc/poly_kernels.cuh
+++ b/lasso_amd/csrc/poly_kernels.cuh
@@ -2,6 +2,7 @@
 #include <hip/hip_runtime.h>
 #include "fr.cuh"
 #include "fr29.cuh"
+#include "fingerprint_leaf.cuh"
 #include "handoff_device.cuh"
 #include "launch_plan.cuh"
 
@@ -1113,10 +1114,10 @@
   for (size_t x = blockIdx.x * (size_t)blockDim.x + threadIdx.x; x < n; x += (size_t)gridDim.x * blockDim.x) out[x] = fr29_store(fr29_mul(fr29_unpack_u(hi[x >> lo_bits]), fr29_unpack_s(lo[x & mask])));
 }
 
-__global__ void __launch_bounds__(LASSO_BLOCK) k_gp_layer(const fr_t* __restrict__ in, size_t half, fr_t* __restrict__ out) {
+__device__ __forceinline__ void gp_layer_body(const fr_t* __restrict__ in, size_t half, fr_t* __restrict__ out) {
   for (size_t i = blockIdx.x * (size_t)blockDim.x + threadIdx.x; i < half; i += (size_t)gridDim.x * blockDim.x) out[i] = fr29_store(fr29_mul(fr29_unpack_u(in[i]), fr29_unpack_s(in[i + half])));
 }
-__global__ void __launch_bounds__(LASSO_BLOCK) k_gp_layer2(const fr_t* __restrict__ in, size_t q, fr_t* __restrict__ o1, fr_t* __restrict__ o2) {
+__device__ __forceinline__ void gp_layer2_body(const fr_t* __restrict__ in, size_t q, fr_t* __restrict__ o1, fr_t* __restrict__ o2) {
   for (size_t i = blockIdx.x * (size_t)blockDim.x + threadIdx.x; i < q; i += (size_t)gridDim.x * blockDim.x) {
     const fr_t a = fr29_store(fr29_mul(fr29_unpack_u(in[i]), fr29_unpack_s(in[i + 2 * q])));
     const fr_t b = fr29_store(fr29_mul(fr29_unpack_u(in[i + q]), fr29_unpack_s(in[i + 3 * q])));
@@ -1124,7 +1125,7 @@
     o2[i] = fr29_store(fr29_mul(fr29_unpack_u(a), fr29_unpack_s(b)));
   }
 }
-__global__ void k_gp_tail(fr_t* __restrict__ tree, size_t len) {
+__device__ __forceinline__ void gp_tail_body(fr_t* __restrict__ tree, size_t len) {
   fr_t* in = tree;
   while (len > 2) {
     size_t half = len / 2; fr_t* out = in + len;
@@ -1134,6 +1135,16 @@
     in = out; len = half;
   }
 }
+__global__ void __launch_bounds__(LASSO_BLOCK) k_gp_layer(const fr_t* __restrict__ in, size_t half, fr_t* __restrict__ out) { gp_layer_body(in, half, out); }
+__global__ void __launch_bounds__(LASSO_BLOCK) k_gp_layer2(const fr_t* __restrict__ in, size_t q, fr_t* __restrict__ o1, fr_t* __restrict__ o2) { gp_layer2_body(in, q, o1, o2); }
+__global__ void k_gp_tail(fr_t* __restrict__ tree, size_t len) { gp_tail_body(tree, len); }
+__global__ void __launch_bounds__(LASSO_BLOCK) k_gp_layer_pair(fr_t* __restrict__ ta, fr_t* __restrict__ tb, size_t off, size_t half) {
+  fr_t* in = (blockIdx.y ? tb : ta) + off; gp_layer_body(in, half, in + 2 * half);
+}
+__global__ void __launch_bounds__(LASSO_BLOCK) k_gp_layer2_pair(fr_t* __restrict__ ta, fr_t* __restrict__ tb, size_t off, size_t q) {
+  fr_t* in = (blockIdx.y ? tb : ta) + off; gp_layer2_body(in, q, in + 4 * q, in + 6 * q);
+}
+__global__ void k_gp_tail_pair(fr_t* __restrict__ ta, fr_t* __restrict__ tb, size_t off, size_t len) { gp_tail_body((blockIdx.x ? tb : ta) + off, len); }
 
 __global__ void __launch_bounds__(LASSO_BLOCK) k_fingerprint_ops(const fr_t* __restrict__ table, const uint32_t* __restrict__ dim, const fr_t* __restrict__ read, size_t s,
                                                                   fr_t gamma, fr_t gamma2, fr_t tau, fr_t* __restrict__ out_r, fr_t* __restrict__ out_w) {
@@ -1167,6 +1178,28 @@
     }
     l1_r[i] = fr29_store(fr29_mul(fr29_unpack_u(lr[0]), fr29_unpack_s(lr[1])));
     l1_w[i] = fr29_store(fr29_mul(fr29_unpack_u(lw[0]), fr29_unpack_s(lw[1])));
+  }
+}
+__global__ void __launch_bounds__(LASSO_BLOCK) k_fingerprint_ops_int_l2(const uint32_t* __restrict__ table, const uint32_t* __restrict__ dim, const uint32_t* __restrict__ read, size_t s,
+                                                                         fr_t gamma, fr_t gamma2, fr_t tau, fr_t* __restrict__ out_r, fr_t* __restrict__ out_w, fr_t* __restrict__ l1_r, fr_t* __restrict__ l1_w,
+                                                                         fr_t* __restrict__ l2_r, fr_t* __restrict__ l2_w) {
+  const fingerprint_consts K = fingerprint_consts_from(gamma, gamma2, tau);
+  const size_t q = s / 4;
+  for (size_t i = blockIdx.x * (size_t)blockDim.x + threadIdx.x; i < q; i += (size_t)gridDim.x * blockDim.x) {
+    fr_t lr[4], lw[4];
+#pragma unroll
+    for (int e = 0; e < 4; e++) {
+      const size_t k = i + e * q;
+      const uint32_t a = dim[k];
+      fingerprint_leaves_int(read[k], table[a], a, K, lr[e], lw[e]);
+      out_r[k] = lr[e]; out_w[k] = lw[e];
+    }
+    const fr_t ar = fr29_store(fr29_mul(fr29_unpack_u(lr[0]), fr29_unpack_s(lr[2]))), br = fr29_store(fr29_mul(fr29_unpack_u(lr[1]), fr29_unpack_s(lr[3])));
+    l1_r[i] = ar; l1_r[i + q] = br;
+    l2_r[i] = fr29_store(fr29_mul(fr29_unpack_u(ar), fr29_unpack_s(br)));
+    const fr_t aw = fr29_store(fr29_mul(fr29_unpack_u(lw[0]), fr29_unpack_s(lw[2]))), bw = fr29_store(fr29_mul(fr29_unpack_u(lw[1]), fr29_unpack_s(lw[3])));
+    l1_w[i] = aw; l1_w[i + q] = bw;
+    l2_w[i] = fr29_store(fr29_mul(fr29_unpack_u(aw), fr29_unpack_s(bw)));
   }
 }
 template <bool RU32>
diff --git a/lasso_amd/device.py b/lasso_amd/device.py
--- a/lasso_amd/device.py
+++ b/lasso_amd/device.py
@@ -245,6 +245,33 @@
     def fingerprint_ops_gp(self, d_table, d_dim, d_read, s, gamma, tau, d_tree_r, d_tree_w):
         g = np.ascontiguousarray(gamma, dtype=np.uint64); t = np.ascontiguousarray(tau, dtype=np.uint64)
         self._chk(self.lib.lasso_fingerprint_ops_gp(self.ctx, C.c_void_p(d_table), C.c_void_p(d_dim), C.c_void_p(d_read), s, _vp(g), _vp(t), C.c_void_p(d_tree_r), C.c_void_p(d_tree_w)))
+
+    def _declare_u32(self):
+        if not hasattr(self, "_u32"):
+            try:
+                _abi.declare_u32(self.lib)
+            except AttributeError:
+                raise LassoError("this device library does not export the integer-column entries (include/lasso_hip_u32.h)")
+            self._u32 = True
+
+    def fingerprint_ops_gp_u32(self, d_table_u32, d_dim, d_read_u32, s, gamma, tau, d_tree_r, d_tree_w):
+        self._declare_u32()
+        g = np.ascontiguousarray(gamma, dtype=np.uint64); t = np.ascontiguousarray(tau, dtype=np.uint64)
+        self._chk(self.lib.lasso_fingerprint_ops_gp_u32(self.ctx, C.c_void_p(d_table_u32), C.c_void_p(d_dim), C.c_void_p(d_read_u32), s, _vp(g), _vp(t), C.c_void_p(d_tree_r), C.c_void_p(d_tree_w)))
+
+    def gp_build2(self, d_tree_a, d_tree_b, n):
+        self._declare_u32()
+        self._chk(self.lib.lasso_gp_build2(self.ctx, C.c_void_p(d_tree_a), C.c_void_p(d_tree_b), n))
+
+    def hyrax_commit_compressed_gather_u32(self, d_tables, d_dims, s, max_value, l_size, r_size, bases, d_e_u32):
+        self._declare_u32()
+        out = np.empty((l_size, 32), dtype=np.uint8)
+        self._chk(self.lib.lasso_hyrax_commit_compressed_gather_u32(self.ctx, self._ptrs(d_tables), self._ptrs(d_dims), len(d_tables), s, max_value, l_size, r_size, C.c_void_p(bases), C.c_void_p(d_e_u32), _vp(out)))
+        return out
+
+    def densify_keep_read_u32(self, d_read_u32):
+        self._declare_u32()
+        self._chk(self.lib.lasso_densify_keep_read_u32(self.ctx, C.c_void_p(d_read_u32) if d_read_u32 else None))
 
     def fingerprint_ops_gp_upper(self, d_table, d_dim, d_read, s, gamma, tau, d_upper_r, d_upper_w, read_u32=False):
         g = np.ascontiguousarray(gamma, dtype=np.uint64); t = np.ascontiguousarray(tau, dtype=np.uint64)
diff --git a/lasso_amd/host/prover.hpp b/lasso_amd/host/prover.hpp
--- a/lasso_amd/host/prover.hpp
+++ b/lasso_amd/host/prover.hpp
@@ -13,6 +13,11 @@
 #include "../../include/lasso_prover.h"
 #include "../csrc/operand_layout.cuh"
 #include "../../include/lasso_custom_check.h"
+#include "../../include/lasso_hip_u32.h"
+extern "C" int32_t lasso_densify_keep_read_u32(lasso_ctx*, uint32_t*) __attribute__((weak));
+extern "C" int32_t lasso_fingerprint_ops_gp_u32(lasso_ctx*, const uint32_t*, const uint32_t*, const uint32_t*, size_t, const lasso_fr*, const lasso_fr*, lasso_fr*, lasso_fr*) __attribute__((weak));
+extern "C" int32_t lasso_gp_build2(lasso_ctx*, lasso_fr*, lasso_fr*, size_t) __attribute__((weak));
+extern "C" int32_t lasso_hyrax_commit_compressed_gather_u32(lasso_ctx*, const uint32_t* const*, const uint32_t* const*, uint32_t, size_t, uint32_t, size_t, size_t, const lasso_bases*, uint32_t*, uint8_t*) __attribute__((weak));
 
 #include <chrono>
 #include <cstdio>
@@ -600,12 +605,15 @@
     if (!D->compact && n_l > 2 * C * s) d.chk(lasso_zero(d.ctx, D->combined_l_variate_polys.p + 2 * C * D->s_loc, (n_l - 2 * C * s) / P * sizeof(lasso_fr)), "lasso_zero");
     if (n_m > C * m) d.chk(lasso_zero(d.ctx, D->combined_log_m_variate_polys.p + C * D->m_loc, (n_m - C * m) / P * sizeof(lasso_fr)), "lasso_zero");
     auto densify_dim = make_source();
+    const bool keep_read = !D->compact && !d.capacity && P == 1 && D->s_loc >= 8 && lasso_densify_keep_read_u32 && lasso_fingerprint_ops_gp_u32 && sw::fingerprint_u32();
     DBuf tmp_dim, tmp_read; if (D->compact) { tmp_dim = DBuf(d, D->s_loc); tmp_read = DBuf(d, D->s_loc); }
     for (size_t i = 0; i < C; i++) {
       DBufU32 d_access(d, D->s_loc);
       lasso_fr* dim_out = D->compact ? tmp_dim.p : D->combined_l_variate_polys.p + i * D->s_loc;
       lasso_fr* read_out = D->compact ? tmp_read.p : D->combined_l_variate_polys.p + (C + i) * D->s_loc;
-      densify_dim(i, s, d_access.p, dim_out, read_out, D->combined_log_m_variate_polys.p + i * D->m_loc);
+      if (keep_read) { D->read_u32.emplace_back(d, D->s_loc); d.chk(lasso_densify_keep_read_u32(d.ctx, D->read_u32.back().p), "lasso_densify_keep_read_u32"); }
+      try { densify_dim(i, s, d_access.p, dim_out, read_out, D->combined_log_m_variate_polys.p + i * D->m_loc); }
+      catch (...) { if (keep_read) (void)lasso_densify_keep_read_u32(d.ctx, nullptr); throw; }
       D->dim_u32.push_back(std::move(d_access));
       if (D->compact) {
         DBufU32 r32(d, D->s_loc); uint32_t mx = 0;
@@ -1485,7 +1493,9 @@
     if (P == 1 && ints) {
       E_u32 = DBufU32(d, n_E);
       if (n_E > alpha * s) d.chk(lasso_zero(d.ctx, E_u32.p + alpha * s, (n_E - alpha * s) * sizeof(uint32_t)), "lasso_zero");
-      for (size_t i = 0; i < alpha; i++)
+      const size_t R_E = (size_t)1 << (nv_derefs - nv_derefs / 2), L_E = (size_t)1 << (nv_derefs / 2);
+      const bool self_gather = lasso_hyrax_commit_compressed_gather_u32 && sw::msm_gather() && s >= R_E && s % R_E == 0 && alpha <= 68;
+      if (!self_gather) for (size_t i = 0; i < alpha; i++)
         d.chk(lasso_gather_u32(d.ctx, tables_u32[S.memory_to_subtable_index(i)].p, dense.dim_u32[S.memory_to_dimension_index(i)].p, s, E_u32.p + i * s), "lasso_gather_u32");
       if (side_new) {
         field_side();
@@ -1493,13 +1503,20 @@
         d.chk_side(lasso_eq_evals(fc, rr.data(), (uint32_t)rr.size(), eq.p), "lasso_eq_evals");
       } else field_side();
       sp.reset(), sp.reset(new Trace("Subtables.commit", d.ctx));
-      comm_derefs = hyrax_commit(d, combined_E.p, nv_derefs, gens.gens_derefs, E_u32.p, table_max);
+      if (self_gather) {
+        std::vector<const uint32_t*> tp, dp;
+        for (size_t i = 0; i < alpha; i++) { tp.push_back(tables_u32[S.memory_to_subtable_index(i)].p); dp.push_back(dense.dim_u32[S.memory_to_dimension_index(i)].p); }
+        LASSO_REQUIRE(R_E == gens.gens_derefs.n);
+        comm_derefs.rows = L_E; comm_derefs.compressed.resize(32 * L_E);
+        d.chk(lasso_hyrax_commit_compressed_gather_u32(d.ctx, tp.data(), dp.data(), (uint32_t)alpha, s, table_max, L_E, R_E, gens.gens_derefs.bases, E_u32.p, comm_derefs.compressed.data()), "lasso_hyrax_commit_compressed_gather_u32");
+      } else comm_derefs = hyrax_commit(d, combined_E.p, nv_derefs, gens.gens_derefs, E_u32.p, table_max);
       if (side_new) side_sync();
     } else {
       field_side();
       sp.reset(), sp.reset(new Trace("Subtables.commit", d.ctx));
       comm_derefs = hyrax_commit(d, combined_E.p, nv_derefs, gens.gens_derefs);
     }
+    if (ops_from_ints()) ops_tables_u32 = std::move(tables_u32);
     tables_u32.clear();
     if (!side_new) eq_evals_local(r, eq.p);
     std::vector<const lasso_fr*> Eptr; for (size_t i = 0; i < alpha; i++) Eptr.push_back(E(i));
@@ -1552,6 +1569,10 @@
     HostClock::dump();
   }
 
+  std::vector<DBufU32> ops_tables_u32;
+  bool ops_from_ints() const {
+    return lasso_fingerprint_ops_gp_u32 && sw::fingerprint_u32() && P == 1 && !d.capacity && !dense.compact && S.integer_tables() && dense.read_u32.size() == dense.C && s_loc >= 8;
+  }
   void memory_checking_prove(const Sc& gamma, const Sc& tau, const std::vector<const lasso_fr*>& Eptr, DBuf& chis, ProofWriter& W) {
     t.append_protocol_name("Lasso MemoryCheckingProof");
     lasso_fr g = gamma.abi(), ta = tau.abi();
@@ -1560,12 +1581,17 @@
     const bool leafless = (d.capacity || dense.compact) && s_loc >= sw::leafless_min();
     if (d.capacity) { chis.reset(); d.trim_keep((leafless ? s_loc : 2 * s_loc) * sizeof(lasso_fr), 2 * alpha + (leafless && alpha == 4 ? 1 : 0)); }
     LeafLayer leaf; leaf.gamma = g; leaf.tau = ta; leaf.n_loc = s_loc;
+    const bool ints = ops_from_ints() && ops_tables_u32.size() == S.num_subtables();
+    const bool pair_trees = lasso_gp_build2 && sw::gp_pair() && P == 1 && !d.capacity;
     for (size_t i = 0; i < alpha; i++) {
       size_t j = S.memory_to_dimension_index(i); const lasso_fr* table = tables[S.memory_to_subtable_index(i)].p;
       DBuf ti(d, 2 * m_loc), tf(d, 2 * m_loc), tr(d, leafless ? s_loc : 2 * s_loc), tw(d, leafless ? s_loc : 2 * s_loc);
       d.chk(lasso_fingerprint_mem_slab(d.ctx, table, dense.final_(j), m_loc, (uint32_t)P, (uint32_t)d.comm.rank, &g, &ta, ti.p, tf.p), "lasso_fingerprint_mem");
-      d.chk(lasso_gp_build(d.ctx, ti.p, m_loc), "lasso_gp_build"); d.chk(lasso_gp_build(d.ctx, tf.p, m_loc), "lasso_gp_build");
-      if (leafless && dense.compact) {
+      if (pair_trees) d.chk(lasso_gp_build2(d.ctx, ti.p, tf.p, m_loc), "lasso_gp_build2");
+      else { d.chk(lasso_gp_build(d.ctx, ti.p, m_loc), "lasso_gp_build"); d.chk(lasso_gp_build(d.ctx, tf.p, m_loc), "lasso_gp_build"); }
+      if (ints) {
+        d.chk(lasso_fingerprint_ops_gp_u32(d.ctx, ops_tables_u32[S.memory_to_subtable_index(i)].p, dense.dim_u32[j].p, dense.read_u32[j].p, s_loc, &g, &ta, tr.p, tw.p), "lasso_fingerprint_ops_gp_u32");
+      } else if (leafless && dense.compact) {
         d.chk(lasso_fingerprint_ops_gp_upper_u32(d.ctx, table, dense.dim_u32[j].p, dense.read_u32[j].p, s_loc, &g, &ta, tr.p, tw.p), "lasso_fingerprint_ops_gp_upper_u32");
         leaf.mems.push_back({table, dense.dim_u32[j].p, nullptr, dense.read_u32[j].p});
       } else if (leafless) {
@@ -1579,6 +1605,7 @@
       }
       t_init.push_back(std::move(ti)); t_final.push_back(std::move(tf)); t_read.push_back(std::move(tr)); t_write.push_back(std::move(tw));
     }
+    ops_tables_u32.clear();
     if (Trace::mem()) d.dump_live("trees built");
     sp.reset(), sp.reset(new Trace("ProductLayer.prove", d.ctx));
     t.append_protocol_name("Lasso ProductLayerProof");
diff --git a/lasso_amd/host/switches.hpp b/lasso_amd/host/switches.hpp
--- a/lasso_amd/host/switches.hpp
+++ b/lasso_amd/host/switches.hpp
@@ -27,6 +27,9 @@
 LASSO_SWITCH(size_t, wire_device_min, [] { const char* e = getenv("LASSO_WIRE_DEVICE_MIN"); const long long x = e ? atoll(e) : 376; return (size_t)(x < 1 ? 1 : x); }())
 LASSO_SWITCH(bool, verify_msm_points, unless0(getenv("LASSO_VERIFY_MSM_POINTS")))
 LASSO_SWITCH(bool, densify_operands, unless0(getenv("LASSO_DENSIFY_OPERANDS")))
+LASSO_SWITCH(bool, fingerprint_u32, unless0(getenv("LASSO_FINGERPRINT_U32")))
+LASSO_SWITCH(bool, gp_pair, unless0(getenv("LASSO_GP_PAIR")))
+LASSO_SWITCH(bool, msm_gather, unless0(getenv("LASSO_MSM_GATHER")))
 inline bool slab_rccl() { return unless0(getenv("LASSO_SLAB_RCCL")); }
 inline bool debug_cubic_host() { return if1(getenv("LASSO_DEBUG_CUBIC_HOST")); }
 #undef LASSO_SWITCH
```
